# kalj/dealii-cuda

Measured on AMD Instinct MI355X. Metric: DoFs/s on 1305x Laplace vmult (bmop), p=4 3D uniform, higher is better.
Workload: dtype f64; 1 GPU; bmop: DEGREE_FE=4, DIMENSION=3, MATRIX_FREE_UNIFORM_MESH, hyper_cube(-1,1), 54^3 cells, 10218313 DoFs, 1 z-slab(s); cells_per_dir=54, n_dofs=10218313, n_cells=157464, parallelism=slab1, dof_numbering=caller's (lexicographic), finite=True, clock_ramp_steps=2000

## Files before the change

### dealii-cuda_amd/csrc/mfgpu_api.hip

```cpp
#include <hip/hip_runtime.h>

#include <type_traits>

#include <algorithm>
#include <cmath>
#include <cstdlib>
#include <cstring>
#include <memory>
#include <string>
#include <vector>

#include "mfgpu_kernels.h"

using namespace mfgpu;

struct EventTimer {
  std::vector<Event> ev;
  size_t used = 0;
  double ms = 0.0;
  int begin(hipStream_t st) {
    if (used + 2 > ev.size()) {
      Event e0, e1;
      int rc;
      if ((rc = e0.create(hipEventDefault)) || (rc = e1.create(hipEventDefault))) return rc;
      ev.push_back(std::move(e0));
      ev.push_back(std::move(e1));
    }
    HIP_TRY(hipEventRecord(ev[used].get(), st));
    return 0;
  }
  int end(hipStream_t st) {
    HIP_TRY(hipEventRecord(ev[used + 1].get(), st));
    used += 2;
    return 0;
  }
  int drain(double *total) {
    for (size_t i = 0; i + 1 < used; i += 2) {
      float t = 0.f;
      HIP_TRY(hipEventElapsedTime(&t, ev[i].get(), ev[i + 1].get()));
      ms += t;
    }
    used = 0;
    *total = ms;
    return 0;
  }
  void reset() {
    used = 0;
    ms = 0.0;
  }
};

struct mfgpu_handle {
  Plan plan;
  int dim = 0, n = 0, nd = 0, number_type = MFGPU_F64;
  bool hn = false;
  std::vector<double> S, Dt;
  std::vector<double> sv, sg;
  DeviceArray<uint32_t> d_batch_cell_off, d_batch_dof_off, d_bdofs;
  DeviceArray<uint8_t> d_bflags;
  DeviceArray<uint16_t> d_lmap;
  DeviceArray<uint16_t> d_lmapx;
  DeviceArray<uint16_t> d_perm;
  DeviceArray<uint32_t> d_bdofsp, d_idxp;
  DeviceArray<uint32_t> d_shtab;
  bool shared_records = false;
  size_t record_bytes = 0;
  DeviceArray<uint32_t> d_hnrec;
  DeviceArray<uint32_t> d_hn_slot;
  DeviceArray<void> d_coefp;
  DeviceArray<void> d_coef;
  DeviceArray<void> d_mass, d_massp;
  bool updatable = false;
  FoldGeometry geo;
  DeviceArray<uint32_t> d_cell_batch, d_cell_pos;
  size_t n_plane_cells = 0;
  DeviceArray<uint32_t> d_cmask, d_orphans;
  DeviceArray<void> d_hnw;
  DeviceArray<uint32_t> d_constrained;
  uint32_t n_constrained = 0;
  DeviceArray<void> d_tabsd;
  DeviceArray<void> d_tab2;
  bool twopass = true;
  DeviceArray<uint32_t> d_batch_nint, d_halo_off;
  std::vector<uint32_t> seg_end;
  std::vector<DeviceArray<uint32_t>> d_p2arr, d_p2tiles;
  std::vector<uint32_t> n_p2tiles;
  DeviceArray<uint32_t> d_p2rec, d_p2tab;
  bool p2_shared = false, p2_reverse = false, no_shared_records = false;
  Stream side;
  std::vector<Event> ev_seg;
  Event ev_side;
  bool side_pending = false;
  DeviceArray<void> d_halo;
  DeviceArray<unsigned long long> d_stamps;
  size_t lds = 0, device_bytes = 0;
  PlaneKernel planes = PlaneKernel::none;
  BatchKernel batches = BatchKernel::none;
  enum { kPlain, kMasked, kBatch };
  CellKernel<double> kernels_f64[3];
  CellKernel<float> kernels_f32[3];
  template <typename T>
  CellKernel<T> &kernel(int which) {
    if constexpr (std::is_same<T, double>::value) return kernels_f64[which];
    else return kernels_f32[which];
  }
  MultiKernel<double> multi_f64[kMaxFusedWidth - 1];
  MultiKernel<float> multi_f32[kMaxFusedWidth - 1];
  template <typename T>
  MultiKernel<T> &multi(int width) {
    if constexpr (std::is_same<T, double>::value) return multi_f64[width - 2];
    else return multi_f32[width - 2];
  }
  int multi_width = 1;
  DeviceArray<void> d_halo_multi;
  size_t halo_bytes = 0;
  uint32_t n_cus = 0, max_workgroups = 0;
  bool prof = false;
  EventTimer t_cells;
  EventTimer t_pass2;
  uint64_t prof_vmults = 0;
};

namespace {

template <typename T>
hipError_t bind_kernel(const mfgpu_handle *h, PlaneKernel pk, BatchKernel bk, bool hn, bool sh, CellKernel<T> *k) {
  const Plan &P = h->plan;
  const auto bind = pk == PlaneKernel::planes3 ? p_bind<T> : pk == PlaneKernel::planes4 ? q_bind<T>
                    : bk == BatchKernel::batches ? apply_bind<T> : bk == BatchKernel::x ? x_bind<T>
                    : bk == BatchKernel::g ? g_bind<T> : bk == BatchKernel::g2 ? g2_bind<T> : nullptr;
  if (!bind) return hipErrorInvalidValue;
  return bind(P.dim, P.n, hn, h->twopass, sh, h->d_mass.get() != nullptr, P.max_batch_dofs, k);
}

template <typename T, typename Args>
int launch_bound(mfgpu_handle *h, const CellKernel<T, Args> &k, const Args &a, uint32_t nbat, hipStream_t st) {
  if (!k.launch[0]) {
    set_error("cell-loop kernel not bound");
    return MFGPU_EINVAL;
  }
  uint32_t grid = (uint32_t)(k.per_cu < 1 ? 1 : k.per_cu) * h->n_cus;
  if (h->max_workgroups && h->max_workgroups < grid) grid = h->max_workgroups;
  HIP_TRY(k.launch[a.add != 0](a, h->S.data(), h->Dt.data(), k.lds, nbat < grid ? nbat : grid, st));
  return 0;
}

int check_symmetrize(int n, std::vector<double> &S, std::vector<double> &Dt) {
  const int p = n - 1;
  double err = 0, mag = 0;
  for (int r = 0; r < n; ++r)
    for (int c = 0; c < n; ++c) {
      const double s1 = S[r * n + c], s2 = S[(p - r) * n + (p - c)];
      const double d1 = Dt[r * n + c], d2 = -Dt[(p - r) * n + (p - c)];
      err = std::fmax(err, std::fmax(std::fabs(s1 - s2), std::fabs(d1 - d2)));
      mag = std::fmax(mag, std::fmax(std::fabs(s1), std::fabs(d1)));
    }
  if (err > 1e-10 * mag) {
    set_error("shape tables are not symmetric about the cell midpoint (unsupported)");
    return MFGPU_EUNSUPPORTED;
  }
  for (int r = 0; r < n; ++r)
    for (int c = 0; c < n; ++c) {
      const int r2 = p - r, c2 = p - c;
      if (r * n + c < r2 * n + c2) {
        const double s = 0.5 * (S[r * n + c] + S[r2 * n + c2]);
        S[r * n + c] = S[r2 * n + c2] = s;
        const double d = 0.5 * (Dt[r * n + c] - Dt[r2 * n + c2]);
        Dt[r * n + c] = d;
        Dt[r2 * n + c2] = -d;
      } else if (r == r2 && c == c2) {
        Dt[r * n + c] = 0.0;
      }
    }
  return 0;
}

int upload_pass2(mfgpu_handle *h, const uint32_t *priority, uint32_t n_priority) {
  const Plan &P = h->plan;
  const size_t ng = 1 + h->seg_end.size();
  const bool shared = P.sh_p2_use && !h->no_shared_records && n_priority == 0 && ng == 2;
  std::vector<Pass2Group> groups;
  int rc;
  if ((rc = pass2_groups(P, h->seg_end, priority, n_priority, shared, groups))) return rc;
  std::vector<DeviceArray<uint32_t>> d_arr(ng), d_tiles(ng);
  std::vector<uint32_t> n_tiles(ng, 0u);
  const bool reverse = (size_t)P.halo_off.back() * esize(h->number_type) <= ((size_t)256 << 20);
  DeviceArray<uint32_t> d_rec, d_tab;
  if (shared) {
    if ((rc = d_rec.upload(P.sh_p2rec.data(), P.sh_p2rec.size()))) return rc;
    if ((rc = d_tab.upload(P.sh_p2tab.data(), P.sh_p2tab.size()))) return rc;
  }
  for (size_t g = 0; g < ng; ++g) {
    std::vector<uint32_t> arr, tiles;
    build_pass2_classes(groups[g].dofs, groups[g].offsets, groups[g].slots, arr, tiles);
    n_tiles[g] = (uint32_t)(tiles.size() / 4);
    if (reverse) {
      const size_t nt = tiles.size() / 4;
      for (size_t a = 0, b = nt ? nt - 1 : 0; a < b; ++a, --b)
        for (int w = 0; w < 4; ++w) std::swap(tiles[4 * a + w], tiles[4 * b + w]);
    }
    if ((rc = d_arr[g].upload(arr.data(), arr.size()))) return rc;
    if ((rc = d_tiles[g].upload(tiles.data(), tiles.size()))) return rc;
  }
  h->d_p2arr = std::move(d_arr);
  h->d_p2tiles = std::move(d_tiles);
  h->n_p2tiles = std::move(n_tiles);
  h->d_p2rec = std::move(d_rec);
  h->d_p2tab = std::move(d_tab);
  h->p2_shared = shared;
  h->p2_reverse = reverse;
  return 0;
}

template <typename T>
int relayout_planes(mfgpu_handle *h, const uint32_t *cell_batch, const uint32_t *cell_pos, bool coef, bool mass,
                    hipStream_t st) {
  const size_t total = h->n_plane_cells * (size_t)h->nd;
  if (coef)
    HIP_TRY(relayout_coef_launch<T>(h->d_coefp.as<T>(), h->d_coef.as<const T>(), cell_batch, cell_pos, total, h->n, st));
  if (mass)
    HIP_TRY(relayout_coef_launch<T>(h->d_massp.as<T>(), h->d_mass.as<const T>(), cell_batch, cell_pos, total, h->n, st));
  return 0;
}

template <typename T>
int update_typed(mfgpu_handle *h, const void *coef, const void *mass, hipStream_t st) {
  const FoldInputs<T> in = h->geo.inputs<T>();
  if (coef) HIP_TRY(fold_coefficient_launch<T>(h->d_coef.as<T>(), (const T *)coef, in, st));
  if (mass) HIP_TRY(fold_mass_launch<T>(h->d_mass.as<T>(), (const T *)mass, in, st));
  if (h->planes == PlaneKernel::none) return 0;
  return relayout_planes<T>(h, h->d_cell_batch.get(), h->d_cell_pos.get(), coef != nullptr, mass != nullptr, st);
}

template <typename T>
int create_arrays(mfgpu_handle *h, const mfgpu_desc &d) {
  const Plan &P = h->plan;
  const size_t ncell = P.n_cells, nd = (size_t)P.nd;
  size_t &acct = h->device_bytes;
  auto up = [&](auto &arr, const void *src, size_t n) {
    const int rc = arr.upload(src, n);
    acct += arr.bytes();
    return rc;
  };
  int rc;
  if ((rc = up(h->d_batch_cell_off, P.batch_cell_off.data(), P.batch_cell_off.size()))) return rc;
  if ((rc = up(h->d_batch_dof_off, P.batch_dof_off.data(), P.batch_dof_off.size()))) return rc;
  if ((rc = up(h->d_bdofs, P.bdofs.data(), P.bdofs.size()))) return rc;
  if ((rc = up(h->d_bflags, P.bflags.data(), P.bflags.size()))) return rc;
  if ((rc = up(h->d_lmap, P.lmap.data(), P.lmap.size()))) return rc;
  const bool general = h->batches == BatchKernel::g || h->batches == BatchKernel::g2;
  if (h->batches == BatchKernel::x && !h->hn) {
    const std::vector<uint16_t> perm = x_lane_permutation(P.n);
    if ((rc = up(h->d_perm, perm.data(), perm.size()))) return rc;
  }
  if (h->batches == BatchKernel::x || general) {
    const std::vector<uint16_t> lx = x_pencil_runs(P.lmap, P.n);
    if ((rc = up(h->d_lmapx, lx.data(), lx.size()))) return rc;
  }
  if (h->batches == BatchKernel::g2) {
    std::vector<T> sd(2 * (size_t)P.n * P.n);
    for (int i = 0; i < P.n * P.n; ++i) {
      sd[i] = (T)h->S[i];
      sd[P.n * P.n + i] = (T)h->Dt[i];
    }
    if ((rc = up(h->d_tabsd, sd.data(), sd.size() * sizeof(T)))) return rc;
  }
  if (h->planes != PlaneKernel::none) {
    if ((rc = build_plane_records(h->plan, d.constraint_mask))) return rc;
    if (!P.pr_hn.empty()) {
      if ((rc = up(h->d_hnrec, P.pr_hn.data(), P.pr_hn.size()))) return rc;
      if ((rc = up(h->d_hn_slot, P.pr_hn_slot.data(), P.pr_hn_slot.size()))) return rc;
    }
    h->shared_records = P.sh_use && !(d.flags & MFGPU_NO_SHARED_RECORDS) &&
                        kernel_exists(h->planes, P.n, d.number_type, false, true, d.mass_coefficient != nullptr);
    const std::vector<uint32_t> &rd = h->shared_records ? P.sh_dofs : P.pr_dofs;
    const std::vector<uint32_t> &rx = h->shared_records ? P.sh_idx : P.pr_idx;
    if ((rc = up(h->d_bdofsp, rd.data(), rd.size()))) return rc;
    if ((rc = up(h->d_idxp, rx.data(), rx.size()))) return rc;
    if (h->shared_records && (rc = up(h->d_shtab, P.sh_batch.data(), P.sh_batch.size()))) return rc;
    h->record_bytes = h->d_bdofsp.bytes() + h->d_idxp.bytes() + h->d_shtab.bytes();
  }
  if ((rc = up(h->d_orphans, P.orphans.data(), P.orphans.size()))) return rc;
  if (h->twopass) {
    if ((rc = up(h->d_batch_nint, P.batch_nint.data(), P.batch_nint.size()))) return rc;
    if ((rc = up(h->d_halo_off, P.halo_off.data(), P.halo_off.size()))) return rc;
    if (h->planes != PlaneKernel::none && (uint64_t)P.halo_off.back() >= (1ull << 29)) {
      set_error("halo buffer too large for 32-bit byte offsets");
      return MFGPU_EUNSUPPORTED;
    }
    const size_t hb = ((size_t)P.halo_off.back() + 1) * sizeof(T);
    if ((rc = h->d_halo.alloc(hb, true))) return rc;
    acct += hb;
    h->halo_bytes = hb;
  }
  if (h->hn) {
    std::vector<uint32_t> cm(ncell);
    for (size_t i = 0; i < ncell; ++i) cm[i] = d.constraint_mask[P.cell_order[i]];
    if ((rc = up(h->d_cmask, cm.data(), ncell))) return rc;
    std::vector<T> w((size_t)h->n * h->n);
    for (size_t i = 0; i < w.size(); ++i) w[i] = (T)d.constraint_weights[i];
    if ((rc = up(h->d_hnw, w.data(), w.size() * sizeof(T)))) return rc;
  }
  FoldGeometry geo;
  if ((rc = geo.upload(d.JxW, d.inv_jac, P.cell_order.data(), P.dim, (uint32_t)ncell, (uint32_t)nd, general,
                       d.number_type)))
    return rc;
  DeviceArray<T> metric;
  if ((rc = fold_coefficient<T>(metric, d.coefficient, d.quadrature_points, geo.inputs<T>()))) return rc;
  h->d_coef = std::move(metric);
  acct += h->d_coef.bytes();
  if (d.mass_coefficient) {
    DeviceArray<T> mass;
    if ((rc = fold_mass<T>(mass, d.mass_coefficient, geo.inputs<T>()))) return rc;
    h->d_mass = std::move(mass);
    acct += h->d_mass.bytes();
  }
  if (h->updatable) {
    acct += geo.bytes();
    h->geo = std::move(geo);
  }
  if (h->planes != PlaneKernel::none) {
    const int n = P.n, NT = p_cells_per_wave(n) * n;
    const size_t nbat = P.n_plane_batches, total = nbat * (size_t)(n * n) * NT;
    const size_t ncell_p = P.batch_cell_off[nbat];
    std::vector<uint32_t> cb(ncell_p), cp(ncell_p);
    for (size_t b = 0; b < nbat; ++b)
      for (uint32_t c = P.batch_cell_off[b]; c < P.batch_cell_off[b + 1]; ++c) {
        cb[c] = (uint32_t)b;
        cp[c] = c - P.batch_cell_off[b];
      }
    DeviceArray<uint32_t> t_cb, t_cp;
    if ((rc = t_cb.upload(cb.data(), ncell_p))) return rc;
    if ((rc = t_cp.upload(cp.data(), ncell_p))) return rc;
    if ((rc = h->d_coefp.alloc(total * sizeof(T), true))) return rc;
    acct += h->d_coefp.bytes();
    h->n_plane_cells = ncell_p;
    if (d.mass_coefficient) {
      if ((rc = h->d_massp.alloc(total * sizeof(T), true))) return rc;
      acct += h->d_massp.bytes();
    }
    if ((rc = relayout_planes<T>(h, t_cb.get(), t_cp.get(), true, d.mass_coefficient != nullptr, nullptr))) return rc;
    HIP_TRY(hipDeviceSynchronize());
    if (h->updatable) {
      acct += t_cb.bytes() + t_cp.bytes();
      h->d_cell_batch = std::move(t_cb);
      h->d_cell_pos = std::move(t_cp);
    }
  }
  int dev = 0;
  hipDeviceProp_t prop;
  HIP_TRY(hipGetDevice(&dev));
  HIP_TRY(hipGetDeviceProperties(&prop, dev));
  h->n_cus = (uint32_t)prop.multiProcessorCount;
  h->max_workgroups = d.max_workgroups;
  if (h->planes != PlaneKernel::none) {
    CellKernel<T> &plain = h->kernel<T>(mfgpu_handle::kPlain), &masked = h->kernel<T>(mfgpu_handle::kMasked);
    HIP_TRY(bind_kernel<T>(h, h->planes, BatchKernel::none, false, h->shared_records, &plain));
    h->lds = plain.lds;
    if (P.n_plain_plane_batches < P.n_plane_batches) {
      HIP_TRY(bind_kernel<T>(h, h->planes, BatchKernel::none, true, false, &masked));
      h->lds = std::max(h->lds, masked.lds);
    }
  }
  if (h->batches == BatchKernel::none) return 0;
  CellKernel<T> &batch = h->kernel<T>(mfgpu_handle::kBatch);
  const hipError_t bind_batch_family = bind_kernel<T>(h, PlaneKernel::none, h->batches, h->hn, false, &batch);
  h->lds = batch.lds;
  if (h->lds > 160 * 1024) {
    set_error("batch needs more than 160 KiB of LDS; lower max_dofs_per_batch");
    return MFGPU_EINVAL;
  }
  HIP_TRY(bind_batch_family);
  if (h->twopass && h->planes == PlaneKernel::none)
    for (const int w : kFusedWidths) {
      if (!fused_kernel_exists(h->batches, P.n, d.number_type, h->hn, h->d_mass.get() != nullptr, w)) continue;
      MultiKernel<T> &mk = h->multi<T>(w);
      if (g_bind_width<T>(P.n, h->hn, false, h->d_mass.get() != nullptr, w, P.max_batch_dofs, &mk) != hipSuccess) {
        (void)hipGetLastError();
        mk = MultiKernel<T>();
      } else
        h->multi_width = std::max(h->multi_width, w);
    }
  return 0;
}

void choose_segments(mfgpu_handle *h, uint32_t request) {
  const Plan &P = h->plan;
  const uint32_t nb = (uint32_t)(P.batch_cell_off.size() - 1);
  h->seg_end.assign(1, nb);
  if (!h->twopass || nb < 2 || request == 1) return;
  const uint32_t npl = P.n_plane_batches, nplain = P.n_plain_plane_batches;
  std::vector<uint32_t> cuts;
  if (npl > 0 && npl < nb) cuts.push_back(npl);
  if (nplain > 0 && nplain < npl) cuts.push_back(nplain);
  if (request > 1) {
    for (uint32_t i = 1; i < request; ++i) cuts.push_back((uint32_t)((uint64_t)nb * i / request));
  }
  if (request == 0 && !P.pr_hn.empty() && nplain == 0 && P.n == 5) cuts.push_back(nb / 2);
  std::sort(cuts.begin(), cuts.end());
  h->seg_end.clear();
  for (uint32_t c : cuts)
    if (c > 0 && c < nb && (h->seg_end.empty() || h->seg_end.back() != c)) h->seg_end.push_back(c);
  h->seg_end.push_back(nb);
}

template <typename T>
int create_typed(mfgpu_handle *h, const mfgpu_desc &d) {
  int rc = create_arrays<T>(h, d);
  if (rc) return rc;
  choose_segments(h, d.cell_loop_segments);
  if (!h->twopass) return 0;
  if (h->seg_end.size() > 1) {
    int prio_least = 0, prio_greatest = 0;
    HIP_TRY(hipDeviceGetStreamPriorityRange(&prio_least, &prio_greatest));
    if ((rc = h->side.create(hipStreamNonBlocking, prio_least))) return rc;
    if ((rc = h->ev_side.create(hipEventDisableTiming))) return rc;
    h->ev_seg.resize(h->seg_end.size() - 1);
    for (Event &e : h->ev_seg)
      if ((rc = e.create(hipEventDisableTiming))) return rc;
  }
  return upload_pass2(h, nullptr, 0);
}

template <typename T>
int launch_pass2_group(mfgpu_handle *h, size_t group, void *dst, const void *src, hipStream_t st, int add) {
  if (h->p2_shared && group == 1)
    HIP_TRY(reduce_owner_batches_launch<T>((T *)dst, (const T *)src, h->d_halo.as<const T>(), h->d_p2rec.get(),
                                           h->d_p2tab.get(), (uint32_t)(h->plan.batch_cell_off.size() - 1),
                                           (uint32_t)p_hs(h->plan.n) * 64u, h->p2_reverse ? 1 : 0, add, st));
  HIP_TRY(reduce_classes_launch<T>((T *)dst, (const T *)src, h->d_halo.as<const T>(), h->d_p2arr[group].get(),
                                   h->d_p2tiles[group].get(), h->n_p2tiles[group], add, st));
  return 0;
}

template <typename T>
int vmult_pass2(mfgpu_handle *h, int phase, void *dst, const void *src, hipStream_t st, int add) {
  if (!h->twopass) return 0;
  if (phase == 0) return launch_pass2_group<T>(h, 0, dst, src, st, add);
  int rc = launch_pass2_group<T>(h, h->seg_end.size(), dst, src, st, add);
  if (!rc && h->side_pending) {
    HIP_TRY(hipStreamWaitEvent(st, h->ev_side.get(), 0));
    h->side_pending = false;
  }
  return rc;
}

template <typename T>
int launch_cells(mfgpu_handle *h, ApplyArgs<T> a, uint32_t b0, uint32_t b1, hipStream_t st) {
  const Plan &P = h->plan;
  const uint32_t npl = P.n_plane_batches, nplain = P.n_plain_plane_batches;
  if (b0 < nplain) {
    a.batch0 = b0;
    a.batch_end = b1 < nplain ? b1 : nplain;
    if (const int rc = launch_bound(h, h->kernel<T>(mfgpu_handle::kPlain), a, a.batch_end - a.batch0, st)) return rc;
    b0 = a.batch_end;
  }
  if (b0 < npl && b0 < b1) {
    a.batch0 = b0;
    a.batch_end = b1 < npl ? b1 : npl;
    if (const int rc = launch_bound(h, h->kernel<T>(mfgpu_handle::kMasked), a, a.batch_end - a.batch0, st)) return rc;
    b0 = a.batch_end;
  }
  if (b0 >= b1) return 0;
  a.batch0 = b0;
  a.batch_end = b1;
  return launch_bound(h, h->kernel<T>(mfgpu_handle::kBatch), a, b1 - b0, st);
}

template <typename T>
ApplyArgs<T> make_args(mfgpu_handle *h, void *dst, const void *src, int add) {
  const Plan &P = h->plan;
  ApplyArgs<T> a;
  a.batch_cell_off = h->d_batch_cell_off.get();
  a.batch_dof_off = h->d_batch_dof_off.get();
  a.bdofs = h->d_bdofs.get();
  a.bflags = h->d_bflags.get();
  a.lmap = h->d_lmap.get();
  a.lmapx = h->d_lmapx.get();
  a.perm = h->d_perm.get();
  a.bdofsp = h->d_bdofsp.get();
  a.idxp = h->d_idxp.get();
  a.shtab = h->shared_records ? h->d_shtab.get() : nullptr;
  a.hnrec = h->d_hnrec.get();
  a.hn_slot = h->d_hn_slot.get();
  a.coefp = h->d_coefp.as<const T>();
  a.coef = h->d_coef.as<const T>();
  a.mass = h->d_mass.as<const T>();
  a.massp = h->d_massp.as<const T>();
  a.cmask = h->d_cmask.get();
  a.hn_weights = h->d_hnw.as<const T>();
  a.tabS = h->d_tabsd.as<const T>();
  a.tabDt = a.tabS ? a.tabS + (size_t)P.n * P.n : nullptr;
  a.batch_nint = h->d_batch_nint.get();
  a.halo_off = h->d_halo_off.get();
  a.halo = h->d_halo.as<T>();
  a.dst = (T *)dst;
  a.src = (const T *)src;
  a.nb_max = P.max_batch_dofs;
  a.add = add;
  a.stamps = h->d_stamps.get();
  a.dbg = 0;
  return a;
}

template <typename T>
int vmult_main(mfgpu_handle *h, void *dst, const void *src, hipStream_t st, int add) {
  const Plan &P = h->plan;
  ApplyArgs<T> a = make_args<T>(h, dst, src, add);
  int rc;
  if (h->prof && (rc = h->t_cells.begin(st))) return rc;
  if (h->twopass) {
    const size_t nseg = h->seg_end.size();
    if (h->side_pending) {
      HIP_TRY(hipStreamWaitEvent(st, h->ev_side.get(), 0));
      h->side_pending = false;
    }
    for (size_t s = 0; s < nseg; ++s) {
      if ((rc = launch_cells<T>(h, a, s ? h->seg_end[s - 1] : 0u, h->seg_end[s], st))) return rc;
      if (s + 1 < nseg) {
        HIP_TRY(hipEventRecord(h->ev_seg[s].get(), st));
        HIP_TRY(hipStreamWaitEvent(h->side.get(), h->ev_seg[s].get(), 0));
        if ((rc = launch_pass2_group<T>(h, 1 + s, dst, src, h->side.get(), add))) return rc;
      }
    }
    if (nseg > 1) {
      HIP_TRY(hipEventRecord(h->ev_side.get(), h->side.get()));
      h->side_pending = true;
    }
  } else {
    for (size_t c = 0; c + 1 < P.color_batch_off.size(); ++c) {
      if (P.color_batch_off[c + 1] == P.color_batch_off[c]) continue;
      if ((rc = launch_cells<T>(h, a, P.color_batch_off[c], P.color_batch_off[c + 1], st))) return rc;
    }
  }
  if (h->prof && (rc = h->t_cells.end(st))) return rc;
  if (!h->twopass)
    HIP_TRY(orphan_launch<T>((T *)dst, (const T *)src, h->d_orphans.get(), (uint32_t)P.orphans.size(), add, st));
  if (h->prof) h->prof_vmults++;
  return 0;
}

template <typename T>
int vmult_typed(mfgpu_handle *h, void *dst, const void *src, hipStream_t st, int add) {
  int rc = vmult_main<T>(h, dst, src, st, add);
  if (rc) return rc;
  const bool timed = h->prof && h->twopass;
  if (timed && (rc = h->t_pass2.begin(st))) return rc;
  rc = vmult_pass2<T>(h, 0, dst, src, st, add);
  if (!rc) rc = vmult_pass2<T>(h, 1, dst, src, st, add);
  if (!rc && timed) rc = h->t_pass2.end(st);
  return rc;
}

bool fused_by_default(int , int ) { return false; }

template <typename T>
int multi_fused_group(mfgpu_handle *h, T *dst, const T *src, int nv, size_t stride, hipStream_t st, int add) {
  const MultiKernel<T> &k = h->multi<T>(nv);
  if (!k.launch[0]) {
    set_error("fused kernel not bound");
    return MFGPU_EINVAL;
  }
  if (!h->d_halo_multi.get()) {
    const size_t bytes = (size_t)(h->multi_width - 1) * h->halo_bytes;
    if (const int rc = h->d_halo_multi.alloc(bytes, true)) return rc;
// ... 41 lines not shown
  for (const uint32_t g : multi_groups(n_vectors, widths)) {
    const int rc = g > 1 ? multi_fused_group<T>(h, d, s, (int)g, stride, st, add) : vmult_typed<T>(h, d, s, st, add);
    if (rc) return rc;
    d += (size_t)g * stride;
    s += (size_t)g * stride;
  }
  return 0;
}

}

namespace {
template <typename T>
int inverse_diagonal_typed(mfgpu_handle *h, void *diag, hipStream_t st) {
  const Plan &P = h->plan;
  const bool general = h->batches == BatchKernel::g || h->batches == BatchKernel::g2;
  if (!h->d_tab2.get()) {
    const int nn = h->n * h->n;
    std::vector<T> t2(2 * (size_t)nn);
    for (int i = 0; i < nn; ++i) {
      t2[i] = (T)(general ? h->sv[i] : h->sv[i] * h->sv[i]);
      t2[nn + i] = (T)(general ? h->sg[i] : h->sg[i] * h->sg[i]);
    }
    if (const int rc = h->d_tab2.upload(t2.data(), t2.size() * sizeof(T))) return rc;
    h->device_bytes += h->d_tab2.bytes();
  }
  HIP_TRY(fill_launch<T>((T *)diag, P.n_dofs, T(0), st));
  const uint32_t nb = (uint32_t)(P.batch_cell_off.size() - 1), *cell_off = h->d_batch_cell_off.get();
  const uint32_t *dof_off = h->d_batch_dof_off.get(), *bdofs = h->d_bdofs.get(), *cmask = h->d_cmask.get();
  const uint16_t *lmap = h->d_lmap.get();
  const T *coef = h->d_coef.as<const T>(), *hnw = h->d_hnw.as<const T>(), *tab2 = h->d_tab2.as<const T>();
  if (h->batches == BatchKernel::g2)
    HIP_TRY(diag_general2_launch<T>(P.n, (T *)diag, nb, cell_off, dof_off, bdofs, lmap, coef, cmask, hnw, tab2, st));
  else if (h->batches == BatchKernel::g)
    HIP_TRY(diag_general_launch<T>(P.n, (T *)diag, nb, cell_off, dof_off, bdofs, lmap, coef, cmask, hnw, tab2, st));
  else
    HIP_TRY(diag_launch<T>(P.dim, P.n, (T *)diag, nb, cell_off, dof_off, bdofs, lmap, coef, cmask, hnw, tab2, st));
  if (h->d_mass.get())
    HIP_TRY(diag_mass_launch<T>(P.dim, P.n, (T *)diag, nb, cell_off, dof_off, bdofs, lmap, h->d_mass.as<const T>(), cmask,
                                hnw, tab2, !general, st));
  HIP_TRY(set_values_launch<T>((T *)diag, h->d_constrained.get(), h->n_constrained, T(1), st));
  HIP_TRY(vec_map_launch<T>(4, (T *)diag, nullptr, T(0), T(0), P.n_dofs, st));
  return 0;
}
}


namespace {
int vec_map(int op, void *v, const void *w, double s, double a, size_t n, int nt, void *stream) {
  if ((!v && n) || (!w && n && op <= 3)) {
    set_error("null vector");
    return MFGPU_EINVAL;
  }
  if (nt == MFGPU_F32)
    HIP_TRY(vec_map_launch<float>(op, (float *)v, (const float *)w, (float)s, (float)a, n, (hipStream_t)stream));
  else if (nt == MFGPU_F64)
    HIP_TRY(vec_map_launch<double>(op, (double *)v, (const double *)w, s, a, n, (hipStream_t)stream));
  else
    return MFGPU_EINVAL;
  return 0;
}
int vec_reduce(int op, void *v, const void *x, const void *w, double a, size_t n, int nt, void *stream, double *out) {
  if (!out || (n && (!v || (op != 2 && !w) || (op == 1 && !x)))) {
    set_error("null argument");
    return MFGPU_EINVAL;
  }
  if (nt == MFGPU_F32)
    HIP_TRY(vec_reduce_launch<float>(op, (float *)v, (const float *)x, (const float *)w, (float)a, n, (hipStream_t)stream, out));
  else if (nt == MFGPU_F64)
    HIP_TRY(vec_reduce_launch<double>(op, (double *)v, (const double *)x, (const double *)w, a, n, (hipStream_t)stream, out));
  else
    return MFGPU_EINVAL;
  return 0;
}
}


namespace mfgpu {
int handle_number_type(const mfgpu_handle *h) { return h->number_type; }
int handle_set_priority_dofs(mfgpu_handle *h, const uint32_t *ids, uint32_t n) {
  return h->twopass ? upload_pass2(h, ids, n) : 0;
}
int handle_n_batches(const mfgpu_handle *h) { return (int)h->plan.batch_cell_off.size() - 1; }
bool handle_ranged_ok(const mfgpu_handle *h) { return h->twopass && h->seg_end.size() == 1; }
int handle_batches_touching(const mfgpu_handle *h, const uint32_t *ids, uint32_t n, std::vector<uint8_t> &flags) {
  const Plan &P = h->plan;
  std::vector<uint8_t> mark(P.n_dofs, 0);
  for (uint32_t i = 0; i < n; ++i) {
    if (ids[i] >= P.n_dofs) {
      set_error("interface dof out of range");
      return MFGPU_EINVAL;
    }
    mark[ids[i]] = 1;
  }
  const size_t nb = P.batch_cell_off.size() - 1;
  flags.assign(nb, 0);
  for (size_t b = 0; b < nb; ++b)
    for (uint32_t t = P.batch_dof_off[b]; t < P.batch_dof_off[b + 1]; ++t)
      if (mark[P.bdofs[t] & 0x7fffffffu]) {
        flags[b] = 1;
        break;
      }
  return 0;
}
int handle_cells_range(mfgpu_handle *h, uint32_t b0, uint32_t b1, void *dst, const void *src, void *stream, int add) {
  if (b0 >= b1) return 0;
  hipStream_t st = (hipStream_t)stream;
  if (h->number_type == MFGPU_F64) return launch_cells<double>(h, make_args<double>(h, dst, src, add), b0, b1, st);
  return launch_cells<float>(h, make_args<float>(h, dst, src, add), b0, b1, st);
}
int handle_cells_two_ranges(mfgpu_handle *h, uint32_t b0, uint32_t b1, uint32_t c0, uint32_t c1, void *dst,
                            const void *src, void *stream, int add) {
  const uint32_t nplain = h->plan.n_plain_plane_batches, npl = h->plan.n_plane_batches;
  const bool plain = c1 <= nplain, masked = b0 >= nplain && c1 <= npl;
  if (b0 >= b1 || c0 >= c1 || b1 > c0 || !(plain || masked)) {
    const int rc = handle_cells_range(h, b0, b1, dst, src, stream, add);
    return rc ? rc : handle_cells_range(h, c0, c1, dst, src, stream, add);
  }
  hipStream_t st = (hipStream_t)stream;
  auto run = [&](auto a) -> int {
    a.batch0 = b0;
    a.batch_end = c1;
    a.hole0 = b1;
    a.hole_len = c0 - b1;
    using T = typename std::remove_const<typename std::remove_pointer<decltype(a.src)>::type>::type;
    return launch_bound(h, h->kernel<T>(plain ? mfgpu_handle::kPlain : mfgpu_handle::kMasked), a, (b1 - b0) + (c1 - c0),
                        st);
  };
  return h->number_type == MFGPU_F64 ? run(make_args<double>(h, dst, src, add)) : run(make_args<float>(h, dst, src, add));
}
int handle_pass2_group(mfgpu_handle *h, int group, void *dst, const void *src, void *stream, int add) {
  if (!h->twopass) return 0;
  hipStream_t st = (hipStream_t)stream;
  return h->number_type == MFGPU_F64 ? launch_pass2_group<double>(h, (size_t)group, dst, src, st, add)
                                     : launch_pass2_group<float>(h, (size_t)group, dst, src, st, add);
}
int handle_vmult_phase(mfgpu_handle *h, int phase, void *dst, const void *src, void *stream, int add) {
  hipStream_t st = (hipStream_t)stream;
  if (h->number_type == MFGPU_F64)
    return phase == 0 ? vmult_main<double>(h, dst, src, st, add) : vmult_pass2<double>(h, phase - 1, dst, src, st, add);
  return phase == 0 ? vmult_main<float>(h, dst, src, st, add) : vmult_pass2<float>(h, phase - 1, dst, src, st, add);
}
}

extern "C" {

int mfgpu_create(const mfgpu_desc *desc, mfgpu_handle **out) {
  if (!desc || !out) {
    set_error("null argument");
    return MFGPU_EINVAL;
  }
  const mfgpu_desc &d = *desc;
  if (!valid_number_type(d.number_type)) {
    set_error("number_type must be MFGPU_F64 or MFGPU_F32");
    return MFGPU_EINVAL;
  }
  const bool general = !(d.flags & MFGPU_UNIFORM_J0);
  if (general && (d.flags & MFGPU_COLORED_SCATTER)) {
    set_error("the general-Jacobian path (no MFGPU_UNIFORM_J0) is implemented in two-pass scatter mode only");
    return MFGPU_EUNSUPPORTED;
  }
  if (!d.JxW || !d.inv_jac || !d.shape_values || !d.shape_gradients ||
      (!d.coefficient && !d.quadrature_points)) {
    set_error("JxW, inv_jac, shape tables and coefficient (or quadrature_points) are required");
    return MFGPU_EINVAL;
  }
  const bool hn = (d.flags & MFGPU_HANGING_NODES) != 0;
// ... 66 lines not shown
}

int mfgpu_vmult_multi(mfgpu_handle *h, void *dst, const void *src, uint32_t n_vectors, size_t stride, uint32_t flags,
                      void *stream) {
  if (!h || !dst || !src) {
    set_error("null argument");
    return MFGPU_EINVAL;
  }
  const size_t nd = h->plan.n_dofs;
  if (n_vectors == 0 || (n_vectors > 1 && stride < nd)) {
    set_error("mfgpu_vmult_multi: n_vectors must be >= 1 and stride >= n_dofs");
    return MFGPU_EINVAL;
  }
  if ((flags & ~(MFGPU_MULTI_ADD | MFGPU_MULTI_LOOP | MFGPU_MULTI_FUSED)) ||
      ((flags & MFGPU_MULTI_LOOP) && (flags & MFGPU_MULTI_FUSED))) {
    set_error("mfgpu_vmult_multi: bad flags (MFGPU_MULTI_LOOP and MFGPU_MULTI_FUSED exclude each other)");
    return MFGPU_EINVAL;
  }
  const size_t bytes = ((size_t)(n_vectors - 1) * stride + nd) * esize(h->number_type);
  const char *d0 = (const char *)dst, *s0 = (const char *)src;
  if (d0 < s0 + bytes && s0 < d0 + bytes) {
    set_error("mfgpu_vmult_multi: the dst range overlaps the src range");
    return MFGPU_EINVAL;
  }
  return h->number_type == MFGPU_F64 ? vmult_multi_typed<double>(h, dst, src, n_vectors, stride, flags, (hipStream_t)stream)
                                     : vmult_multi_typed<float>(h, dst, src, n_vectors, stride, flags, (hipStream_t)stream);
}

int mfgpu_multi_width(const mfgpu_handle *h) { return h ? h->multi_width : 0; }

int mfgpu_update_coefficients(mfgpu_handle *h, const void *coefficient_dev, const void *mass_coefficient_dev,
                              void *stream) {
  if (!h) {
    set_error("null argument");
    return MFGPU_EINVAL;
  }
  if (!h->updatable) {
    set_error("mfgpu_update_coefficients: the handle was created without MFGPU_UPDATABLE_COEFFICIENTS");
    return MFGPU_EINVAL;
  }
  if (!coefficient_dev && !mass_coefficient_dev) {
    set_error("mfgpu_update_coefficients: coefficient_dev and mass_coefficient_dev are both NULL");
    return MFGPU_EINVAL;
  }
  if (mass_coefficient_dev && !h->d_mass.get()) {
    set_error("mfgpu_update_coefficients: the handle was created without a mass term (its kernels have no mass "
              "instantiation bound); create it with mass_coefficient");
    return MFGPU_EINVAL;
  }
  return h->number_type == MFGPU_F64 ? update_typed<double>(h, coefficient_dev, mass_coefficient_dev, (hipStream_t)stream)
                                     : update_typed<float>(h, coefficient_dev, mass_coefficient_dev, (hipStream_t)stream);
}

uint32_t mfgpu_n_dofs(const mfgpu_handle *h) { return h ? h->plan.n_dofs : 0; }

size_t mfgpu_memory_consumption(const mfgpu_handle *h) { return h ? h->device_bytes : 0; }

int mfgpu_plan_stats(const mfgpu_handle *h, uint64_t s[8]) {
  if (!h || !s) return MFGPU_EINVAL;
  const Plan &P = h->plan;
  s[0] = P.batch_cell_off.size() - 1;
  s[1] = P.color_batch_off.size() - 1;
  s[2] = P.bdofs.size();
  s[3] = P.max_batch_dofs;
  s[4] = P.max_batch_cells;
  s[5] = P.orphans.size();
  s[6] = P.n_first;
  s[7] = P.n_add;
  if (h->twopass) {
    const uint32_t nb = (uint32_t)s[0], npl = P.n_plane_batches, nplain = P.n_plain_plane_batches;
    const uint32_t edge[4] = {0u, nplain, npl, nb};
    s[1] = 0;
    for (size_t g = 0; g < h->seg_end.size(); ++g) {
      const uint32_t s0 = g ? h->seg_end[g - 1] : 0u, s1 = h->seg_end[g];
      for (int f = 0; f < 3; ++f)
        if (std::max(s0, edge[f]) < std::min(s1, edge[f + 1])) ++s[1];
    }
    s[6] = P.sdofs.size();
    s[7] = P.halo_off.back();
  }
  return 0;
}

int mfgpu_record_stats(const mfgpu_handle *h, uint64_t s[4]) {
  if (!h || !s) return MFGPU_EINVAL;
  const Plan &P = h->plan;
  const size_t n = (size_t)P.n, nb = (size_t)p_kgu((int)n) * 64, nx = ((n * n + 1) / 2) * (p_cells_per_wave((int)n) * n);
  const bool planes = h->planes != PlaneKernel::none;
  s[0] = (h->shared_records ? 1 : 0) | (h->p2_shared ? 2 : 0);
  s[1] = planes ? P.sh_dofs.size() / nb : 0;
  s[2] = planes ? P.sh_idx.size() / nx : 0;
  s[3] = h->record_bytes;
  return 0;
}

const char *mfgpu_kernel_name(const mfgpu_handle *h) {
  if (!h) return "";
  const bool x = h->batches == BatchKernel::x;
  switch (h->planes) {
    case PlaneKernel::planes3: return x ? "apply_planes3+apply_batches_x" : "apply_planes3";
    case PlaneKernel::planes4: return x ? "apply_planes4+apply_batches_x" : "apply_planes4";
    default: break;
  }
  switch (h->batches) {
    case BatchKernel::x: return "apply_batches_x";
    case BatchKernel::g: return "apply_batches_g";
    case BatchKernel::g2: return "apply_batches_g2";
    default: return "apply_batches";
  }
}

int mfgpu_profile_enable(mfgpu_handle *h, int on) {
  if (!h) return MFGPU_EINVAL;
  h->prof = on != 0;
  h->t_cells.reset();
  h->t_pass2.reset();
  h->prof_vmults = 0;
  return 0;
}

int mfgpu_profile_read_pass2(mfgpu_handle *h, double *ms) {
  if (!h || !ms) return MFGPU_EINVAL;
  HIP_TRY(hipDeviceSynchronize());
  return h->t_pass2.drain(ms);
}

int mfgpu_profile_read(mfgpu_handle *h, double *ms, uint64_t *nv) {
  if (!h || !ms || !nv) return MFGPU_EINVAL;
  HIP_TRY(hipDeviceSynchronize());
  if (const int rc = h->t_cells.drain(ms)) return rc;
  *nv = h->prof_vmults;
  return 0;
}

#ifdef MFGPU_STAMPS
int mfgpu_debug_stamps(mfgpu_handle *h, unsigned long long *out, size_t n_batches) {
  if (!h) return MFGPU_EINVAL;
  const size_t nbt = h->plan.batch_cell_off.size() - 1;
  if (!h->d_stamps.get()) return h->d_stamps.alloc(2 * nbt * 16, true);
  if (out && n_batches == nbt) {
    HIP_TRY(hipDeviceSynchronize());
    HIP_TRY(hipMemcpy(out, h->d_stamps.get(), 2 * nbt * 16 * sizeof(unsigned long long), hipMemcpyDeviceToHost));
  }
  return 0;
}
#endif


int mfgpu_compute_inverse_diagonal(mfgpu_handle *h, void *inv_diag, void *stream) {
  if (!h || !inv_diag) {
    set_error("null argument");
    return MFGPU_EINVAL;
  }
  return h->number_type == MFGPU_F64 ? inverse_diagonal_typed<double>(h, inv_diag, (hipStream_t)stream)
                                     : inverse_diagonal_typed<float>(h, inv_diag, (hipStream_t)stream);
}

int mfgpu_set_constrained_values(mfgpu_handle *h, void *vec, double value, void *stream) {
  if (!h || !vec) {
    set_error("null argument");
    return MFGPU_EINVAL;
  }
  if (h->number_type == MFGPU_F64)
    HIP_TRY(set_values_launch<double>((double *)vec, h->d_constrained.get(), h->n_constrained, value, (hipStream_t)stream));
  else
    HIP_TRY(set_values_launch<float>((float *)vec, h->d_constrained.get(), h->n_constrained, (float)value,
// ... 81 lines not shown
```

### dealii-cuda_amd/csrc/mfgpu_internal.h

```cpp
#ifndef MFGPU_INTERNAL_H
#define MFGPU_INTERNAL_H

#include <cstdint>
#include <string>
#include <vector>

#include "../../include/mfgpu.h"

namespace mfgpu {

void set_error(const std::string &msg);

inline int ipow(int a, int e) {
  int r = 1;
  for (int i = 0; i < e; ++i) r *= a;
  return r;
}

constexpr int p_cells_per_wave(int n) { return 64 / n; }
constexpr int p_ji(int n) { return n == 3 ? 2 : n == 4 ? 5 : n == 5 ? 9 : n == 6 ? 14 : 23; }
constexpr int p_hs(int n) { return n == 3 ? 3 : n == 4 ? 6 : n == 5 ? 9 : n == 6 ? 14 : 18; }
constexpr int p_kgu(int n) { return p_ji(n) + p_hs(n); }
constexpr int p_cell_stride(int n) {
  int s = n * n * n;
  while ((s & 31) != (n & 31)) ++s;
  return s;
}

constexpr int q_plane_stride(int n) { return n >= 6 ? 65 : n == 5 ? 33 : n == 4 ? 17 : 33; }
constexpr int q_cell_stride(int n) { return n * q_plane_stride(n); }
constexpr int p_priv_max(int n) { return n >= 5 ? 384 : n == 4 ? 256 : 192; }
constexpr int kHnOpRounds = 2;
constexpr int p_hn_rows(int n) { return p_priv_max(n) / 64 + 3 * kHnOpRounds * 3 + 2; }

template <typename T>
constexpr size_t q_region_doubles(int n) {
  const size_t t = ((size_t)(p_cells_per_wave(n) + 1) * q_cell_stride(n) * sizeof(T) + 7) / 8;
  const size_t u = (size_t)p_kgu(n) * 64 + p_priv_max(n);
  return t > u ? t : u;
}
template <typename T>
constexpr size_t q_lds_bytes(int n, bool hn) {
  return (q_region_doubles<T>(n) + (hn ? (size_t)n * n : 0)) * 8;
}

constexpr uint8_t kFlagConstrained = 1;
constexpr uint8_t kFlagAdd = 2;

struct Plan {
  int dim = 0, degree = 0, n = 0, nd = 0;
  uint32_t n_dofs = 0, n_cells = 0;
  std::vector<uint32_t> cell_order;
  std::vector<uint32_t> batch_cell_off;
  std::vector<uint32_t> batch_dof_off;
  std::vector<uint32_t> color_batch_off;
  std::vector<uint32_t> bdofs;
  std::vector<uint8_t> bflags;
  std::vector<uint16_t> lmap;
  std::vector<uint32_t> orphans;
  std::vector<uint32_t> batch_nint;
  std::vector<uint32_t> halo_off;
  std::vector<uint32_t> sdofs;
  std::vector<uint32_t> s_off;
  std::vector<uint32_t> s_idx;
  std::vector<uint32_t> chunks;
  std::vector<uint32_t> gstarts;
  uint32_t max_batch_dofs = 0, max_batch_cells = 0;
  uint32_t n_plane_batches = 0;
  uint32_t n_plain_plane_batches = 0;
  std::vector<uint32_t> pr_dofs, pr_idx, pr_hn, pr_hn_slot;
  std::vector<uint32_t> sh_dofs, sh_idx, sh_batch;
  bool sh_use = false;
  std::vector<uint32_t> sh_p2rec, sh_p2tab;
  bool sh_p2_use = false;
  uint64_t n_first = 0, n_add = 0;
};

struct PlanLimits {
  uint32_t max_cells = 0, max_dofs = 0;
  uint32_t interior_max = 0, shared_max = 0, halo_stride = 0;
  bool segregate_masked = false;
  bool masked_planes = false;
  uint32_t private_max = 0;
};

int build_plan(const mfgpu_desc &d, Plan &plan, uint32_t max_chunks = 3, const PlanLimits *limits = nullptr);

struct HnLine {
  uint16_t node[8];
};
void hn_cell_lines(unsigned mask, int n, std::vector<HnLine> (&lines)[3], std::vector<uint16_t> &nodes);

enum class PlaneKernel : uint8_t { none, planes3, planes4 };
enum class BatchKernel : uint8_t { none, batches, x, g, g2 };
int choose_kernel_and_plan(const mfgpu_desc &d, PlaneKernel &pk, BatchKernel &bk, Plan &plan);

constexpr bool planes4_wide(int n) { return n >= 6; }
constexpr bool kernel_exists(PlaneKernel k, int n, int number_type, bool hn, bool sh, bool mass) {
  switch (k) {
    case PlaneKernel::planes3: return n >= 3 && n <= 5 && !(sh && hn);
    case PlaneKernel::planes4:
      return planes4_wide(n) ? n <= 7 && !hn && !sh && !mass
                             : n >= 3 && !sh && !(mass && n == 5 && number_type == MFGPU_F64);
    default: return false;
  }
}
constexpr bool kernel_exists(BatchKernel k, int n, int , bool , bool sh, bool ) {
  return k != BatchKernel::none && n >= 2 && n <= 7 && !sh;
}
constexpr int kFusedWidths[] = {3, 2};
constexpr bool fused_kernel_exists(BatchKernel k, int n, int number_type, bool hn, bool , int nv) {
  return k == BatchKernel::g && n >= 2 && n <= 7 && (nv == 2 || nv == 3) &&
         !(hn && number_type == MFGPU_F64 && n >= (nv == 3 ? 6 : 7));
}
std::vector<uint32_t> multi_groups(uint32_t n_vectors, const std::vector<uint32_t> &widths);
int build_plane_records(Plan &plan, const uint32_t *constraint_mask);
constexpr int kShBatchWords = 4;
constexpr double kShareMaxFraction = 0.5;
void share_plane_records(Plan &plan);
constexpr int kP2Header = 16, kP2MaxK = 12, kP2SlotBits = 12;
void share_pass2_records(Plan &plan);

std::vector<uint16_t> x_lane_permutation(int n);
std::vector<uint16_t> x_pencil_runs(const std::vector<uint16_t> &lmap, int n);
struct Pass2Group {
  std::vector<uint32_t> dofs, offsets = std::vector<uint32_t>(1, 0u), slots;
};
int pass2_groups(const Plan &plan, const std::vector<uint32_t> &seg_end, const uint32_t *priority, uint32_t n_priority,
                 bool shared, std::vector<Pass2Group> &groups);

int derive_tables(int n, const double *shape_values, const double *shape_gradients,
                  std::vector<double> &S, std::vector<double> &Dt);

int handle_number_type(const mfgpu_handle *h);
int handle_set_priority_dofs(mfgpu_handle *h, const uint32_t *ids, uint32_t n);
int handle_vmult_phase(mfgpu_handle *h, int phase, void *dst, const void *src, void *stream, int add);
int handle_n_batches(const mfgpu_handle *h);
bool handle_ranged_ok(const mfgpu_handle *h);
int handle_batches_touching(const mfgpu_handle *h, const uint32_t *ids, uint32_t n, std::vector<uint8_t> &flags);
int handle_cells_range(mfgpu_handle *h, uint32_t b0, uint32_t b1, void *dst, const void *src, void *stream, int add);
int handle_cells_two_ranges(mfgpu_handle *h, uint32_t b0, uint32_t b1, uint32_t c0, uint32_t c1, void *dst,
                            const void *src, void *stream, int add);
int handle_pass2_group(mfgpu_handle *h, int group, void *dst, const void *src, void *stream, int add);

void transfer_sizes(const mfgpu_transfer *t, uint32_t *n_coarse_dofs, uint32_t *n_fine_dofs, int *number_type);
void vcycle_active(const mfgpu_vcycle *v, int *active_type, uint32_t *n_active);

}

struct mfgpu_plan {
  mfgpu::Plan plan;
};

#endif
```

### dealii-cuda_amd/csrc/mfgpu_kernels.h

```cpp
#ifndef MFGPU_KERNELS_H
#define MFGPU_KERNELS_H

#include <hip/hip_runtime.h>

#include <type_traits>

#include "mfgpu_device.h"
#include "mfgpu_internal.h"

namespace mfgpu {

template <typename T>
struct ApplyArgs {
  const uint32_t *batch_cell_off;
  const uint32_t *batch_dof_off;
  const uint32_t *bdofs;
  const uint8_t *bflags;
  const uint16_t *lmap;
  const uint16_t *lmapx;
  const uint16_t *perm;
  const uint32_t *bdofsp;
  const uint32_t *idxp;
  const T *coefp;
  const uint32_t *hnrec;
  const uint32_t *hn_slot;
  const T *coef;
  const uint32_t *cmask;
  const T *hn_weights;
  const T *tabS, *tabDt;
  const uint32_t *batch_nint;
  const uint32_t *halo_off;
  T *halo;
  T *dst;
  const T *src;
  uint32_t batch0;
  uint32_t batch_end;
  uint32_t hole0 = 0xffffffffu, hole_len = 0;
  uint32_t nb_max;
  int add;
  unsigned long long *stamps;
  int dbg;
  const uint32_t *shtab = nullptr;
  const T *mass = nullptr;
  const T *massp = nullptr;
};

constexpr int kMaxFusedWidth = 3;
template <typename T>
struct MultiArgs : ApplyArgs<T> {
  size_t stride = 0;
  T *halos[kMaxFusedWidth];
};
constexpr size_t kMaxLdsBytes = 160 * 1024;

template <typename T, int n>
struct Tables {
  T S[((n + 1) / 2) * n];
  T Dt[((n + 1) / 2) * n];
};

template <typename T, int n>
inline Tables<T, n> make_tables(const double *S, const double *Dt) {
  Tables<T, n> tab;
  for (int i = 0; i < ((n + 1) / 2) * n; ++i) {
    tab.S[i] = (T)S[i];
    tab.Dt[i] = (T)Dt[i];
  }
  return tab;
}

template <typename T, typename Args = ApplyArgs<T>>
struct CellKernel {
  size_t lds = 0;
  int per_cu = 0;
  hipError_t (*launch[2])(const Args &a, const double *S, const double *Dt, size_t lds, uint32_t grid,
                          hipStream_t st) = {nullptr, nullptr};
};

template <typename T, int Block, auto K, auto MakeTab, typename Args = ApplyArgs<T>>
hipError_t launch_cell_kernel(const Args &a, const double *S, const double *Dt, size_t lds, uint32_t grid,
                              hipStream_t st) {
  if constexpr (std::is_null_pointer_v<decltype(MakeTab)>)
    hipLaunchKernelGGL(K, dim3(grid), dim3(Block), lds, st, a);
  else
    hipLaunchKernelGGL(K, dim3(grid), dim3(Block), lds, st, a, MakeTab(S, Dt));
  return hipGetLastError();
}

template <typename T, int Block, auto K0, auto K1, auto MakeTab, typename Args = ApplyArgs<T>>
hipError_t bind_cell_kernel(size_t lds, CellKernel<T, Args> *k) {
  k->lds = lds;
  for (const void *f : {(const void *)K1, (const void *)K0})
    if (const hipError_t e = hipFuncSetAttribute(f, hipFuncAttributeMaxDynamicSharedMemorySize, (int)lds)) return e;
  k->launch[0] = launch_cell_kernel<T, Block, K0, MakeTab, Args>;
  k->launch[1] = launch_cell_kernel<T, Block, K1, MakeTab, Args>;
  return hipOccupancyMaxActiveBlocksPerMultiprocessor(&k->per_cu, (const void *)K0, Block, lds);
}

template <typename F>
hipError_t dispatch_flags(F &&f) { return f(); }
template <typename F, typename... B>
hipError_t dispatch_flags(F &&f, bool flag, B... rest) {
  return dispatch_flags(
      [&](auto... c) { return flag ? f(std::true_type{}, c...) : f(std::false_type{}, c...); }, rest...);
}
template <typename F, typename... B>
hipError_t dispatch_instantiation(int n, F &&f, B... flags) {
  auto at = [&](auto N) { return dispatch_flags([&](auto... c) { return f(N, c...); }, flags...); };
  switch (n) {
    case 2: return at(std::integral_constant<int, 2>{});
    case 3: return at(std::integral_constant<int, 3>{});
    case 4: return at(std::integral_constant<int, 4>{});
    case 5: return at(std::integral_constant<int, 5>{});
    case 6: return at(std::integral_constant<int, 6>{});
    case 7: return at(std::integral_constant<int, 7>{});
    default: return hipErrorInvalidValue;
  }
}
template <typename T>
constexpr int number_type_of = sizeof(T) == 8 ? MFGPU_F64 : MFGPU_F32;

#define MFGPU_CELL_LOOP_FAMILY(F)                                                                              \
  template <typename T>                                                                                        \
  hipError_t F##_bind(int dim, int n, bool hn, bool twopass, bool sh, bool mass, uint32_t nb_max, CellKernel<T> *k);
MFGPU_CELL_LOOP_FAMILY(apply)
MFGPU_CELL_LOOP_FAMILY(x)
MFGPU_CELL_LOOP_FAMILY(g)
MFGPU_CELL_LOOP_FAMILY(g2)
MFGPU_CELL_LOOP_FAMILY(p)
MFGPU_CELL_LOOP_FAMILY(q)
#undef MFGPU_CELL_LOOP_FAMILY
template <typename T>
using MultiKernel = CellKernel<T, MultiArgs<T>>;
template <typename T, typename Args>
hipError_t g_bind_width(int n, bool hn, bool sh, bool mass, int nv, uint32_t nb_max, CellKernel<T, Args> *k);

void build_pass2_classes(const std::vector<uint32_t> &sdofs, const std::vector<uint32_t> &s_off,
                         const std::vector<uint32_t> &s_idx, std::vector<uint32_t> &arr, std::vector<uint32_t> &tiles);
template <typename T>
hipError_t reduce_classes_launch(T *dst, const T *src, const T *halo, const uint32_t *arr, const uint32_t *tiles,
                                 uint32_t n_tiles, int add, hipStream_t st);
template <typename T>
hipError_t reduce_classes_multi_launch(int nv, T *dst, const T *src, size_t stride, T *const *halos, const uint32_t *arr,
                                       const uint32_t *tiles, uint32_t n_tiles, int add, hipStream_t st);
template <typename T>
hipError_t reduce_owner_batches_launch(T *dst, const T *src, const T *halo, const uint32_t *rec, const uint32_t *tab,
                                       uint32_t n_batches, uint32_t hstride, int reverse, int add, hipStream_t st);
template <typename T>
hipError_t relayout_coef_launch(T *out, const T *in, const uint32_t *cell_batch, const uint32_t *cell_pos,
                                size_t total, int n, hipStream_t st);
template <typename T>
hipError_t fold_general_launch(T *M, const T *coef, const T *jxw, const T *jinv, const uint32_t *order,
                               uint32_t n_cells, uint32_t nd, hipStream_t st);
template <typename T>
hipError_t fold_general2_launch(T *M, const T *coef, const T *jxw, const T *jinv, const uint32_t *order,
                                uint32_t n_cells, uint32_t nd, hipStream_t st);
template <typename T>
hipError_t orphan_launch(T *dst, const T *src, const uint32_t *orph, uint32_t n, int add, hipStream_t st);
template <typename T>
hipError_t coefficient_launch(T *coef, const T *qpts, size_t nq, int dim, hipStream_t st);
template <typename T>
hipError_t fold_launch(T *c, const T *coef, const T *jxw, const T *j0, const uint32_t *order,
                       uint32_t n_cells, uint32_t nd, hipStream_t st);
template <typename T>
hipError_t fill_launch(T *v, size_t n, T a, hipStream_t st);
template <typename T>
struct FoldInputs {
  const T *jxw = nullptr, *jinv = nullptr;
  const uint32_t *order = nullptr;
  int dim = 0;
  uint32_t n_cells = 0, nd = 0;
  bool general = false;
  size_t metric_entries() const { return (size_t)n_cells * nd * (general ? (dim == 3 ? 6 : 3) : 1); }
};
template <typename T>
hipError_t fold_coefficient_launch(T *out, const T *coef, const FoldInputs<T> &in, hipStream_t st);
template <typename T>
hipError_t fold_mass_launch(T *out, const T *c, const FoldInputs<T> &in, hipStream_t st);
struct FoldGeometry {
  DeviceArray<void> jxw, jinv;
  DeviceArray<uint32_t> order;
  int dim = 0;
  uint32_t n_cells = 0, nd = 0;
  bool general = false;
  int upload(const void *JxW, const void *inv_jac, const uint32_t *cell_order, int dim_, uint32_t n_cells_, uint32_t nd_,
             bool general_, int number_type);
  size_t bytes() const { return jxw.bytes() + jinv.bytes() + order.bytes(); }
  template <typename T>
  FoldInputs<T> inputs(const T *jxw_resident = nullptr) const {
    FoldInputs<T> in;
    in.jxw = jxw_resident ? jxw_resident : jxw.as<const T>();
    in.jinv = jinv.as<const T>();
    in.order = order.get();
    in.dim = dim, in.n_cells = n_cells, in.nd = nd, in.general = general;
    return in;
  }
};
template <typename T>
int fold_mass(DeviceArray<T> &out, const void *mass_coefficient, const FoldInputs<T> &in);
template <typename T>
int fold_coefficient(DeviceArray<T> &out, const void *coefficient, const void *quadrature_points,
                     const FoldInputs<T> &in);

template <typename T>
hipError_t diag_launch(int dim, int n, T *diag, uint32_t n_batches, const uint32_t *batch_cell_off,
                       const uint32_t *batch_dof_off, const uint32_t *bdofs, const uint16_t *lmap, const T *coef,
                       const uint32_t *cmask, const T *hn_weights, const T *tab2, hipStream_t st);
template <typename T>
hipError_t diag_general_launch(int n, T *diag, uint32_t n_batches, const uint32_t *batch_cell_off,
                               const uint32_t *batch_dof_off, const uint32_t *bdofs, const uint16_t *lmap,
                               const T *metric, const uint32_t *cmask, const T *hn_weights, const T *tab,
                               hipStream_t st);
template <typename T>
hipError_t diag_general2_launch(int n, T *diag, uint32_t n_batches, const uint32_t *batch_cell_off,
                                const uint32_t *batch_dof_off, const uint32_t *bdofs, const uint16_t *lmap,
                                const T *metric, const uint32_t *cmask, const T *hn_weights, const T *tab,
                                hipStream_t st);
template <typename T>
hipError_t diag_mass_launch(int dim, int n, T *diag, uint32_t n_batches, const uint32_t *batch_cell_off,
                            const uint32_t *batch_dof_off, const uint32_t *bdofs, const uint16_t *lmap, const T *mass,
                            const uint32_t *cmask, const T *hn_weights, const T *tab, bool squared, hipStream_t st);
template <typename T>
hipError_t set_values_launch(T *v, const uint32_t *idx, uint32_t n, T value, hipStream_t st);
template <typename T>
hipError_t vec_map_launch(int op, T *v, const T *w, T s, T a, size_t n, hipStream_t st);
template <typename T>
hipError_t vec_reduce_launch(int op, T *v, const T *x, const T *w, T a, size_t n, hipStream_t st, double *out);

}
#endif
// ... 1 lines not shown
```

### dealii-cuda_amd/csrc/mfgpu_kernels_p.hip

```cpp
#include <hip/hip_runtime.h>

#include "mfgpu_cell.h"
#include "mfgpu_kernels.h"
#include "mfgpu_planes.h"

namespace mfgpu {

#define MFGPU_PIN_VMEM() __builtin_amdgcn_sched_barrier(0x380)

template <int n, typename T, bool ADD, bool HN, bool SH = false, bool MASS = false>
__global__ void __launch_bounds__(64) __attribute__((amdgpu_waves_per_eu(1, 1)))
apply_planes3(const ApplyArgs<T> A, const TablesEO<T, n> tab) {
  constexpr int n2 = n * n;
  constexpr int CW = p_cells_per_wave(n);
  constexpr int NT = CW * n;
  constexpr int KGU = p_kgu(n);
  constexpr int JI = p_ji(n);
  constexpr int HS = KGU - JI;
  constexpr int SA = p_cell_stride(n);
  constexpr int NIW = (n2 + 1) / 2;
  extern __shared__ __attribute__((aligned(16))) unsigned char smem_raw[];
  constexpr int PRIV = HN ? p_priv_max(n) : 0;
  double *ua = reinterpret_cast<double *>(smem_raw);
  T *Aw = reinterpret_cast<T *>(ua + KGU * 64 + PRIV + (HN ? n2 : 0));
  T *Bw = Aw + (CW + 1) * SA;
  double *Wl = ua + KGU * 64 + PRIV;

  const int lane = threadIdx.x;
  if (HN) {
    if (lane < n2) Wl[lane] = (double)A.hn_weights[lane];
  }
  const int lc = lane / n, k = lane - lc * n;
  const bool lane_on = lane < NT;
  const int tk = lane_on ? lane : NT - 1;

  uint32_t b, bstride, bend;
  {
    const uint32_t nbt = A.batch_end - A.batch0 - A.hole_len, G = gridDim.x;
    if (G >= 8 && nbt >= G) {
      const uint32_t xcd = blockIdx.x & 7u, slot = blockIdx.x >> 3;
      const uint32_t q = G >> 3, rem = G & 7u;
      const uint32_t wlo = xcd * q + (xcd < rem ? xcd : rem);
      const uint32_t w = q + (xcd < rem ? 1u : 0u);
      b = A.batch0 + (uint32_t)((uint64_t)nbt * wlo / G) + slot;
      bend = A.batch0 + (uint32_t)((uint64_t)nbt * (wlo + w) / G);
      bstride = w;
    } else {
      b = A.batch0 + blockIdx.x;
      bend = A.batch_end - A.hole_len;
      bstride = G;
    }
  }
  if (b >= bend) return;
  const uint32_t hole0 = A.hole0, hole_len = A.hole_len;
  auto next_of = [&](uint32_t x) {
    const uint32_t l = (x >= hole0 ? x - hole_len : x) + bstride;
    return l < bend ? (l >= hole0 ? l + hole_len : l) : x;
  };
  if (b >= hole0) b += hole_len;
  static_assert(kernel_exists(PlaneKernel::planes3, n, number_type_of<T>, HN, SH, MASS), "no such instantiation");
  struct Meta {
    uint32_t base, drec, irec;
  };
  auto meta_request = [&](uint32_t bb) -> uint32_t {
    return A.shtab[(size_t)bb * kShBatchWords + (lane & (kShBatchWords - 1))];
  };
  auto meta_of = [&](uint32_t v) -> Meta {
    return Meta{(uint32_t)__builtin_amdgcn_readlane((int)v, 0), (uint32_t)__builtin_amdgcn_readlane((int)v, 1),
                (uint32_t)__builtin_amdgcn_readlane((int)v, 2)};
  };

  auto load_dofs = [&](uint32_t rec, uint32_t (&g)[KGU]) {
    const uint32_t *p = A.bdofsp + (size_t)rec * (KGU * 64) + lane;
#pragma unroll
    for (int j = 0; j < KGU; ++j) g[j] = SH ? p[j * 64] : nt_load(p + j * 64);
  };
  auto src_at = [&](uint32_t base, uint32_t g) -> T {
    const T *const sp = SH ? A.src + base : A.src;
    return *reinterpret_cast<const T *>(reinterpret_cast<const char *>(sp) + (uint32_t)(g * (uint32_t)sizeof(T)));
  };
  auto dst_at = [&](uint32_t base, uint32_t g) -> T * {
    T *const dp = SH ? A.dst + base : A.dst;
    return reinterpret_cast<T *>(reinterpret_cast<char *>(dp) + (uint32_t)(g * (uint32_t)sizeof(T)));
  };
  auto load_ix = [&](uint32_t rec, uint32_t (&ix)[NIW]) {
    const uint32_t *p = A.idxp + (size_t)rec * (NIW * NT) + tk;
#pragma unroll
    for (int w = 0; w < NIW; ++w) ix[w] = SH ? p[w * NT] : nt_load(p + w * NT);
  };
  auto stage_src = [&](const uint32_t (&g)[KGU], const T (&sv)[KGU]) {
#pragma unroll
    for (int j = 0; j < KGU; ++j) {
      double v = (double)sv[j];
      if (j >= JI) {
        const unsigned long long keep = (unsigned long long)(long long)~((int)g[j] >> 31);
        v = __longlong_as_double((long long)((unsigned long long)__double_as_longlong(v) & keep));
      }
      ua[lane + j * 64] = v;
    }
  };
  auto ixb = [&](const uint32_t (&ix)[NIW], int i) -> uint32_t {
    return (i & 1) ? (ix[i >> 1] >> 16) : (ix[i >> 1] & 0xffffu);
  };
  auto scatter_slot = [&](int j, uint32_t bb, uint32_t base, uint32_t g, T r, T oldv) {
    if (j < JI) {
      *dst_at(base, g) = ADD ? oldv + r : r;
    } else {
      T *const hp = A.halo + (size_t)bb * (HS * 64) + lane;
      hp[(j - JI) * 64] = r;
    }
  };

  uint32_t b1 = next_of(b), b2 = next_of(b1);
  uint32_t Gp[KGU], Gc[KGU], Gn[KGU], Gnn[KGU];
  uint32_t IXc[NIW], IXn[NIW];
  constexpr int CR = PRIV / 64, HROWS = HN ? p_hn_rows(n) : 1;
  uint32_t Hc[HROWS], Hn[HROWS];
  auto load_hn = [&](uint32_t bb, uint32_t (&H)[HROWS]) {
    const uint32_t slot = A.hn_slot[bb];
    if (slot != 0xffffffffu) {
      const uint32_t *p = A.hnrec + (size_t)slot * (HROWS * 64) + lane;
#pragma unroll
      for (int w = 0; w < HROWS; ++w) H[w] = nt_load(p + w * 64);
    } else {
#pragma unroll
      for (int w = 0; w < HROWS; ++w) H[w] = 0u;
    }
  };
  T Cc[n2];
  T Mm[MASS ? n2 : 1];
  T SVn[KGU], R[KGU], old[KGU];
  Meta Mp{0u, 0u, 0u}, Mc = Mp, M1 = Mp, M2 = Mp;
  uint32_t Mv = 0u;
  if (SH) {
    Mc = meta_of(meta_request(b));
    M1 = meta_of(meta_request(b1));
    M2 = meta_of(meta_request(b2));
    Mp = Mc;
  }
  load_dofs(SH ? Mc.drec : b, Gc);
  load_dofs(SH ? M1.drec : b1, Gn);
  load_ix(SH ? Mc.irec : b, IXc);
  if (HN) load_hn(b, Hc);
  constexpr uint32_t kDummyIx = 8u * (uint32_t)(KGU * 64 - 1) * 0x10001u;
#pragma unroll
  for (int w = 0; w < NIW; ++w) IXc[w] = lane_on ? IXc[w] : kDummyIx;
  {
    const T *p = A.coefp + (size_t)b * (n2 * NT) + tk;
#pragma unroll
    for (int r = 0; r < n2; ++r) Cc[r] = nt_load(p + r * NT);
  }
  if (MASS) {
    const T *p = A.massp + (size_t)b * (n2 * NT) + tk;
#pragma unroll
    for (int r = 0; r < n2; ++r) Mm[r] = nt_load(p + r * NT);
  }
#pragma unroll
  for (int j = 0; j < KGU; ++j) {
    SVn[j] = src_at(Mc.base, Gc[j]);
    Gp[j] = Gc[j];
    R[j] = T(0);
    old[j] = T(0);
  }
  stage_src(Gc, SVn);
  WaveSync::sync();

  const int pxy = lc * SA + n2 * k;
  const int pyz = lc * SA + k;
  uint32_t bp = b;

  while (true) {
    const bool has_next = b1 != b;
    constexpr int kH2 = HN ? HROWS - 2 : 0, kH1 = HN ? HROWS - 1 : 0;
    const uint32_t hn_ncopy = HN ? (uint32_t)__builtin_amdgcn_readfirstlane(Hc[kH2] & 0xffffu) : 0u;
    auto hn_count = [&](int dir) -> uint32_t {
      const uint32_t w = dir == 0 ? Hc[kH2] >> 16 : dir == 1 ? Hc[kH1] & 0xffffu : Hc[kH1] >> 16;
      return (uint32_t)__builtin_amdgcn_readfirstlane(w);
    };
    auto hn_pass = [&](int dir, bool transposed, const double (&Wr)[n2]) {
      const uint32_t count = hn_count(dir);
#pragma unroll
      for (int r = 0; r < kHnOpRounds; ++r) {
        if ((uint32_t)(r * 64) >= count) break;
        const bool on = (uint32_t)(r * 64 + lane) < count;
        const uint32_t *ww = &Hc[CR + (dir * kHnOpRounds + r) * 3];
        double v[n], o[n];
        uint32_t pos[n];
#pragma unroll
        for (int t = 0; t < n; ++t) {
          pos[t] = on ? (ww[t >> 1] >> (16 * (t & 1))) & 0xffffu : (uint32_t)(KGU * 64 + PRIV - 1);
          v[t] = ua[pos[t]];
        }
#pragma unroll
        for (int i = 0; i < n; ++i) {
          double acc = 0.0;
#pragma unroll
          for (int k2 = 0; k2 < n; ++k2) acc = fma(transposed ? Wr[k2 * n + i] : Wr[i * n + k2], v[k2], acc);
          o[i] = acc;
        }
        if (on) {
#pragma unroll
          for (int i = 0; i < n; ++i) ua[pos[i]] = o[i];
        }
      }
    };
    if (HN && hn_ncopy) {
      double Wr[n2];
#pragma unroll
      for (int i = 0; i < n2; ++i) Wr[i] = Wl[i];
      double cv[CR > 0 ? CR : 1];
#pragma unroll
      for (int r = 0; r < CR; ++r) cv[r] = (uint32_t)(r * 64 + lane) < hn_ncopy ? ua[Hc[r] & 0xffffu] : 0.0;
#pragma unroll
      for (int r = 0; r < CR; ++r)
        if ((uint32_t)(r * 64 + lane) < hn_ncopy) ua[Hc[r] >> 16] = cv[r];
      WaveSync::sync();
      hn_pass(0, false, Wr);
      WaveSync::sync();
      hn_pass(1, false, Wr);
      WaveSync::sync();
      hn_pass(2, false, Wr);
      WaveSync::sync();
    }
    STAMP(0);
    RSTAMP(8);
    WGSTAMP(10);
    load_dofs(SH ? M2.drec : b2, Gnn);
    load_ix(SH ? M1.irec : b1, IXn);
    if (SH) Mv = meta_request(next_of(b2));
    if (HN) load_hn(b1, Hn);
    if (ADD) {
#pragma unroll
      for (int j = 0; j < JI; ++j) old[j] = *dst_at(Mp.base, Gp[j]);
    }
    STAMP(1);
    auto hookA = [&](int) {};
    auto hookB = [&](int s) {
      MFGPU_PIN_VMEM();
#pragma unroll
      for (int j = (KGU * s) / (5 * n); j < (KGU * (s + 1)) / (5 * n); ++j)
        scatter_slot(j, bp, Mp.base, Gp[j], R[j], old[j]);
#pragma unroll
      for (int j = (KGU * s) / (5 * n); j < (KGU * (s + 1)) / (5 * n); ++j)
        SVn[j] = src_at(M1.base, Gn[j]);
      MFGPU_PIN_VMEM();
    };
    const T *const cnext = A.coefp + (size_t)b1 * (n2 * NT) + tk;
    const T *const mnext = MASS ? A.massp + (size_t)b1 * (n2 * NT) + tk : nullptr;
    auto hookC = [&](int s) {
      MFGPU_PIN_VMEM();
#pragma unroll
      for (int r = (n2 * s) / (2 * n); r < (n2 * (s + 1)) / (2 * n); ++r)
        Cc[r] = nt_load(cnext + r * NT);
      if (MASS) {
#pragma unroll
        for (int r = (n2 * s) / (2 * n); r < (n2 * (s + 1)) / (2 * n); ++r)
          Mm[r] = nt_load(mnext + r * NT);
      }
      MFGPU_PIN_VMEM();
    };

    {
      T u[n2];
#pragma unroll
      for (int x = 0; x < n; ++x)
#pragma unroll
        for (int y = 0; y < n; ++y)
          u[x + n * y] = (T) * reinterpret_cast<const double *>(reinterpret_cast<const char *>(ua) + ixb(IXc, x + n * y));
#pragma unroll
      for (int x = 0; x < n; ++x) {
        T in[n], out[n];
        get_line<n, 1>(u, x, in);
        eo_apply<n, 0>(tab, in, out);
        set_line<n, 1>(u, x, out);
        hookA(x);
      }
#pragma unroll
      for (int y = 0; y < n; ++y) {
        T in[n], a[n], bb[n];
        get_line<n, 0>(u, y, in);
        eo_apply<n, 0>(tab, in, a);
        eo_apply<n, 2>(tab, a, bb);
#pragma unroll
        for (int x = 0; x < n; ++x) {
          Aw[pxy + x + n * y] = a[x];
          Bw[pxy + x + n * y] = bb[x];
        }
        hookA(n + y);
      }
    }
    WaveSync::sync();
    STAMP(2);
#pragma unroll
    for (int j = 0; j < KGU + PRIV / 64; ++j) ua[lane + j * 64] = 0.0;

    {
      T nx[n];
#pragma unroll
      for (int z = 0; z < n; ++z) nx[z] = Bw[pyz + n2 * z];
#pragma unroll
      for (int y = 0; y < n; ++y) {
        T in[n], g[n], o[n];
#pragma unroll
        for (int z = 0; z < n; ++z) in[z] = nx[z];
#pragma unroll
        for (int z = 0; z < n; ++z) nx[z] = y + 1 < n ? Bw[pyz + n * (y + 1) + n2 * z] : Aw[pyz + n2 * z];
        eo_apply<n, 0>(tab, in, g);
#pragma unroll
        for (int z = 0; z < n; ++z) g[z] *= Cc[y + n * z];
        eo_apply<n, 1>(tab, g, o);
#pragma unroll
        for (int z = 0; z < n; ++z) Bw[pyz + n * y + n2 * z] = o[z];
        hookB(y);
      }
      T v[n2], r[n2];
#pragma unroll
      for (int y = 0; y < n; ++y) {
        T in[n], o[n];
#pragma unroll
        for (int z = 0; z < n; ++z) in[z] = nx[z];
        if (y + 1 < n) {
#pragma unroll
          for (int z = 0; z < n; ++z) nx[z] = Aw[pyz + n * (y + 1) + n2 * z];
        }
// ... 21 lines not shown
        for (int y = 0; y < n; ++y) g[y] *= Cc[y + n * z];
        eo_apply<n, 3>(tab, g, o);
#pragma unroll
        for (int y = 0; y < n; ++y) r[y + n * z] += MASS ? fma(Mm[y + n * z], in[y], o[y]) : o[y];
        hookB(3 * n + z);
      }
#pragma unroll
      for (int y = 0; y < n; ++y) {
        T in[n], o[n];
        get_line<n, 1>(r, y, in);
        eo_apply<n, 1>(tab, in, o);
#pragma unroll
        for (int z = 0; z < n; ++z) Aw[pyz + n * y + n2 * z] = o[z];
        hookB(4 * n + y);
      }
    }
    WaveSync::sync();
    STAMP(3);

    {
      T o[n2];
      T nr[n], nt[n];
#pragma unroll
      for (int x = 0; x < n; ++x) {
        nr[x] = Aw[pxy + x];
        nt[x] = Bw[pxy + x];
      }
#pragma unroll
      for (int y = 0; y < n; ++y) {
        T rp[n], tp[n], w[n], ol[n];
#pragma unroll
        for (int x = 0; x < n; ++x) {
          rp[x] = nr[x];
          tp[x] = nt[x];
        }
        if (y + 1 < n) {
#pragma unroll
          for (int x = 0; x < n; ++x) {
            nr[x] = Aw[pxy + x + n * (y + 1)];
            nt[x] = Bw[pxy + x + n * (y + 1)];
          }
        }
        eo_apply<n, 3>(tab, tp, w);
#pragma unroll
        for (int x = 0; x < n; ++x) w[x] += rp[x];
        eo_apply<n, 1>(tab, w, ol);
        set_line<n, 0>(o, y, ol);
        hookC(y);
      }
#pragma unroll
      for (int x = 0; x < n; ++x) {
        T in[n], out[n];
        get_line<n, 1>(o, x, in);
        eo_apply<n, 1>(tab, in, out);
#pragma unroll
        for (int y = 0; y < n; ++y)
          lds_add(reinterpret_cast<double *>(reinterpret_cast<char *>(ua) + ixb(IXc, x + n * y)), (double)out[y]);
        hookC(n + x);
      }
    }
    WaveSync::sync();
    STAMP(4);

    if (HN && hn_ncopy) {
      double Wr[n2];
#pragma unroll
      for (int i = 0; i < n2; ++i) Wr[i] = Wl[i];
      hn_pass(2, true, Wr);
      WaveSync::sync();
      hn_pass(1, true, Wr);
      WaveSync::sync();
      hn_pass(0, true, Wr);
      WaveSync::sync();
      double cv[CR > 0 ? CR : 1];
#pragma unroll
      for (int r = 0; r < CR; ++r) cv[r] = (uint32_t)(r * 64 + lane) < hn_ncopy ? ua[Hc[r] >> 16] : 0.0;
#pragma unroll
      for (int r = 0; r < CR; ++r)
        if ((uint32_t)(r * 64 + lane) < hn_ncopy) lds_add(ua + (Hc[r] & 0xffffu), cv[r]);
      WaveSync::sync();
    }
#pragma unroll
    for (int j = 0; j < KGU; ++j) R[j] = (T)ua[lane + j * 64];
    WaveSync::sync();
    STAMP(5);
    stage_src(Gn, SVn);
    STAMP(6);
    bp = b;
    if (SH) Mp = Mc;
#pragma unroll
    for (int j = 0; j < KGU; ++j) Gp[j] = Gc[j];
    STAMP(7);
    RSTAMP(9);
    if (!has_next) break;
    WaveSync::sync();
    b = b1;
    b1 = b2;
    b2 = next_of(b2);
    if (SH) {
      Mc = M1;
      M1 = M2;
      M2 = meta_of(Mv);
    }
#pragma unroll
    for (int j = 0; j < KGU; ++j) {
      Gc[j] = Gn[j];
      Gn[j] = Gnn[j];
    }
#pragma unroll
    for (int w = 0; w < NIW; ++w) IXc[w] = lane_on ? IXn[w] : kDummyIx;
    if (HN) {
#pragma unroll
      for (int w = 0; w < HROWS; ++w) Hc[w] = Hn[w];
    }
  }
  if (ADD) {
#pragma unroll
    for (int j = 0; j < JI; ++j) old[j] = *dst_at(Mp.base, Gp[j]);
  }
#pragma unroll
  for (int j = 0; j < KGU; ++j) scatter_slot(j, bp, Mp.base, Gp[j], R[j], old[j]);
}

template <int n, typename T>
static size_t p_lds_bytes(bool hn) {
  return ((size_t)p_kgu(n) * 64 + (hn ? (size_t)p_priv_max(n) + n * n : 0)) * sizeof(double) +
         (size_t)2 * (p_cells_per_wave(n) + 1) * p_cell_stride(n) * sizeof(T);
}

template <typename T>
hipError_t p_bind(int, int n, bool hn, bool, bool sh, bool mass, uint32_t, CellKernel<T> *k) {
  return dispatch_instantiation(n, [&](auto N, auto HN, auto SH, auto MASS) {
    constexpr int n_ = N;
    if constexpr (kernel_exists(PlaneKernel::planes3, n_, number_type_of<T>, HN, SH, MASS))
      return bind_cell_kernel<T, 64, apply_planes3<n_, T, false, HN, SH, MASS>, apply_planes3<n_, T, true, HN, SH, MASS>,
                              make_tables_eo<T, n_>>(p_lds_bytes<n_, T>(HN), k);
    else
      return hipErrorInvalidValue;
  }, hn, sh, mass);
}
template hipError_t p_bind<double>(int, int, bool, bool, bool, bool, uint32_t, CellKernel<double> *);
template hipError_t p_bind<float>(int, int, bool, bool, bool, bool, uint32_t, CellKernel<float> *);

template <typename T>
__global__ void relayout_coef_kernel(T *out, const T *in, const uint32_t *cell_batch, const uint32_t *cell_pos,
                                     size_t total, int n) {
  const size_t i = (size_t)blockIdx.x * blockDim.x + threadIdx.x;
  if (i >= total) return;
  const int n2 = n * n, nd = n2 * n, NT = (64 / n) * n;
  const size_t cell = i / nd;
  const int q = (int)(i - cell * nd);
  const int x = q % n, r = q / n;
  out[((size_t)cell_batch[cell] * n2 + r) * NT + cell_pos[cell] * n + x] = in[i];
}

template <typename T>
hipError_t relayout_coef_launch(T *out, const T *in, const uint32_t *cell_batch, const uint32_t *cell_pos,
                                size_t total, int n, hipStream_t st) {
  if (total == 0) return hipSuccess;
  hipLaunchKernelGGL(relayout_coef_kernel<T>, dim3((unsigned)((total + 255) / 256)), dim3(256), 0, st, out, in,
                     cell_batch, cell_pos, total, n);
  return hipGetLastError();
}
template hipError_t relayout_coef_launch<double>(double *, const double *, const uint32_t *, const uint32_t *, size_t,
                                                 int, hipStream_t);
template hipError_t relayout_coef_launch<float>(float *, const float *, const uint32_t *, const uint32_t *, size_t, int,
                                                hipStream_t);

}
```

### dealii-cuda_amd/csrc/mfgpu_pass2.hip

```cpp
#include <hip/hip_runtime.h>

#include <algorithm>

#include "mfgpu_kernels.h"

namespace mfgpu {

namespace {

template <typename T>
struct GroupHalos {
  size_t stride;
  const T *h[kMaxFusedWidth];
};
template <typename T, typename P>
__device__ __forceinline__ P *vec_at(const T *, P *p, int) { return p; }
template <typename T, typename P>
__device__ __forceinline__ P *vec_at(const GroupHalos<T> &g, P *p, int v) { return p + (size_t)v * g.stride; }
template <typename T>
__device__ __forceinline__ const T *vec_halo(const T *halo, int) { return halo; }
template <typename T>
__device__ __forceinline__ const T *vec_halo(const GroupHalos<T> &g, int v) { return g.h[v]; }

template <typename T, int NV>
using HalosArg = std::conditional_t<NV == 1, const T *__restrict__, GroupHalos<T>>;

template <typename T, int K, int NV>
__device__ __forceinline__ void reduce_two(T *__restrict__ dst0, const T *__restrict__ src0, const HalosArg<T, NV> halos,
                                           const uint32_t *__restrict__ p, uint32_t cnt, uint32_t i0, uint32_t k,
                                           int add) {
  const uint32_t i1 = i0 + 256u;
  const uint32_t d0 = p[i0], d1 = p[i1];
  constexpr int KU = K > 0 ? K : 1;
  uint32_t s0[KU], s1[KU];
#pragma unroll
  for (int t = 0; t < KU; ++t) {
    s0[t] = p[(size_t)(1 + t) * cnt + i0];
    s1[t] = p[(size_t)(1 + t) * cnt + i1];
  }
  const bool on0 = d0 != 0xffffffffu, on1 = d1 != 0xffffffffu;
  const uint32_t g0 = d0 & 0x7fffffffu, g1 = d1 & 0x7fffffffu;
#pragma unroll
  for (int iv = 0; iv < NV; ++iv) {
    const int v = NV == 1 ? 0 : iv;
    const T *__restrict__ halo = vec_halo(halos, v);
    const T *__restrict__ src = vec_at(halos, src0, v);
    T *__restrict__ dst = vec_at(halos, dst0, v);
    T v0 = T(0), v1 = T(0), o0 = T(0), o1 = T(0);
    if (on0) {
      if (d0 >> 31) {
        v0 = src[g0];
      } else {
        T q[KU];
#pragma unroll
        for (int t = 0; t < KU; ++t) q[t] = halo[s0[t]];
        v0 = q[0];
#pragma unroll
        for (int t = 1; t < KU; ++t) v0 += q[t];
        if (K == 0)
          for (uint32_t t = 1; t < k; ++t) v0 += halo[p[(size_t)(1 + t) * cnt + i0]];
      }
      if (add) o0 = dst[g0];
    }
    if (on1) {
      if (d1 >> 31) {
        v1 = src[g1];
      } else {
        T q[KU];
#pragma unroll
        for (int t = 0; t < KU; ++t) q[t] = halo[s1[t]];
        v1 = q[0];
#pragma unroll
        for (int t = 1; t < KU; ++t) v1 += q[t];
        if (K == 0)
          for (uint32_t t = 1; t < k; ++t) v1 += halo[p[(size_t)(1 + t) * cnt + i1]];
      }
      if (add) o1 = dst[g1];
    }
    if (on0) dst[g0] = add ? o0 + v0 : v0;
    if (on1) dst[g1] = add ? o1 + v1 : v1;
    if (NV == 1) break;
  }
}

template <typename T, int NV>
__global__ void __launch_bounds__(256)
reduce_classes(T *__restrict__ dst, const T *__restrict__ src, const HalosArg<T, NV> halos,
               const uint32_t *__restrict__ arr, const uint4 *__restrict__ tiles, int add) {
  const uint4 td = tiles[blockIdx.x];
  const uint32_t *p = arr + td.x;
  const uint32_t i0 = td.w + threadIdx.x;
  switch (td.y) {
    case 1: reduce_two<T, 1, NV>(dst, src, halos, p, td.z, i0, 1, add); break;
    case 2: reduce_two<T, 2, NV>(dst, src, halos, p, td.z, i0, 2, add); break;
    case 3: reduce_two<T, 3, NV>(dst, src, halos, p, td.z, i0, 3, add); break;
    case 4: reduce_two<T, 4, NV>(dst, src, halos, p, td.z, i0, 4, add); break;
    case 8: reduce_two<T, 8, NV>(dst, src, halos, p, td.z, i0, 8, add); break;
    default: reduce_two<T, 0, NV>(dst, src, halos, p, td.z, i0, td.y, add); break;
  }
}

template <typename T, int K>
__device__ __forceinline__ void reduce_owned(T *__restrict__ dst, const T *__restrict__ src,
                                             const T *__restrict__ halo, const uint32_t *__restrict__ r, uint32_t e,
                                             uint32_t d, uint32_t kk, uint32_t kw, uint32_t hslot0, uint32_t hstride,
                                             int add) {
  const T *const hb = halo + hslot0;
  auto partial = [&](uint32_t w) -> T {
    return hb[(w >> kP2SlotBits) * hstride + (w & ((1u << kP2SlotBits) - 1u))];
  };
  constexpr int KU = K > 0 ? K : 1;
  uint32_t w[KU];
#pragma unroll
  for (int t = 0; t < KU; ++t) w[t] = (uint32_t)t < kk ? r[r[3 + t] + e] : 0u;
  if (d == 0xffffffffu) return;
  T v;
  if (d >> 31) {
    v = src[d & 0x7fffffffu];
  } else {
    T q[KU];
#pragma unroll
    for (int t = 0; t < KU; ++t) q[t] = (uint32_t)t < kk ? partial(w[t]) : T(0);
    v = q[0];
#pragma unroll
    for (int t = 1; t < KU; ++t)
      if ((uint32_t)t < kk) v += q[t];
    if (K == 0)
      for (uint32_t t = 1; t < kw; ++t)
        if (t < kk) v += partial(r[r[3 + t] + e]);
  }
  T *const out = dst + (d & 0x7fffffffu);
  *out = add ? *out + v : v;
}

template <typename T>
__global__ void __launch_bounds__(256)
reduce_owner_batches(T *__restrict__ dst, const T *__restrict__ src, const T *__restrict__ halo,
                     const uint32_t *__restrict__ rec, const uint2 *__restrict__ tab, uint32_t n_batches,
                     uint32_t hstride, int reverse, int add) {
  const uint32_t ob = reverse ? n_batches - 1u - blockIdx.x : blockIdx.x;
  const uint2 t = tab[ob];
  const uint32_t *const r = rec + t.y;
  const uint32_t e0 = r[1];
  dst += t.x;
  src += t.x;
  for (uint32_t e = threadIdx.x; e < e0; e += 256u) {
    const uint32_t d = r[kP2Header + e], kk = r[kP2Header + e0 + e];
    const uint32_t kw = (uint32_t)__builtin_amdgcn_readfirstlane((int)kk);
    const uint32_t h0 = ob * hstride;
    switch (kw) {
      case 0: break;
      case 1: reduce_owned<T, 1>(dst, src, halo, r, e, d, kk, kw, h0, hstride, add); break;
      case 2: reduce_owned<T, 2>(dst, src, halo, r, e, d, kk, kw, h0, hstride, add); break;
      case 3: reduce_owned<T, 3>(dst, src, halo, r, e, d, kk, kw, h0, hstride, add); break;
      case 4: reduce_owned<T, 4>(dst, src, halo, r, e, d, kk, kw, h0, hstride, add); break;
      case 5: case 6: case 7:
      case 8: reduce_owned<T, 8>(dst, src, halo, r, e, d, kk, kw, h0, hstride, add); break;
      default: reduce_owned<T, 0>(dst, src, halo, r, e, d, kk, kw, h0, hstride, add); break;
    }
  }
}

}

void build_pass2_classes(const std::vector<uint32_t> &sdofs, const std::vector<uint32_t> &s_off,
                         const std::vector<uint32_t> &s_idx, std::vector<uint32_t> &arr, std::vector<uint32_t> &tiles) {
  arr.clear();
  tiles.clear();
  const size_t ns = sdofs.size();
  uint32_t kmax = 0;
  for (size_t i = 0; i < ns; ++i) kmax = std::max(kmax, s_off[i + 1] - s_off[i]);
  std::vector<std::vector<uint32_t>> members(kmax + 1);
  for (size_t i = 0; i < ns; ++i) {
    uint32_t k = s_off[i + 1] - s_off[i];
    if (k == 0) k = 1;
    members[k].push_back((uint32_t)i);
  }
  for (uint32_t k = 1; k <= kmax; ++k) {
    const std::vector<uint32_t> &m = members[k];
    if (m.empty()) continue;
    const uint32_t entries = (uint32_t)((m.size() + 511) / 512 * 512);
    const uint32_t base = (uint32_t)arr.size();
    arr.resize(arr.size() + (size_t)(1 + k) * entries, 0u);
    for (uint32_t e = 0; e < entries; ++e) arr[base + e] = e < m.size() ? sdofs[m[e]] : 0xffffffffu;
    for (size_t e = 0; e < m.size(); ++e) {
      const uint32_t i = m[e], cnt = s_off[i + 1] - s_off[i];
      for (uint32_t t = 0; t < k; ++t) arr[base + (size_t)(1 + t) * entries + e] = t < cnt ? s_idx[s_off[i] + t] : 0u;
    }
    for (uint32_t first = 0; first < entries; first += 512) {
      tiles.push_back(base);
      tiles.push_back(k);
      tiles.push_back(entries);
      tiles.push_back(first);
    }
  }
}

template <typename T>
hipError_t reduce_classes_launch(T *dst, const T *src, const T *halo, const uint32_t *arr, const uint32_t *tiles,
                                 uint32_t n_tiles, int add, hipStream_t st) {
  if (n_tiles == 0) return hipSuccess;
  hipLaunchKernelGGL((reduce_classes<T, 1>), dim3(n_tiles), dim3(256), 0, st, dst, src, halo, arr,
                     reinterpret_cast<const uint4 *>(tiles), add);
  return hipGetLastError();
}
template <typename T>
hipError_t reduce_classes_multi_launch(int nv, T *dst, const T *src, size_t stride, T *const *halos, const uint32_t *arr,
                                       const uint32_t *tiles, uint32_t n_tiles, int add, hipStream_t st) {
  if (n_tiles == 0) return hipSuccess;
  if (nv != 2 && nv != 3) return hipErrorInvalidValue;
  GroupHalos<T> gh;
  gh.stride = stride;
  for (int v = 0; v < kMaxFusedWidth; ++v) gh.h[v] = v < nv ? halos[v] : nullptr;
  const uint4 *t4 = reinterpret_cast<const uint4 *>(tiles);
  if (nv == 2)
    hipLaunchKernelGGL((reduce_classes<T, 2>), dim3(n_tiles), dim3(256), 0, st, dst, src, gh, arr, t4, add);
  else
    hipLaunchKernelGGL((reduce_classes<T, 3>), dim3(n_tiles), dim3(256), 0, st, dst, src, gh, arr, t4, add);
  return hipGetLastError();
}
template hipError_t reduce_classes_multi_launch<double>(int, double *, const double *, size_t, double *const *,
                                                        const uint32_t *, const uint32_t *, uint32_t, int, hipStream_t);
template hipError_t reduce_classes_multi_launch<float>(int, float *, const float *, size_t, float *const *,
                                                       const uint32_t *, const uint32_t *, uint32_t, int, hipStream_t);
template <typename T>
hipError_t reduce_owner_batches_launch(T *dst, const T *src, const T *halo, const uint32_t *rec, const uint32_t *tab,
                                       uint32_t n_batches, uint32_t hstride, int reverse, int add, hipStream_t st) {
  if (n_batches == 0) return hipSuccess;
  hipLaunchKernelGGL(reduce_owner_batches<T>, dim3(n_batches), dim3(256), 0, st, dst, src, halo, rec,
                     reinterpret_cast<const uint2 *>(tab), n_batches, hstride, reverse, add);
  return hipGetLastError();
}
template hipError_t reduce_owner_batches_launch<double>(double *, const double *, const double *, const uint32_t *,
                                                        const uint32_t *, uint32_t, uint32_t, int, int, hipStream_t);
template hipError_t reduce_owner_batches_launch<float>(float *, const float *, const float *, const uint32_t *,
                                                       const uint32_t *, uint32_t, uint32_t, int, int, hipStream_t);
template hipError_t reduce_classes_launch<double>(double *, const double *, const double *, const uint32_t *,
                                                  const uint32_t *, uint32_t, int, hipStream_t);
template hipError_t reduce_classes_launch<float>(float *, const float *, const float *, const uint32_t *,
                                                 const uint32_t *, uint32_t, int, hipStream_t);

}
```

### dealii-cuda_amd/csrc/mfgpu_plan.cpp

```cpp
#include <algorithm>
#include <cassert>
#include <cmath>
#include <cstring>
#include <numeric>
#include <unordered_map>

#include "mfgpu_internal.h"

namespace mfgpu {

static thread_local std::string g_err;
void set_error(const std::string &msg) { g_err = msg; }
const char *last_error() { return g_err.c_str(); }

int derive_tables(int n, const double *sv, const double *sg, std::vector<double> &S,
                  std::vector<double> &Dt) {
  std::vector<long double> A(n * n), B(n * n);
  for (int i = 0; i < n * n; ++i) {
    A[i] = sv[i];
    B[i] = sg[i];
  }
  for (int c = 0; c < n; ++c) {
    int piv = c;
    for (int r = c + 1; r < n; ++r)
// ... 610 lines not shown
  P.halo_off.assign(1, 0);
  for (uint32_t k = 0; k < nb; ++k) {
    const uint32_t b = order[k];
    const std::vector<uint32_t> &v = C.bd[b];
    P.batch_nint.push_back(C.nint[b]);
    P.halo_off.push_back(P.halo_off.back() +
                         (R.in_planes(B.masked[b]) ? R.halo_stride : (uint32_t)(v.size() - C.nint[b])));
    for (uint32_t g : v) {
      uint8_t f = 0;
      if (m.constrained[g]) f |= kFlagConstrained;
      if (touched[g]) {
        f |= kFlagAdd;
        ++P.n_add;
      } else {
        touched[g] = 1;
        ++P.n_first;
      }
      P.bdofs.push_back(m.flagged(g));
      P.bflags.push_back(f);
    }
    for (size_t t = 0; t < v.size(); ++t) pos_in_batch[v[t]] = (uint16_t)t;
    for (uint32_t c : B.cells[b]) {
      const size_t pos = P.cell_order.size();
      P.cell_order.push_back(c);
      for (uint32_t i = 0; i < m.nd; ++i) P.lmap[pos * m.nd + i] = pos_in_batch[m.dofs_of(c)[i]];
    }
    P.batch_cell_off.push_back((uint32_t)P.cell_order.size());
    P.batch_dof_off.push_back((uint32_t)P.bdofs.size());
    P.max_batch_dofs = std::max<uint32_t>(P.max_batch_dofs, (uint32_t)v.size());
    P.max_batch_cells = std::max<uint32_t>(P.max_batch_cells, (uint32_t)B.cells[b].size());
  }
  P.orphans.clear();
  for (uint32_t g = 0; g < m.N; ++g)
    if (!touched[g]) P.orphans.push_back(m.flagged(g));
}

void count_plane_batches(Plan &P, const BatchRules &R, const std::vector<uint8_t> &batch_masked) {
  P.n_plane_batches = P.n_plain_plane_batches = 0;
  for (const uint8_t cls : batch_masked)
    if (R.in_planes(cls)) {
      ++P.n_plane_batches;
      P.n_plain_plane_batches += cls ? 0u : 1u;
    }
  if (P.n_plain_plane_batches < P.n_plane_batches) P.n_plain_plane_batches = 0;
}

void emit_pass2_csr(Plan &P, const Description &m, const std::vector<uint32_t> &ntouch, const SharedGroups &G) {
  const size_t ns = G.ids.size(), nb = P.batch_nint.size();
  P.sdofs.resize(ns);
  for (size_t i = 0; i < ns; ++i) P.sdofs[i] = m.flagged(G.ids[G.sorder[i]]);
  P.s_off.assign(ns + 1, 0);
  for (size_t i = 0; i < ns; ++i) P.s_off[i + 1] = P.s_off[i] + ntouch[P.sdofs[i] & 0x7fffffffu];
  P.s_idx.assign(P.s_off[ns], 0);
  std::vector<uint32_t> fill(P.s_off.begin(), P.s_off.end() - 1);
  for (size_t k = 0; k < nb; ++k) {
    const uint32_t ni = P.batch_nint[k];
    const uint32_t d0 = P.batch_dof_off[k], d1 = P.batch_dof_off[k + 1];
    for (uint32_t t = d0 + ni; t < d1; ++t) {
      const uint32_t g = P.bdofs[t] & 0x7fffffffu;
      P.s_idx[fill[G.spos[g]]++] = P.halo_off[k] + (t - d0 - ni);
    }
  }
}

void emit_pass2_groups(Plan &P, const SharedGroups &G) {
  const size_t ns = G.ids.size();
  P.chunks.clear();
  P.gstarts.clear();
  for (size_t i = 0; i < ns;) {
    size_t j = i + 1;
    while (j < ns && G.same_group(G.sorder[i], G.sorder[j])) ++j;
    const uint32_t k = P.s_off[i + 1] - P.s_off[i], tstart = (uint32_t)P.gstarts.size();
    for (uint32_t t = 0; t < k; ++t) P.gstarts.push_back(P.s_idx[P.s_off[i] + t]);
    for (size_t o = i; o < j; o += 64) {
      const uint32_t cnt = (uint32_t)std::min<size_t>(64, j - o);
      P.chunks.push_back((uint32_t)o);
      P.chunks.push_back(cnt | (k << 16));
      P.chunks.push_back(tstart);
      P.chunks.push_back((uint32_t)(o - i));
    }
    i = j;
  }
}
}

int build_plan(const mfgpu_desc &d, Plan &P, uint32_t max_chunks, const PlanLimits *limits) {
  int rc;
  Description m;
  if ((rc = check_description(d, m))) return rc;
  P.dim = d.dim;
  P.degree = d.degree;
  P.n = m.n;
  P.nd = (int)m.nd;
  P.n_dofs = d.n_dofs;
  P.n_cells = d.n_cells;
  BatchRules R;
  if ((rc = resolve_batch_rules(d, max_chunks, limits, R))) return rc;
  const Incidence inc = dof_cell_incidence(m);
  Batches B = make_batches(m, inc, R);
  if (R.segregate && !R.in_planes(true)) plane_batches_first(B);
  if ((d.flags & MFGPU_HANGING_NODES) && d.constraint_mask) masked_cells_first(B, d.constraint_mask);
  Classified C;
  if ((rc = classify_dofs(m, R, B, C))) return rc;
  std::vector<uint32_t> order;
  if ((rc = colour_and_order(C.bd, m.N, (d.flags & MFGPU_COLORED_SCATTER) != 0, order, P.color_batch_off))) return rc;
  const SharedGroups G = group_shared_dofs(C, order, m.N);
  emit_batches(P, m, R, B, C, order);
  count_plane_batches(P, R, B.masked);
  emit_pass2_csr(P, m, C.ntouch, G);
  emit_pass2_groups(P, G);
  return 0;
}

int build_plane_records(Plan &P, const uint32_t *constraint_mask) {
  const int n = P.n, n2 = n * n, NT = p_cells_per_wave(n) * n, NIW = (n2 + 1) / 2;
  const int JI = p_ji(n) * 64, NB = p_kgu(n) * 64;
  const size_t nbat = P.n_plane_batches;
  const uint32_t dummy = 8u * (uint32_t)(NB - 1);
  std::vector<uint32_t> &bd = P.pr_dofs, &ix = P.pr_idx;
  bd.assign((size_t)NB * nbat, 0u);
  ix.assign((size_t)NIW * NT * nbat, dummy | (dummy << 16));
  std::vector<uint32_t> slot_of;
  const int HROWS = p_hn_rows(n), CR = p_priv_max(n) / 64;
  std::vector<uint32_t> &hnrec = P.pr_hn;
  hnrec.clear();
  P.pr_hn_slot.assign(nbat, 0xffffffffu);
  std::vector<HnLine> lines[3];
  std::vector<uint16_t> pnodes;
  std::vector<uint32_t> priv_pos((size_t)P.nd);
  for (size_t b = 0; b < nbat; ++b) {
    const uint32_t c0 = P.batch_cell_off[b], nc = P.batch_cell_off[b + 1] - c0;
    const uint32_t d0 = P.batch_dof_off[b], nbd = P.batch_dof_off[b + 1] - d0, ni = P.batch_nint[b];
    if ((int)nc * n > NT || (int)ni > JI || (int)(nbd - ni) >= NB - JI || nbd == ni) {
      set_error("internal: batch does not fit the plane kernel's dof-list slots");
      return MFGPU_EINVAL;
    }
    slot_of.assign(nbd, 0u);
    for (uint32_t t = 0; t < nbd; ++t) slot_of[t] = t < ni ? t : (uint32_t)JI + (t - ni);
    for (int t = 0; t < NB; ++t) {
      uint32_t src_t;
      if (t < JI) src_t = (uint32_t)t < ni ? (uint32_t)t : ni;
      else src_t = std::min<uint32_t>(ni + (uint32_t)(t - JI), nbd - 1);
      bd[b * NB + t] = P.bdofs[d0 + src_t];
    }
    bool hnb = false;
    if (constraint_mask && b >= P.n_plain_plane_batches)
      for (uint32_t c = 0; c < nc; ++c) hnb = hnb || constraint_mask[P.cell_order[c0 + c]] != 0;
    uint32_t next_priv = (uint32_t)NB;
    std::vector<uint32_t> copies, ops_d[3];
    for (uint32_t c = 0; c < nc; ++c) {
      const unsigned mask = hnb ? constraint_mask[P.cell_order[c0 + c]] : 0u;
      std::fill(priv_pos.begin(), priv_pos.end(), 0xffffffffu);
      if (mask) {
        hn_cell_lines(mask, n, lines, pnodes);
        for (uint16_t node : pnodes) {
          if (next_priv >= (uint32_t)NB + (uint32_t)p_priv_max(n)) {
            set_error("internal: batch exceeds the plane kernel's private hanging-node entries");
            return MFGPU_EINVAL;
          }
          priv_pos[node] = next_priv;
          copies.push_back((next_priv << 16) | slot_of[P.lmap[(size_t)(c0 + c) * P.nd + node]]);
          ++next_priv;
        }
        for (int dir = 0; dir < 3; ++dir)
          for (const HnLine &L : lines[dir]) {
            uint32_t w[3] = {0u, 0u, 0u};
            for (int t = 0; t < n; ++t) w[t >> 1] |= priv_pos[L.node[t]] << (16 * (t & 1));
            ops_d[dir].insert(ops_d[dir].end(), w, w + 3);
          }
      }
      for (int k = 0; k < n; ++k)
        for (int i = 0; i < n2; ++i) {
          const int node = i + n2 * k;
          const uint32_t pos = priv_pos[node] != 0xffffffffu ? priv_pos[node] : slot_of[P.lmap[(size_t)(c0 + c) * P.nd + node]];
          const uint32_t off = 8u * pos;
          uint32_t &w = ix[(b * NIW + i / 2) * NT + c * n + k];
          w = (i & 1) ? ((w & 0xffffu) | (off << 16)) : ((w & 0xffff0000u) | off);
        }
    }
    if (hnb) {
      P.pr_hn_slot[b] = (uint32_t)(hnrec.size() / ((size_t)HROWS * 64));
      hnrec.resize(hnrec.size() + (size_t)HROWS * 64, 0u);
      uint32_t *rec = hnrec.data() + (size_t)P.pr_hn_slot[b] * HROWS * 64;
      for (size_t e = 0; e < copies.size(); ++e) rec[e] = copies[e];
      for (int dir = 0; dir < 3; ++dir) {
        const size_t nops = ops_d[dir].size() / 3;
        if (nops > (size_t)kHnOpRounds * 64) {
          set_error("internal: more hanging-node lines in a batch than the plane kernel's record holds");
          return MFGPU_EINVAL;
        }
        for (size_t e = 0; e < nops; ++e)
          for (int w = 0; w < 3; ++w)
            rec[(size_t)(CR + (dir * kHnOpRounds + (int)(e / 64)) * 3 + w) * 64 + e % 64] = ops_d[dir][e * 3 + w];
      }
      const uint32_t h0 = (uint32_t)copies.size() | ((uint32_t)(ops_d[0].size() / 3) << 16);
      const uint32_t h1 = (uint32_t)(ops_d[1].size() / 3) | ((uint32_t)(ops_d[2].size() / 3) << 16);
      for (int l = 0; l < 64; ++l) {
        rec[(size_t)(HROWS - 2) * 64 + l] = h0;
        rec[(size_t)(HROWS - 1) * 64 + l] = h1;
      }
    }
  }
  share_plane_records(P);
  share_pass2_records(P);
  return 0;
}

namespace {
uint64_t hash_words(const uint32_t *w, size_t n) {
  uint64_t h = 1469598103934665603ull;
  for (size_t i = 0; i < n; ++i) h = (h ^ w[i]) * 1099511628211ull;
  return h;
}

using SeenRecords = std::unordered_multimap<uint64_t, std::pair<size_t, size_t>>;
size_t intern_record(std::vector<uint32_t> &table, SeenRecords &seen, const uint32_t *rec, size_t len) {
  const uint64_t h = hash_words(rec, len);
  const auto range = seen.equal_range(h);
  for (auto it = range.first; it != range.second; ++it)
    if (it->second.second == len && !std::memcmp(table.data() + it->second.first, rec, len * sizeof(uint32_t)))
      return it->second.first;
  const size_t off = table.size();
  table.insert(table.end(), rec, rec + len);
  seen.emplace(h, std::make_pair(off, len));
  return off;
}
}

void share_plane_records(Plan &P) {
  const int n = P.n, NT = p_cells_per_wave(n) * n, NIW = (n * n + 1) / 2;
  const size_t NB = (size_t)p_kgu(n) * 64, NX = (size_t)NIW * NT, nbat = P.n_plane_batches;
  P.sh_dofs.clear();
  P.sh_idx.clear();
  P.sh_batch.assign(nbat * kShBatchWords, 0u);
  SeenRecords seen_d, seen_x;
  std::vector<uint32_t> rel(NB);
  for (size_t b = 0; b < nbat; ++b) {
    const uint32_t *g = P.pr_dofs.data() + b * NB;
    uint32_t base = 0x7fffffffu;
    for (size_t t = 0; t < NB; ++t) base = std::min(base, g[t] & 0x7fffffffu);
    for (size_t t = 0; t < NB; ++t) rel[t] = g[t] - base;
    uint32_t *e = P.sh_batch.data() + b * kShBatchWords;
    e[0] = base;
    e[1] = (uint32_t)(intern_record(P.sh_dofs, seen_d, rel.data(), NB) / NB);
    e[2] = (uint32_t)(intern_record(P.sh_idx, seen_x, P.pr_idx.data() + b * NX, NX) / NX);
  }
  const size_t shared = P.sh_dofs.size() + P.sh_idx.size() + P.sh_batch.size();
  const size_t expanded = P.pr_dofs.size() + P.pr_idx.size();
  P.sh_use = nbat > 0 && P.pr_hn.empty() && (double)shared <= kShareMaxFraction * (double)expanded;
}

void share_pass2_records(Plan &P) {
  P.sh_p2rec.clear();
  P.sh_p2tab.clear();
  P.sh_p2_use = false;
  const size_t nb = P.batch_cell_off.size() - 1;
  const uint32_t hs = (uint32_t)p_hs(P.n) * 64u;
  if (nb == 0 || P.n_plane_batches != nb || P.halo_off.size() != nb + 1 || hs > (1u << kP2SlotBits)) return;
  for (size_t b = 0; b <= nb; ++b)
    if (P.halo_off[b] != (uint64_t)b * hs) return;
  std::vector<std::vector<uint32_t>> owned(nb);
  size_t expanded = 0;
  for (size_t i = 0; i < P.sdofs.size(); ++i) {
    const uint32_t k = P.s_off[i + 1] - P.s_off[i];
    expanded += 1 + (k ? k : 1);
    if (k == 0) continue;
    if (k > (uint32_t)kP2MaxK) return;
    const uint32_t owner = P.s_idx[P.s_off[i]] / hs;
    for (uint32_t t = 0; t < k; ++t) {
      const uint32_t tb = P.s_idx[P.s_off[i] + t] / hs;
      if (tb >= nb || tb < owner || tb - owner >= (1u << (32 - kP2SlotBits))) return;
    }
    owned[owner].push_back((uint32_t)i);
  }
  P.sh_p2tab.assign(2 * nb, 0u);
  SeenRecords seen;
  std::vector<uint32_t> rec;
  for (size_t b = 0; b < nb; ++b) {
    std::vector<uint32_t> &m = owned[b];
    auto k_of = [&](uint32_t i) { return P.s_off[i + 1] - P.s_off[i]; };
    std::stable_sort(m.begin(), m.end(), [&](uint32_t x, uint32_t y) { return k_of(x) > k_of(y); });
    const uint32_t base = P.sh_batch[b * kShBatchWords], ne = (uint32_t)m.size(), kmax = ne ? k_of(m[0]) : 0u;
    auto pad = [](uint32_t x) { return (x + 63u) & ~63u; };
    const uint32_t e0 = pad(ne);
    rec.assign(kP2Header, 0u);
    rec[0] = ne;
    rec[1] = e0;
    rec[2] = kmax;
    rec.resize(kP2Header + 2 * (size_t)e0, 0u);
    for (uint32_t e = 0; e < e0; ++e) rec[kP2Header + e] = e < ne ? P.sdofs[m[e]] - base : 0xffffffffu;
    for (uint32_t e = 0; e < ne; ++e) rec[kP2Header + e0 + e] = k_of(m[e]);
    for (uint32_t t = 0; t < kmax; ++t) {
      uint32_t cnt = 0;
      while (cnt < ne && k_of(m[cnt]) > t) ++cnt;
      rec[3 + t] = (uint32_t)rec.size();
      rec.resize(rec.size() + pad(cnt), 0u);
      for (uint32_t e = 0; e < cnt; ++e) {
        const uint32_t slot = P.s_idx[P.s_off[m[e]] + t], tb = slot / hs;
        rec[rec[3 + t] + e] = ((tb - (uint32_t)b) << kP2SlotBits) | (slot - tb * hs);
      }
    }
    P.sh_p2tab[2 * b] = base;
    P.sh_p2tab[2 * b + 1] = (uint32_t)intern_record(P.sh_p2rec, seen, rec.data(), rec.size());
  }
  const size_t shared = P.sh_p2rec.size() + P.sh_p2tab.size();
  P.sh_p2_use = (double)shared <= kShareMaxFraction * (double)expanded;
}

int choose_kernel_and_plan(const mfgpu_desc &d, PlaneKernel &pk, BatchKernel &bk, Plan &plan) {
  const bool general = !(d.flags & MFGPU_UNIFORM_J0), hn = (d.flags & MFGPU_HANGING_NODES) != 0;
  const bool colored = (d.flags & MFGPU_COLORED_SCATTER) != 0;
  if (d.kernel > MFGPU_KERNEL_PLANES_2W) {
    set_error("unknown mfgpu_desc.kernel");
    return MFGPU_EINVAL;
  }
  const bool pk_ok = d.dim == 3 && !general && !colored && d.degree >= 2 && d.degree <= 6 &&
                     d.n_dofs < (1u << 29);
  const bool xk_ok = d.dim == 3 && !general && !colored;
  const bool want_planes = d.kernel == MFGPU_KERNEL_PLANES || d.kernel == MFGPU_KERNEL_PLANES_2W;
  if ((want_planes && !pk_ok) || (d.kernel == MFGPU_KERNEL_PENCILS_X && !xk_ok) ||
      (d.kernel == MFGPU_KERNEL_PENCILS && general)) {
    set_error("mfgpu_desc.kernel: this kernel family does not cover the description (see include/mfgpu.h)");
    return MFGPU_EUNSUPPORTED;
  }
  const bool planes4 = d.kernel == MFGPU_KERNEL_PLANES_2W || d.degree >= 5 ||
                       (d.kernel == MFGPU_KERNEL_AUTO && d.degree == 3 && d.number_type == MFGPU_F64);
  const PlaneKernel plane_kind = planes4 ? PlaneKernel::planes4 : PlaneKernel::planes3;
  const bool mass = d.mass_coefficient != nullptr;
  auto plane_kernel_exists = [&](bool with_hn) {
    return kernel_exists(plane_kind, d.degree + 1, d.number_type, with_hn, false, mass);
  };
  const bool mass_without_planes = mass && pk_ok && !plane_kernel_exists(false);
  if (mass_without_planes && want_planes) {
    set_error("mfgpu_desc.kernel: this plane kernel has no mass-term instantiation at this degree (apply_planes4w at "
              "p = 5, 6; apply_planes4 at p = 4 in double); use MFGPU_KERNEL_AUTO or MFGPU_KERNEL_PENCILS_X");
    return MFGPU_EUNSUPPORTED;
  }
  bool planes = pk_ok && !mass_without_planes && (want_planes || (d.kernel == MFGPU_KERNEL_AUTO &&
                                     (d.degree >= 4 || (d.degree == 3 && (hn || d.number_type == MFGPU_F64)))));
  bool pencils_x = xk_ok && !planes && d.kernel != MFGPU_KERNEL_PENCILS;
  PlanLimits lim;
  if (planes) {
    lim.max_cells = (uint32_t)p_cells_per_wave(d.degree + 1);
    lim.max_dofs = (uint32_t)p_kgu(d.degree + 1) * 64u - 1u;
    lim.interior_max = (uint32_t)p_ji(d.degree + 1) * 64u;
    lim.halo_stride = (uint32_t)p_hs(d.degree + 1) * 64u;
    lim.shared_max = lim.halo_stride - 1u;
    lim.segregate_masked = hn;
    lim.masked_planes = hn && plane_kernel_exists(true);
    lim.private_max = (uint32_t)p_priv_max(d.degree + 1);
  }
  int rc = build_plan(d, plan, (pencils_x && d.degree == 3) ? 4u : 3u, planes ? &lim : nullptr);
  if (rc == MFGPU_EUNSUPPORTED && planes && d.kernel == MFGPU_KERNEL_AUTO && xk_ok) {
    planes = false;
    pencils_x = true;
    plan = Plan();
    rc = build_plan(d, plan, d.degree == 3 ? 4u : 3u, nullptr);
  }
  if (!rc && planes) {
    const uint32_t nbat = (uint32_t)plan.batch_cell_off.size() - 1;
    pencils_x = plan.n_plane_batches < nbat;
    if (plan.n_plane_batches == 0) planes = false;
  }
  pk = planes ? plane_kind : PlaneKernel::none;
  bk = pencils_x ? BatchKernel::x : general ? (d.dim == 2 ? BatchKernel::g2 : BatchKernel::g)
                                   : planes ? BatchKernel::none : BatchKernel::batches;
  assert(rc || (pk != PlaneKernel::none) == (plan.n_plane_batches > 0));
  return rc;
}

}

namespace mfgpu {
std::vector<uint32_t> multi_groups(uint32_t n_vectors, const std::vector<uint32_t> &widths) {
  std::vector<uint32_t> groups;
  uint32_t left = n_vectors;
  for (uint32_t w : widths)
    for (; w > 1 && left >= w; left -= w) groups.push_back(w);
  groups.insert(groups.end(), left, 1u);
  return groups;
}

std::vector<uint16_t> x_lane_permutation(int n) {
  const int n2 = n * n, PP = n2, CH = 256 / PP, ndl = n2 * n;
  std::vector<uint16_t> perm(512, 0xffff);
  for (int layout = 0; layout < 2; ++layout) {
    uint16_t *lanes = perm.data() + 256 * layout;
    std::vector<int> fill(32, 0), overflow;
    for (int q = 0; q < CH * PP; ++q) {
      const int cell = q / PP, pen = q % PP, a = pen % n, b = pen / n;
      const int base = cell * ndl + (layout == 0 ? a + n2 * b : a + n * b);
      const int r = base & 31;
      if (fill[r] < 8) lanes[32 * fill[r]++ + r] = (uint16_t)q;
      else overflow.push_back(q);
    }
    for (int l = 255; l >= 0 && !overflow.empty(); --l)
      if (lanes[l] == 0xffff) {
        lanes[l] = (uint16_t)overflow.back();
        overflow.pop_back();
      }
  }
  return perm;
}

std::vector<uint16_t> x_pencil_runs(const std::vector<uint16_t> &lmap, int n_) {
  const size_t n = (size_t)n_, np = (n + 1) & ~(size_t)1, runs = lmap.size() / n;
  std::vector<uint16_t> lx(runs * np, 0);
  for (size_t r = 0; r < runs; ++r)
    for (size_t i = 0; i < n; ++i) lx[r * np + i] = lmap[r * n + i];
  return lx;
}

int pass2_groups(const Plan &P, const std::vector<uint32_t> &seg_end, const uint32_t *priority, uint32_t n_priority,
                 bool shared, std::vector<Pass2Group> &groups) {
  std::vector<uint8_t> prio(P.n_dofs, 0);
  for (uint32_t i = 0; i < n_priority; ++i) {
    if (priority[i] >= P.n_dofs) {
      set_error("priority dof out of range");
      return MFGPU_EINVAL;
    }
    prio[priority[i]] = 1;
  }
  groups.assign(1 + seg_end.size(), Pass2Group());
  auto add = [&](uint32_t dof, const uint32_t *slots, uint32_t k, size_t seg) {
    Pass2Group &g = groups[prio[dof & 0x7fffffffu] ? 0 : 1 + seg];
    g.dofs.push_back(dof);
    g.slots.insert(g.slots.end(), slots, slots + k);
    g.offsets.push_back((uint32_t)g.slots.size());
  };
  for (size_t i = 0; i < P.sdofs.size(); ++i) {
    size_t seg = 0;
    if (shared && P.s_off[i + 1] > P.s_off[i]) continue;
    if (P.s_off[i + 1] > P.s_off[i]) {
      const uint32_t slot = P.s_idx[P.s_off[i + 1] - 1];
      const uint32_t batch = (uint32_t)(std::upper_bound(P.halo_off.begin(), P.halo_off.end(), slot) - P.halo_off.begin()) - 1;
      seg = (size_t)(std::upper_bound(seg_end.begin(), seg_end.end(), batch) - seg_end.begin());
      if (seg >= seg_end.size()) seg = seg_end.size() - 1;
    }
    add(P.sdofs[i], P.s_idx.data() + P.s_off[i], P.s_off[i + 1] - P.s_off[i], seg);
  }
  const uint32_t zero_slot = P.halo_off.empty() ? 0u : P.halo_off.back();
  for (uint32_t orph : P.orphans) add(orph, &zero_slot, 1, 0);
  return 0;
}
}

extern "C" {

const char *mfgpu_last_error(void) { return mfgpu::last_error(); }

int mfgpu_plan_create(const mfgpu_desc *desc, mfgpu_plan **out) {
  if (!desc || !out) {
    mfgpu::set_error("null argument");
    return MFGPU_EINVAL;
  }
  mfgpu_plan *p = new mfgpu_plan();
  mfgpu::PlaneKernel pk;
  mfgpu::BatchKernel bk;
  mfgpu_desc d = *desc;
  d.mass_coefficient = nullptr;
  int rc = mfgpu::choose_kernel_and_plan(d, pk, bk, p->plan);
  if (!rc && pk != mfgpu::PlaneKernel::none) rc = mfgpu::build_plane_records(p->plan, desc->constraint_mask);
  if (rc) {
    delete p;
    return rc;
  }
  *out = p;
  return 0;
}

void mfgpu_plan_destroy(mfgpu_plan *p) { delete p; }

size_t mfgpu_desc_size(void) { return sizeof(mfgpu_desc); }

int mfgpu_suggest_renumbering(const mfgpu_desc *desc, uint32_t *new_index) {
  if (!desc || !new_index) {
    mfgpu::set_error("null argument");
    return MFGPU_EINVAL;
  }
  mfgpu::Plan P;
  mfgpu::PlaneKernel pk;
  mfgpu::BatchKernel bk;
  mfgpu_desc d = *desc;
  d.mass_coefficient = nullptr;
  int rc = mfgpu::choose_kernel_and_plan(d, pk, bk, P);
  if (rc) return rc;
  const uint32_t NONE = 0xffffffffu;
  std::fill(new_index, new_index + desc->n_dofs, NONE);
  uint32_t next = 0;
  const size_t nb = P.batch_cell_off.size() - 1;
  for (size_t b = 0; b < nb; ++b) {
    const uint32_t d0 = P.batch_dof_off[b];
    const uint32_t ni = P.batch_nint.empty() ? P.batch_dof_off[b + 1] - d0 : P.batch_nint[b];
    for (uint32_t t = 0; t < ni; ++t) {
      const uint32_t g = P.bdofs[d0 + t] & 0x7fffffffu;
      if (new_index[g] == NONE) new_index[g] = next++;
    }
  }
  for (uint32_t e : P.sdofs) {
    const uint32_t g = e & 0x7fffffffu;
    if (new_index[g] == NONE) new_index[g] = next++;
  }
  for (uint32_t g = 0; g < desc->n_dofs; ++g)
    if (new_index[g] == NONE) new_index[g] = next++;
  if (next != desc->n_dofs) {
    mfgpu::set_error("internal: renumbering is not a permutation");
    return MFGPU_EINVAL;
  }
  return 0;
}

int64_t mfgpu_plan_array_u32(const mfgpu_plan *p, int what, const uint32_t **ptr) {
  if (!p || !ptr) return MFGPU_EINVAL;
  const std::vector<uint32_t> *v = nullptr;
  switch (what) {
    case 0: v = &p->plan.batch_cell_off; break;
    case 1: v = &p->plan.batch_dof_off; break;
    case 2: v = &p->plan.color_batch_off; break;
    case 3: v = &p->plan.cell_order; break;
    case 4: v = &p->plan.bdofs; break;
    case 5: v = &p->plan.orphans; break;
    case 6: v = &p->plan.batch_nint; break;
    case 7: v = &p->plan.halo_off; break;
    case 8: v = &p->plan.sdofs; break;
    case 9: v = &p->plan.s_off; break;
    case 10: v = &p->plan.s_idx; break;
    case 11: v = &p->plan.chunks; break;
    case 12: v = &p->plan.gstarts; break;
    case 13: v = &p->plan.pr_dofs; break;
    case 14: v = &p->plan.pr_idx; break;
    case 15: v = &p->plan.pr_hn; break;
    case 16: v = &p->plan.pr_hn_slot; break;
    case 17: v = &p->plan.sh_dofs; break;
    case 18: v = &p->plan.sh_idx; break;
    case 19: v = &p->plan.sh_batch; break;
    case 20: v = &p->plan.sh_p2rec; break;
    case 21: v = &p->plan.sh_p2tab; break;
    default: mfgpu::set_error("bad array id"); return MFGPU_EINVAL;
  }
  *ptr = v->data();
  return (int64_t)v->size();
}

int mfgpu_plan_multi_groups(uint32_t n_vectors, const uint32_t *widths, uint32_t n_widths, uint32_t *groups,
                            uint32_t capacity) {
  if ((!widths && n_widths) || (!groups && capacity)) return MFGPU_EINVAL;
  const std::vector<uint32_t> g = mfgpu::multi_groups(n_vectors, std::vector<uint32_t>(widths, widths + n_widths));
  for (size_t i = 0; i < g.size() && i < capacity; ++i) groups[i] = g[i];
  return (int)g.size();
}

int mfgpu_plan_shares_records(const mfgpu_plan *p) {
  return p ? (p->plan.sh_use ? 1 : 0) | (p->plan.sh_p2_use ? 2 : 0) : 0;
}

int64_t mfgpu_plan_lmap(const mfgpu_plan *p, const uint16_t **ptr) {
  if (!p || !ptr) return MFGPU_EINVAL;
  *ptr = p->plan.lmap.data();
  return (int64_t)p->plan.lmap.size();
}

int64_t mfgpu_plan_bflags(const mfgpu_plan *p, const uint8_t **ptr) {
  if (!p || !ptr) return MFGPU_EINVAL;
  *ptr = p->plan.bflags.data();
  return (int64_t)p->plan.bflags.size();
}

}
```

### dealii-cuda_amd/pymfgpu/__init__.py

```python
from __future__ import annotations

import ctypes as C
import os

import numpy as np

_HERE = os.path.dirname(os.path.abspath(__file__))
LIB_PATH = os.environ.get("MFGPU_LIB") or os.path.join(os.path.dirname(_HERE), "lib", "libmfgpu.so")

F64, F32 = 0, 1
OK, EINVAL = 0, -1
EUNSUPPORTED = -4
MULTI_ADD, MULTI_LOOP, MULTI_FUSED = 1, 2, 4
UNIFORM_J0, HANGING_NODES, COLORED_SCATTER, NO_SHARED_RECORDS = 1, 2, 1 << 8, 1 << 9
UPDATABLE_COEFFICIENTS = 1 << 10
KERNEL_AUTO, KERNEL_PENCILS, KERNEL_PENCILS_X, KERNEL_PLANES, KERNEL_PLANES_2W = 0, 1, 2, 3, 4


class MfgpuError(RuntimeError):
    pass


class Desc(C.Structure):
    _fields_ = [
        ("dim", C.c_int32), ("degree", C.c_int32), ("number_type", C.c_int32), ("flags", C.c_uint32),
        ("n_dofs", C.c_uint32), ("n_cells", C.c_uint32),
        ("loc2glob", C.c_void_p), ("constraint_mask", C.c_void_p),
        ("JxW", C.c_void_p), ("inv_jac", C.c_void_p), ("coefficient", C.c_void_p),
        ("quadrature_points", C.c_void_p), ("shape_values", C.c_void_p), ("shape_gradients", C.c_void_p),
        ("constraint_weights", C.c_void_p), ("constrained_dofs", C.c_void_p),
        ("n_constrained", C.c_uint32), ("max_cells_per_batch", C.c_uint32), ("max_dofs_per_batch", C.c_uint32),
        ("kernel", C.c_uint32), ("cell_loop_segments", C.c_uint32), ("max_workgroups", C.c_uint32),
        ("mass_coefficient", C.c_void_p),
    ]


CG_NONE, CG_JACOBI, CG_CHEBYSHEV, CG_CALLBACK = 0, 1, 2, 3
CG_STATE_BYTES, CG_PARTIAL_BYTES = 128, 3 * 2048 * 8


class CGInfo(C.Structure):
    _fields_ = [("iterations", C.c_uint32), ("status", C.c_uint32), ("residual", C.c_double),
                ("initial_residual", C.c_double)]

    def as_tuple(self):
        return int(self.iterations), int(self.status), float(self.residual), float(self.initial_residual)


VCYCLE_COARSE_AUTO, VCYCLE_COARSE_DENSE, VCYCLE_COARSE_CG = 0, 1, 2
VCYCLE_DENSE_MAX = 2048
SPD_INVERSE_DEVICE_MAX = 512
EIG_STATE_BYTES, EIG_PARTIAL_BYTES = 64, 2 * 2048 * 8


class EigResult(C.Structure):
    _fields_ = [("lambda_max", C.c_double), ("estimate", C.c_double), ("steps", C.c_uint32), ("status", C.c_uint32)]


class VCycleRefreshInfo(C.Structure):
    _fields_ = [("coarse_status", C.c_uint32), ("eig_status_max", C.c_uint32), ("eig_steps_max", C.c_uint32),
                ("reserved", C.c_uint32)]


class VCycleLevelDesc(C.Structure):
    _fields_ = [("op", C.c_void_p), ("edges", C.c_void_p), ("from_coarser", C.c_void_p), ("to_mg", C.c_void_p),
                ("from_mg", C.c_void_p)]


class VCycleDesc(C.Structure):
    _fields_ = [("n_levels", C.c_uint32), ("levels", C.POINTER(VCycleLevelDesc)), ("active_type", C.c_int32),
                ("n_active", C.c_uint32), ("smoother_degree", C.c_uint32), ("smoothing_range", C.c_double),
                ("eig_iterations", C.c_uint32), ("lambda_max", C.POINTER(C.c_double)), ("coarse", C.c_uint32),
                ("coarse_tolerance", C.c_double), ("coarse_max_iterations", C.c_uint32)]


CG_CALLBACK_TYPE = C.CFUNCTYPE(C.c_int, C.c_void_p, C.c_void_p, C.c_void_p, C.c_void_p)


SYMBOLS = [
    "mfgpu_vmult_multi", "mfgpu_multi_width", "mfgpu_plan_multi_groups",
    "mfgpu_create", "mfgpu_vmult", "mfgpu_vmult_add", "mfgpu_n_dofs", "mfgpu_memory_consumption",
    "mfgpu_destroy", "mfgpu_last_error", "mfgpu_plan_stats", "mfgpu_kernel_name", "mfgpu_compute_inverse_diagonal", "mfgpu_set_constrained_values",
    "mfgpu_vec_sadd", "mfgpu_vec_equ", "mfgpu_vec_scale", "mfgpu_vec_divide", "mfgpu_vec_invert", "mfgpu_vec_mul",
    "mfgpu_vec_dot", "mfgpu_vec_l2_norm", "mfgpu_vec_add_and_dot", "mfgpu_vec_all_zero", "mfgpu_profile_enable", "mfgpu_profile_read", "mfgpu_profile_read_pass2",
    "mfgpu_plan_create", "mfgpu_plan_destroy", "mfgpu_plan_array_u32", "mfgpu_plan_lmap", "mfgpu_plan_bflags",
    "mfgpu_plan_shares_records", "mfgpu_record_stats",
    "mfgpu_vec_alloc", "mfgpu_vec_free", "mfgpu_vec_fill", "mfgpu_vec_from_host", "mfgpu_vec_to_host",
    "mfgpu_device_synchronize", "mfgpu_device_memory_info", "mfgpu_mesh_create_uniform", "mfgpu_mesh_create_adaptive", "mfgpu_mesh_create_ball", "mfgpu_mesh_create_from_leaves",
    "mfgpu_mesh_cell_levels", "mfgpu_mesh_destroy",
    "mfgpu_mesh_desc", "mfgpu_mesh_dof_coords", "mfgpu_mesh_interface_dofs",
    "mfgpu_dist_unique_id", "mfgpu_dist_create", "mfgpu_dist_connect_local", "mfgpu_dist_attach", "mfgpu_dist_schedule",
    "mfgpu_vmult_dist_begin", "mfgpu_vmult_dist_end", "mfgpu_vmult_dist", "mfgpu_dist_destroy",
    "mfgpu_transfer_create", "mfgpu_transfer_create_from_meshes", "mfgpu_transfer_prolongate",
    "mfgpu_transfer_restrict_and_add", "mfgpu_transfer_memory_consumption", "mfgpu_transfer_destroy",
    "mfgpu_mesh_transfer_patches", "mfgpu_suggest_renumbering", "mfgpu_mesh_renumber",
    "mfgpu_level_create", "mfgpu_level_operator", "mfgpu_level_vmult_interface_down", "mfgpu_level_vmult_interface_up",
    "mfgpu_level_destroy", "mfgpu_index_pairs_create", "mfgpu_vec_copy_pairs", "mfgpu_index_pairs_destroy",
    "mfgpu_mesh_create_adaptive_mg", "mfgpu_mg_hierarchy_create", "mfgpu_mg_n_levels", "mfgpu_mg_level_mesh",
    "mfgpu_mg_edge_dofs", "mfgpu_mg_copy_pairs", "mfgpu_mg_transfer_arrays", "mfgpu_mg_hierarchy_destroy",
    "mfgpu_integrator_create", "mfgpu_integrator_rhs", "mfgpu_integrator_l2_error", "mfgpu_integrator_error_points",
    "mfgpu_integrator_destroy",
    "mfgpu_vec_convert", "mfgpu_vec_copy_pairs_convert", "mfgpu_vec_chebyshev_start", "mfgpu_vec_chebyshev_update",
    "mfgpu_desc_size",
    "mfgpu_update_coefficients", "mfgpu_level_update_coefficients", "mfgpu_integrator_update_coefficients",
    "mfgpu_integrator_evaluate",
    "mfgpu_cg_create", "mfgpu_cg_set_callback", "mfgpu_cg_begin", "mfgpu_cg_iterate", "mfgpu_cg_status", "mfgpu_cg_solve",
    "mfgpu_cg_memory_consumption", "mfgpu_cg_destroy", "mfgpu_cg_chebyshev_scalars",
    "mfgpu_cg_begin_relative", "mfgpu_cg_set_vcycle", "mfgpu_transfer_prolongate_add", "mfgpu_vec_residual",
    "mfgpu_vcycle_create", "mfgpu_vcycle_apply", "mfgpu_vcycle_lambda_max", "mfgpu_vcycle_memory_consumption",
    "mfgpu_vcycle_destroy", "mfgpu_estimate_lambda_max", "mfgpu_spd_inverse",
    "mfgpu_vec_chebyshev_start_dev", "mfgpu_vec_chebyshev_update_dev", "mfgpu_cg_chebyshev_scalars_dev",
    "mfgpu_eig_workspace_bytes", "mfgpu_estimate_lambda_max_enqueue", "mfgpu_spd_inverse_workspace_bytes",
    "mfgpu_spd_inverse_enqueue", "mfgpu_vcycle_refresh", "mfgpu_vcycle_refresh_status", "mfgpu_estimate_lambda_max_steps",
    "mfgpu_transfer_create_p", "mfgpu_transfer_create_p_from_meshes", "mfgpu_transfer_p_prolongation_1d",
    "mfgpu_transfer_create_p_hn", "mfgpu_transfer_create_p_hn_from_meshes", "mfgpu_transfer_p_owner_list",
]

_lib = None


def lib():
    global _lib
    if _lib is None:
        if not os.path.exists(LIB_PATH):
            raise MfgpuError(f"{LIB_PATH} not found: build it with __graft_entry__.build() "
                             "(make -C dealii-cuda_amd); there is no fallback path")
        L = C.CDLL(LIB_PATH)
        L.mfgpu_last_error.restype = C.c_char_p
        L.mfgpu_create.argtypes = [C.POINTER(Desc), C.POINTER(C.c_void_p)]
        L.mfgpu_desc_size.argtypes = []
        L.mfgpu_desc_size.restype = C.c_size_t
        L.mfgpu_vmult.argtypes = [C.c_void_p, C.c_void_p, C.c_void_p, C.c_void_p]
        L.mfgpu_vmult_add.argtypes = [C.c_void_p, C.c_void_p, C.c_void_p, C.c_void_p]
        L.mfgpu_n_dofs.argtypes = [C.c_void_p]
        L.mfgpu_n_dofs.restype = C.c_uint32
        L.mfgpu_memory_consumption.argtypes = [C.c_void_p]
        L.mfgpu_memory_consumption.restype = C.c_size_t
        L.mfgpu_destroy.argtypes = [C.c_void_p]
        L.mfgpu_destroy.restype = None
        L.mfgpu_plan_stats.argtypes = [C.c_void_p, C.POINTER(C.c_uint64)]
        L.mfgpu_device_memory_info.argtypes = [C.POINTER(C.c_size_t), C.POINTER(C.c_size_t)]
        L.mfgpu_kernel_name.argtypes = [C.c_void_p]
        L.mfgpu_kernel_name.restype = C.c_char_p
        L.mfgpu_compute_inverse_diagonal.argtypes = [C.c_void_p, C.c_void_p, C.c_void_p]
        L.mfgpu_set_constrained_values.argtypes = [C.c_void_p, C.c_void_p, C.c_double, C.c_void_p]
        vp, d, z, i = C.c_void_p, C.c_double, C.c_size_t, C.c_int
        L.mfgpu_vec_sadd.argtypes = [vp, d, d, vp, z, i, vp]
        L.mfgpu_vec_equ.argtypes = [vp, d, vp, z, i, vp]
        L.mfgpu_vec_scale.argtypes = [vp, vp, z, i, vp]
        L.mfgpu_vec_divide.argtypes = [vp, vp, z, i, vp]
        L.mfgpu_vec_invert.argtypes = [vp, z, i, vp]
        L.mfgpu_vec_mul.argtypes = [vp, d, z, i, vp]
        L.mfgpu_vec_dot.argtypes = [vp, vp, z, i, vp, C.POINTER(d)]
        L.mfgpu_vec_l2_norm.argtypes = [vp, z, i, vp, C.POINTER(d)]
        L.mfgpu_vec_add_and_dot.argtypes = [vp, d, vp, vp, z, i, vp, C.POINTER(d)]
        L.mfgpu_vec_all_zero.argtypes = [vp, z, i, vp, C.POINTER(i)]
        L.mfgpu_profile_enable.argtypes = [C.c_void_p, C.c_int]
        L.mfgpu_profile_read.argtypes = [C.c_void_p, C.POINTER(C.c_double), C.POINTER(C.c_uint64)]
        L.mfgpu_profile_read_pass2.argtypes = [C.c_void_p, C.POINTER(C.c_double)]
        L.mfgpu_plan_create.argtypes = [C.POINTER(Desc), C.POINTER(C.c_void_p)]
        L.mfgpu_plan_destroy.argtypes = [C.c_void_p]
        L.mfgpu_plan_destroy.restype = None
        L.mfgpu_plan_array_u32.argtypes = [C.c_void_p, C.c_int, C.POINTER(C.c_void_p)]
        L.mfgpu_plan_array_u32.restype = C.c_int64
        L.mfgpu_plan_lmap.argtypes = [C.c_void_p, C.POINTER(C.c_void_p)]
        L.mfgpu_plan_lmap.restype = C.c_int64
        L.mfgpu_plan_bflags.argtypes = [C.c_void_p, C.POINTER(C.c_void_p)]
        L.mfgpu_plan_bflags.restype = C.c_int64
        L.mfgpu_plan_shares_records.argtypes = [C.c_void_p]
        L.mfgpu_record_stats.argtypes = [C.c_void_p, C.POINTER(C.c_uint64)]
        L.mfgpu_vec_alloc.argtypes = [C.POINTER(C.c_void_p), C.c_size_t, C.c_int]
        L.mfgpu_vec_free.argtypes = [C.c_void_p]
        L.mfgpu_vec_fill.argtypes = [C.c_void_p, C.c_size_t, C.c_int, C.c_double, C.c_void_p]
        L.mfgpu_vec_from_host.argtypes = [C.c_void_p, C.c_void_p, C.c_size_t, C.c_int]
        L.mfgpu_vec_to_host.argtypes = [C.c_void_p, C.c_void_p, C.c_size_t, C.c_int]
        L.mfgpu_mesh_create_uniform.argtypes = [C.c_int, C.c_int, C.POINTER(C.c_uint32), C.c_double, C.c_double,
                                                C.c_uint32, C.c_uint32, C.c_int, C.POINTER(C.c_void_p)]
        L.mfgpu_mesh_create_adaptive.argtypes = [C.c_int, C.c_int, C.c_int, C.c_int, C.POINTER(C.c_void_p)]
        L.mfgpu_mesh_create_ball.argtypes = [C.c_int, C.c_int, C.c_int, C.c_int, C.POINTER(C.c_void_p)]
        L.mfgpu_mesh_create_from_leaves.argtypes = [C.c_int, C.c_int, C.c_void_p, C.c_uint32, C.c_int, C.POINTER(C.c_void_p)]
        L.mfgpu_mesh_cell_levels.argtypes = [C.c_void_p, C.POINTER(C.c_void_p)]
        L.mfgpu_mesh_cell_levels.restype = C.c_int64
        L.mfgpu_mesh_destroy.argtypes = [C.c_void_p]
        L.mfgpu_mesh_destroy.restype = None
        L.mfgpu_mesh_desc.argtypes = [C.c_void_p, C.POINTER(Desc)]
        L.mfgpu_mesh_dof_coords.argtypes = [C.c_void_p, C.POINTER(C.c_void_p)]
        L.mfgpu_mesh_dof_coords.restype = C.c_int64
        L.mfgpu_mesh_interface_dofs.argtypes = [C.c_void_p, C.c_int, C.POINTER(C.c_void_p)]
        L.mfgpu_mesh_interface_dofs.restype = C.c_int64
        L.mfgpu_transfer_create.argtypes = [C.c_int, C.c_int, C.c_int, C.c_uint32, C.c_void_p, C.c_void_p, C.c_uint32,
                                            C.c_uint32, C.c_void_p, C.c_uint32, C.c_void_p, C.POINTER(C.c_void_p)]
        L.mfgpu_transfer_create_from_meshes.argtypes = [C.c_void_p, C.c_void_p, C.POINTER(C.c_void_p)]
        L.mfgpu_transfer_prolongate.argtypes = [C.c_void_p, C.c_void_p, C.c_void_p, C.c_void_p]
        L.mfgpu_transfer_restrict_and_add.argtypes = [C.c_void_p, C.c_void_p, C.c_void_p, C.c_void_p]
        L.mfgpu_transfer_memory_consumption.argtypes = [C.c_void_p]
        L.mfgpu_transfer_memory_consumption.restype = C.c_size_t
        L.mfgpu_mesh_transfer_patches.argtypes = [C.c_void_p, C.c_void_p, C.c_void_p, C.c_void_p]
        L.mfgpu_mesh_transfer_patches.restype = C.c_int64
        L.mfgpu_suggest_renumbering.argtypes = [C.POINTER(Desc), C.c_void_p]
        L.mfgpu_mesh_renumber.argtypes = [C.c_void_p, C.c_void_p]
        L.mfgpu_level_create.argtypes = [C.POINTER(Desc), C.c_void_p, C.c_uint32, C.POINTER(C.c_void_p)]
        L.mfgpu_level_operator.argtypes = [C.c_void_p]
        L.mfgpu_level_operator.restype = C.c_void_p
        L.mfgpu_level_vmult_interface_down.argtypes = [C.c_void_p, C.c_void_p, C.c_void_p, C.c_void_p]
        L.mfgpu_level_vmult_interface_up.argtypes = [C.c_void_p, C.c_void_p, C.c_void_p, C.c_void_p]
        L.mfgpu_mesh_create_adaptive_mg.argtypes = [C.c_int, C.c_int, C.c_int, C.c_int, C.POINTER(C.c_void_p)]
        L.mfgpu_mg_hierarchy_create.argtypes = [C.c_void_p, C.POINTER(C.c_void_p)]
        L.mfgpu_mg_n_levels.argtypes = [C.c_void_p]
        L.mfgpu_mg_level_mesh.argtypes = [C.c_void_p, C.c_int]
        L.mfgpu_mg_level_mesh.restype = C.c_void_p
        L.mfgpu_mg_edge_dofs.argtypes = [C.c_void_p, C.c_int, C.POINTER(C.c_void_p)]
        L.mfgpu_mg_edge_dofs.restype = C.c_int64
        L.mfgpu_mg_copy_pairs.argtypes = [C.c_void_p, C.c_int, C.POINTER(C.c_void_p), C.POINTER(C.c_void_p)]
        L.mfgpu_mg_copy_pairs.restype = C.c_int64
        L.mfgpu_mg_transfer_arrays.argtypes = [C.c_void_p, C.c_int, C.POINTER(C.c_void_p), C.POINTER(C.c_void_p)]
        L.mfgpu_mg_transfer_arrays.restype = C.c_int64
        L.mfgpu_mg_hierarchy_destroy.argtypes = [C.c_void_p]
        L.mfgpu_mg_hierarchy_destroy.restype = None
        L.mfgpu_index_pairs_create.argtypes = [C.c_void_p, C.c_void_p, C.c_uint32, C.POINTER(C.c_void_p)]
        L.mfgpu_vec_copy_pairs.argtypes = [C.c_void_p, C.c_void_p, C.c_void_p, C.c_int, C.c_void_p]
        L.mfgpu_index_pairs_destroy.argtypes = [C.c_void_p]
        L.mfgpu_index_pairs_destroy.restype = None
        L.mfgpu_level_destroy.argtypes = [C.c_void_p]
        L.mfgpu_level_destroy.restype = None
        L.mfgpu_transfer_destroy.argtypes = [C.c_void_p]
        L.mfgpu_transfer_destroy.restype = None
        L.mfgpu_integrator_create.argtypes = [C.POINTER(Desc), C.POINTER(C.c_void_p)]
        L.mfgpu_integrator_rhs.argtypes = [C.c_void_p, C.c_void_p, C.c_void_p, C.c_void_p, C.c_void_p]
        L.mfgpu_integrator_l2_error.argtypes = [C.c_void_p, C.c_void_p, C.c_void_p, C.c_void_p, C.c_void_p,
                                                C.POINTER(C.c_double)]
        L.mfgpu_integrator_error_points.argtypes = [C.c_void_p, C.c_void_p, C.c_void_p]
        L.mfgpu_integrator_destroy.argtypes = [C.c_void_p]
        L.mfgpu_integrator_destroy.restype = None
        L.mfgpu_vec_convert.argtypes = [vp, i, vp, i, z, vp]
        L.mfgpu_update_coefficients.argtypes = [vp, vp, vp, vp]
        L.mfgpu_level_update_coefficients.argtypes = [vp, vp, vp, vp]
        L.mfgpu_integrator_update_coefficients.argtypes = [vp, vp, vp, vp]
        L.mfgpu_integrator_evaluate.argtypes = [vp, vp, vp, vp, vp]
        L.mfgpu_vec_copy_pairs_convert.argtypes = [vp, vp, i, vp, i, vp]
        L.mfgpu_vec_chebyshev_start.argtypes = [vp, vp, vp, vp, vp, vp, d, i, z, i, vp]
        L.mfgpu_vec_chebyshev_update.argtypes = [vp, vp, vp, vp, vp, d, d, z, i, vp]
        L.mfgpu_vmult_multi.argtypes = [vp, vp, vp, C.c_uint32, z, C.c_uint32, vp]
        L.mfgpu_multi_width.argtypes = [vp]
        L.mfgpu_plan_multi_groups.argtypes = [C.c_uint32, C.POINTER(C.c_uint32), C.c_uint32, C.POINTER(C.c_uint32),
                                              C.c_uint32]
        u32 = C.c_uint32
        L.mfgpu_cg_create.argtypes = [vp, i, vp, u32, d, d, C.POINTER(vp)]
        L.mfgpu_cg_set_callback.argtypes = [vp, CG_CALLBACK_TYPE, vp]
        L.mfgpu_cg_begin.argtypes = [vp, vp, vp, d, u32, vp]
        L.mfgpu_cg_iterate.argtypes = [vp, u32, vp]
        L.mfgpu_cg_status.argtypes = [vp, vp, C.POINTER(CGInfo)]
        L.mfgpu_cg_solve.argtypes = [vp, vp, vp, d, u32, u32, vp, C.POINTER(CGInfo)]
        L.mfgpu_cg_memory_consumption.argtypes = [vp]
# ... 185 lines not shown
    def ptr(a, dtype):
        if a is None:
            return None
        a = np.ascontiguousarray(a, dtype=dtype)
        keep.append(a)
        return a.ctypes.data

    d = Desc()
    d.dim, d.degree, d.number_type = dim, degree, number_type
    l2g = np.ascontiguousarray(loc2glob, dtype=np.uint32)
    d.n_dofs = int(n_dofs)
    d.n_cells = l2g.size // ((degree + 1) ** dim)
    uniform = np.asarray(inv_jac).size == d.n_cells
    assert uniform or np.asarray(inv_jac).size == l2g.size * dim * dim
    d.flags = ((UNIFORM_J0 if uniform else 0) | (HANGING_NODES if constraint_mask is not None else 0)
               | (COLORED_SCATTER if colored else 0))
    d.loc2glob = ptr(l2g, np.uint32)
    d.constraint_mask = ptr(constraint_mask, np.uint32)
    d.JxW = ptr(JxW, dt)
    d.inv_jac = ptr(inv_jac, dt)
    d.coefficient = ptr(coefficient, dt)
    d.quadrature_points = ptr(quadrature_points, dt)
    d.shape_values = ptr(shape_values, dt)
    d.shape_gradients = ptr(shape_gradients, dt)
    d.constraint_weights = ptr(constraint_weights, np.float64)
    c = np.ascontiguousarray(constrained, dtype=np.uint32)
    d.constrained_dofs = ptr(c, np.uint32)
    d.n_constrained = c.size
    d.max_cells_per_batch = max_cells_per_batch
    d.max_dofs_per_batch = max_dofs_per_batch
    d.kernel = kernel
    d.cell_loop_segments = cell_loop_segments
    d.max_workgroups = max_workgroups
    d.mass_coefficient = ptr(mass_coefficient, dt)
    return d, keep


class Plan:

    def __init__(self, desc: Desc, keep=None):
        self._keep = keep
        self.nd = (desc.degree + 1) ** desc.dim
        h = C.c_void_p()
        _check(lib().mfgpu_plan_create(C.byref(desc), C.byref(h)))
        self._h = h

    def __del__(self):
        if getattr(self, "_h", None) and _lib is not None:
            _lib.mfgpu_plan_destroy(self._h)
            self._h = None

    def _u32(self, what):
        p = C.c_void_p()
        cnt = lib().mfgpu_plan_array_u32(self._h, what, C.byref(p))
        if cnt < 0:
            _check(int(cnt))
        return _view(p.value, cnt, np.uint32).copy()

    batch_cell_off = property(lambda s: s._u32(0))
    batch_dof_off = property(lambda s: s._u32(1))
    color_batch_off = property(lambda s: s._u32(2))
    cell_order = property(lambda s: s._u32(3))
    bdofs = property(lambda s: s._u32(4) & np.uint32(0x7fffffff))
    bdofs_constrained = property(lambda s: (s._u32(4) >> np.uint32(31)).astype(bool))
    orphans = property(lambda s: s._u32(5))
    batch_nint = property(lambda s: s._u32(6))
    halo_off = property(lambda s: s._u32(7))
    sdofs = property(lambda s: s._u32(8))
    s_off = property(lambda s: s._u32(9))
    s_idx = property(lambda s: s._u32(10))
    chunks = property(lambda s: s._u32(11).reshape(-1, 4))
    gstarts = property(lambda s: s._u32(12))
    pr_dofs = property(lambda s: s._u32(13))
    pr_idx = property(lambda s: s._u32(14))
    pr_hn = property(lambda s: s._u32(15))
    pr_hn_slot = property(lambda s: s._u32(16))
    sh_dofs = property(lambda s: s._u32(17))
    sh_idx = property(lambda s: s._u32(18))
    sh_batch = property(lambda s: s._u32(19).reshape(-1, 4))
    shares_records = property(lambda s: bool(lib().mfgpu_plan_shares_records(s._h) & 1))
    sh_p2rec = property(lambda s: s._u32(20))
    sh_p2tab = property(lambda s: s._u32(21).reshape(-1, 2))
    shares_pass2_records = property(lambda s: bool(lib().mfgpu_plan_shares_records(s._h) & 2))

    @property
    def lmap(self):
        p = C.c_void_p()
        cnt = lib().mfgpu_plan_lmap(self._h, C.byref(p))
        return _view(p.value, cnt, np.uint16).reshape(-1, self.nd).copy()

    @property
    def bflags(self):
        p = C.c_void_p()
        cnt = lib().mfgpu_plan_bflags(self._h, C.byref(p))
        return _view(p.value, cnt, np.uint8).copy()


class DeviceVector:

    def __init__(self, n, number_type=F64):
        self.n, self.number_type = int(n), number_type
        p = C.c_void_p()
        _check(lib().mfgpu_vec_alloc(C.byref(p), self.n, number_type))
        self.ptr = p.value

    @classmethod
    def view(cls, ptr, n, number_type=F64):
        v = cls.__new__(cls)
        v.n, v.number_type, v.ptr, v._borrowed = int(n), number_type, int(ptr), True
        return v

    def __del__(self):
        if getattr(self, "ptr", None) and _lib is not None and not getattr(self, "_borrowed", False):
            _lib.mfgpu_vec_free(self.ptr)
            self.ptr = None

    def fill(self, value, stream=None):
        _check(lib().mfgpu_vec_fill(self.ptr, self.n, self.number_type, float(value), stream))

    def from_host(self, a):
        a = np.ascontiguousarray(a, dtype=np_dtype(self.number_type))
        assert a.size == self.n
        _check(lib().mfgpu_vec_from_host(self.ptr, a.ctypes.data, self.n, self.number_type))

    def to_host(self):
        a = np.empty(self.n, dtype=np_dtype(self.number_type))
        _check(lib().mfgpu_vec_to_host(a.ctypes.data, self.ptr, self.n, self.number_type))
        return a

    def swap(self, other):
        self.ptr, other.ptr = other.ptr, self.ptr
        self.n, other.n = other.n, self.n

    def _a(self, other=None):
        if other is not None:
            assert other.n == self.n and other.number_type == self.number_type
        return self.n, self.number_type

    def sadd(self, s, a, w, stream=None):
        _check(lib().mfgpu_vec_sadd(self.ptr, float(s), float(a), w.ptr, *self._a(w), stream))

    def add(self, a, w, stream=None):
        self.sadd(1.0, a, w, stream)

    def equ(self, a, w, stream=None):
        _check(lib().mfgpu_vec_equ(self.ptr, float(a), w.ptr, *self._a(w), stream))

    def scale(self, w, stream=None):
        _check(lib().mfgpu_vec_scale(self.ptr, w.ptr, *self._a(w), stream))

    def divide(self, w, stream=None):
        _check(lib().mfgpu_vec_divide(self.ptr, w.ptr, *self._a(w), stream))

    def invert(self, stream=None):
        _check(lib().mfgpu_vec_invert(self.ptr, *self._a(), stream))

    def mul(self, a, stream=None):
        _check(lib().mfgpu_vec_mul(self.ptr, float(a), *self._a(), stream))

    def dot(self, w, stream=None):
        r = C.c_double()
        _check(lib().mfgpu_vec_dot(self.ptr, w.ptr, *self._a(w), stream, C.byref(r)))
        return r.value

    def l2_norm(self, stream=None):
        r = C.c_double()
        _check(lib().mfgpu_vec_l2_norm(self.ptr, *self._a(), stream, C.byref(r)))
        return r.value

    def add_and_dot(self, a, x, w, stream=None):
        r = C.c_double()
        self._a(x)
        _check(lib().mfgpu_vec_add_and_dot(self.ptr, float(a), x.ptr, w.ptr, *self._a(w), stream, C.byref(r)))
        return r.value

    def all_zero(self, stream=None):
        r = C.c_int()
        _check(lib().mfgpu_vec_all_zero(self.ptr, *self._a(), stream, C.byref(r)))
        return bool(r.value)


class Operator:

    def __init__(self, desc: Desc, keep=None):
        self._keep = keep
        self.number_type = desc.number_type
        h = C.c_void_p()
        _check(lib().mfgpu_create(C.byref(desc), C.byref(h)))
        self._h = h

    def __del__(self):
        self.clear()

    def clear(self):
        if getattr(self, "_h", None) and _lib is not None:
            _lib.mfgpu_destroy(self._h)
            self._h = None

    def n(self):
        return int(lib().mfgpu_n_dofs(self._h))

    m = n

    def vmult(self, dst, src, stream=None):
        _check(lib().mfgpu_vmult(self._h, _ptr(dst), _ptr(src), stream))

    def vmult_add(self, dst, src, stream=None):
        _check(lib().mfgpu_vmult_add(self._h, _ptr(dst), _ptr(src), stream))

    def vmult_multi(self, dst, src, n_vectors, stride=None, add=False, mode=None, stream=None):
        flags = (MULTI_ADD if add else 0) | (mode or 0)
        _check(lib().mfgpu_vmult_multi(self._h, _ptr(dst), _ptr(src), int(n_vectors),
                                       self.n() if stride is None else int(stride), flags, stream))

    def multi_width(self):
        return int(lib().mfgpu_multi_width(self._h))

    def memory_consumption(self):
        return int(lib().mfgpu_memory_consumption(self._h))

    def plan_stats(self):
        s = (C.c_uint64 * 8)()
        _check(lib().mfgpu_plan_stats(self._h, s))
        keys = ["n_batches", "n_launches", "batch_dofs", "max_batch_dofs", "max_batch_cells", "n_orphans",
                "first_touch_or_shared_dofs", "rmw_adds_or_halo_slots"]
        out = dict(zip(keys, [int(v) for v in s]))
        r = (C.c_uint64 * 4)()
        _check(lib().mfgpu_record_stats(self._h, r))
        out.update(index_records="shared" if r[0] & 1 else "expanded",
                   pass2_records="shared" if r[0] & 2 else "expanded", distinct_dof_records=int(r[1]),
                   distinct_index_records=int(r[2]), index_record_bytes=int(r[3]))
        return out

    def kernel_name(self):
        return lib().mfgpu_kernel_name(self._h).decode()

    def compute_inverse_diagonal(self, inv_diag, stream=None):
        _check(lib().mfgpu_compute_inverse_diagonal(self._h, _ptr(inv_diag), stream))

    def set_constrained_values(self, vec, value, stream=None):
        _check(lib().mfgpu_set_constrained_values(self._h, _ptr(vec), float(value), stream))

    def update_coefficients(self, coef=None, mass=None, stream=None):
        _check(lib().mfgpu_update_coefficients(self._h, _optr(coef), _optr(mass), stream))

    def profile_enable(self, on=True):
        _check(lib().mfgpu_profile_enable(self._h, int(on)))

    def profile_read(self):
        ms, nv = C.c_double(), C.c_uint64()
        _check(lib().mfgpu_profile_read(self._h, C.byref(ms), C.byref(nv)))
        return ms.value, int(nv.value)

    def profile_read_pass2(self):
        ms = C.c_double()
        _check(lib().mfgpu_profile_read_pass2(self._h, C.byref(ms)))
        return ms.value


def cg_chebyshev_scalars(degree, lambda_max, smoothing_range):
    out = (C.c_double * max(2 * int(degree) - 1, 1))()
    _check(lib().mfgpu_cg_chebyshev_scalars(int(degree), float(lambda_max), float(smoothing_range), out))
    return np.array(out[:2 * int(degree) - 1], dtype=np.float64)


class CG:

    def __init__(self, op: "Operator", preconditioner=CG_NONE, inv_diag=None, degree=0, lambda_max=0.0,
                 smoothing_range=0.0, callback=None):
        self._op, self._inv_diag = op, inv_diag
        self._cb = self._cb_error = None
        self.n, self.number_type = op.n(), op.number_type
        h = C.c_void_p()
        _check(lib().mfgpu_cg_create(op._h, int(preconditioner), _optr(inv_diag), int(degree), float(lambda_max),
                                     float(smoothing_range), C.byref(h)))
        self._h = h
        if callback is not None:
            self.set_callback(callback)

    def set_callback(self, callback):
        def trampoline(_ctx, z, r, stream):
            try:
                rc = callback(DeviceVector.view(z, self.n, self.number_type),
                              DeviceVector.view(r, self.n, self.number_type), stream)
                return 0 if rc is None else int(rc)
            except Exception as e:
                self._cb_error = e
                return EINVAL

        cb = CG_CALLBACK_TYPE(trampoline)
        _check(lib().mfgpu_cg_set_callback(self._h, cb, None))
        self._cb = cb

    def _done(self, rc, check):
        e, self._cb_error = self._cb_error, None
        if e is not None:
            raise e
        return _check(rc) if check else rc

    def destroy(self):
        if getattr(self, "_h", None) and _lib is not None:
            _lib.mfgpu_cg_destroy(self._h)
            self._h = None

    __del__ = destroy

    def begin(self, x, b, tolerance, max_iterations, stream=None, check=True):
        return self._done(lib().mfgpu_cg_begin(self._h, _optr(x), _optr(b), float(tolerance), int(max_iterations), stream),
                          check)

    def begin_relative(self, x, b, relative_tolerance, max_iterations, stream=None, check=True):
        return self._done(lib().mfgpu_cg_begin_relative(self._h, _optr(x), _optr(b), float(relative_tolerance),
                                                        int(max_iterations), stream), check)

# ... 577 lines not shown
```

### include/mfgpu.h

```cpp
#ifndef MFGPU_H
#define MFGPU_H

#include <stddef.h>
#include <stdint.h>

#ifdef __cplusplus
extern "C" {
#endif

#define MFGPU_OK 0
#define MFGPU_EINVAL (-1)
#define MFGPU_EHIP (-2)
#define MFGPU_ENOMEM (-3)
#define MFGPU_EUNSUPPORTED (-4)

#define MFGPU_F64 0
#define MFGPU_F32 1

#define MFGPU_UNIFORM_J0 (1u << 0)
#define MFGPU_HANGING_NODES (1u << 1)

#define MFGPU_COLORED_SCATTER (1u << 8)

#define MFGPU_NO_SHARED_RECORDS (1u << 9)

#define MFGPU_UPDATABLE_COEFFICIENTS (1u << 10)

typedef struct mfgpu_handle mfgpu_handle;

typedef struct mfgpu_desc {
  int32_t dim;
  int32_t degree;
  int32_t number_type;
  uint32_t flags;
  uint32_t n_dofs;
  uint32_t n_cells;
  const uint32_t *loc2glob;
  const uint32_t *constraint_mask;
  const void *JxW;
  const void *inv_jac;
  const void *coefficient;
  const void *quadrature_points;
  const void *shape_values;
  const void *shape_gradients;
  const double *constraint_weights;
  const uint32_t *constrained_dofs;
  uint32_t n_constrained;
  uint32_t max_cells_per_batch;
  uint32_t max_dofs_per_batch;
  uint32_t kernel;
  uint32_t cell_loop_segments;
  uint32_t max_workgroups;
  const void *mass_coefficient;
} mfgpu_desc;

size_t mfgpu_desc_size(void);

#define MFGPU_KERNEL_AUTO 0
#define MFGPU_KERNEL_PENCILS 1
#define MFGPU_KERNEL_PENCILS_X 2
#define MFGPU_KERNEL_PLANES 3
#define MFGPU_KERNEL_PLANES_2W 4


int mfgpu_create(const mfgpu_desc *desc, mfgpu_handle **out);

int mfgpu_vmult(mfgpu_handle *h, void *dst_dev, const void *src_dev, void *stream);

int mfgpu_vmult_add(mfgpu_handle *h, void *dst_dev, const void *src_dev, void *stream);

#define MFGPU_MULTI_ADD   (1u << 0)
#define MFGPU_MULTI_LOOP  (1u << 1)
#define MFGPU_MULTI_FUSED (1u << 2)

int mfgpu_vmult_multi(mfgpu_handle *h, void *dst_dev, const void *src_dev, uint32_t n_vectors, size_t stride,
                      uint32_t flags, void *stream);
int mfgpu_multi_width(const mfgpu_handle *h);

int mfgpu_update_coefficients(mfgpu_handle *h, const void *coefficient_dev, const void *mass_coefficient_dev,
                              void *stream);

uint32_t mfgpu_n_dofs(const mfgpu_handle *h);

size_t mfgpu_memory_consumption(const mfgpu_handle *h);

void mfgpu_destroy(mfgpu_handle *h);

const char *mfgpu_last_error(void);

int mfgpu_plan_stats(const mfgpu_handle *h, uint64_t stats[8]);

int mfgpu_record_stats(const mfgpu_handle *h, uint64_t stats[4]);

const char *mfgpu_kernel_name(const mfgpu_handle *h);

int mfgpu_profile_enable(mfgpu_handle *h, int on);
int mfgpu_profile_read(mfgpu_handle *h, double *kernel_ms_total, uint64_t *n_vmults);
int mfgpu_profile_read_pass2(mfgpu_handle *h, double *pass2_ms_total);

typedef struct mfgpu_plan mfgpu_plan;
int mfgpu_plan_create(const mfgpu_desc *desc, mfgpu_plan **out);
void mfgpu_plan_destroy(mfgpu_plan *p);
int64_t mfgpu_plan_array_u32(const mfgpu_plan *p, int what, const uint32_t **ptr);
int mfgpu_plan_shares_records(const mfgpu_plan *p);
int mfgpu_plan_multi_groups(uint32_t n_vectors, const uint32_t *widths, uint32_t n_widths, uint32_t *groups,
                            uint32_t capacity);
int64_t mfgpu_plan_lmap(const mfgpu_plan *p, const uint16_t **ptr);
int64_t mfgpu_plan_bflags(const mfgpu_plan *p, const uint8_t **ptr);

int mfgpu_suggest_renumbering(const mfgpu_desc *desc, uint32_t *new_index );

int mfgpu_compute_inverse_diagonal(mfgpu_handle *h, void *inv_diag, void *stream);
int mfgpu_set_constrained_values(mfgpu_handle *h, void *vec, double value, void *stream);

int mfgpu_vec_sadd(void *v, double s, double a, const void *w, size_t n, int number_type, void *stream);
int mfgpu_vec_equ(void *v, double a, const void *w, size_t n, int number_type, void *stream);
int mfgpu_vec_scale(void *v, const void *w, size_t n, int number_type, void *stream);
int mfgpu_vec_divide(void *v, const void *w, size_t n, int number_type, void *stream);
int mfgpu_vec_invert(void *v, size_t n, int number_type, void *stream);
int mfgpu_vec_mul(void *v, double a, size_t n, int number_type, void *stream);
int mfgpu_vec_dot(const void *v, const void *w, size_t n, int number_type, void *stream, double *result);
int mfgpu_vec_l2_norm(const void *v, size_t n, int number_type, void *stream, double *result);
int mfgpu_vec_add_and_dot(void *v, double a, const void *x, const void *w, size_t n, int number_type,
                          void *stream, double *result);
int mfgpu_vec_all_zero(const void *v, size_t n, int number_type, void *stream, int *result);

int mfgpu_vec_alloc(void **dev, size_t n, int number_type);
int mfgpu_vec_free(void *dev);
int mfgpu_vec_fill(void *dev, size_t n, int number_type, double value, void *stream);
int mfgpu_vec_from_host(void *dev, const void *host, size_t n, int number_type);
int mfgpu_vec_to_host(void *host, const void *dev, size_t n, int number_type);
int mfgpu_device_synchronize(void);
int mfgpu_device_memory_info(size_t *free_bytes, size_t *total_bytes);

typedef struct mfgpu_dist mfgpu_dist;
int mfgpu_dist_unique_id(void *id128);
int mfgpu_dist_create(const void *id128, int rank, int world, const uint32_t *lower_ids, uint32_t n_lower,
                      const uint32_t *upper_ids, uint32_t n_upper, const uint32_t *constrained_dofs,
                      uint32_t n_constrained, uint32_t n_dofs, int number_type, mfgpu_dist **out);
int mfgpu_dist_connect_local(mfgpu_dist *lower_rank, mfgpu_dist *upper_rank);
int mfgpu_dist_attach(mfgpu_dist *d, mfgpu_handle *h);
int mfgpu_dist_schedule(const mfgpu_dist *d, uint32_t info[4]);
int mfgpu_vmult_dist_begin(mfgpu_handle *h, mfgpu_dist *d, void *dst_dev, const void *src_dev, void *stream);
int mfgpu_vmult_dist_end(mfgpu_handle *h, mfgpu_dist *d, void *dst_dev, void *stream);
int mfgpu_vmult_dist(mfgpu_handle *h, mfgpu_dist *d, void *dst_dev, const void *src_dev, void *stream);
void mfgpu_dist_destroy(mfgpu_dist *d);

typedef struct mfgpu_transfer mfgpu_transfer;
int mfgpu_transfer_create(int dim, int degree, int number_type, uint32_t n_coarse_cells,
                          const uint32_t *coarse_cell_dofs ,
                          const uint32_t *fine_patch_dofs  , uint32_t n_coarse_dofs,
                          uint32_t n_fine_dofs, const uint32_t *coarse_dirichlet, uint32_t n_coarse_dirichlet,
                          const double *prolongation_1d ,
                          mfgpu_transfer **out);
int mfgpu_transfer_prolongate(mfgpu_transfer *t, void *dst_fine_dev, const void *src_coarse_dev, void *stream);
int mfgpu_transfer_restrict_and_add(mfgpu_transfer *t, void *dst_coarse_dev, const void *src_fine_dev, void *stream);
int mfgpu_transfer_prolongate_add(mfgpu_transfer *t, void *dst_fine_dev, const void *src_coarse_dev, void *stream);
size_t mfgpu_transfer_memory_consumption(const mfgpu_transfer *t);
void mfgpu_transfer_destroy(mfgpu_transfer *t);

int mfgpu_transfer_create_p(int dim, int degree_coarse, int degree_fine, int number_type, uint32_t n_cells,
                            const uint32_t *coarse_cell_dofs ,
                            const uint32_t *fine_cell_dofs , uint32_t n_coarse_dofs,
                            uint32_t n_fine_dofs, const uint32_t *coarse_dirichlet, uint32_t n_coarse_dirichlet,
                            const double *prolongation_1d ,
                            mfgpu_transfer **out);
int mfgpu_transfer_p_prolongation_1d(int degree_coarse, int degree_fine, double *p1);
int mfgpu_transfer_create_p_hn(int dim, int degree_coarse, int degree_fine, int number_type, uint32_t n_cells,
                               const uint32_t *coarse_cell_dofs ,
                               const uint32_t *fine_cell_dofs , uint32_t n_coarse_dofs,
                               uint32_t n_fine_dofs, const uint32_t *coarse_dirichlet, uint32_t n_coarse_dirichlet,
                               const double *prolongation_1d ,
                               const uint32_t *constraint_mask ,
                               const double *coarse_constraint_weights , mfgpu_transfer **out);
int mfgpu_transfer_p_owner_list(int dim, int degree_fine, uint32_t n_cells, const uint32_t *fine_cell_dofs,
                                const uint32_t *constraint_mask , uint32_t n_fine_dofs,
                                uint32_t *out );

typedef struct mfgpu_level mfgpu_level;
int mfgpu_level_create(const mfgpu_desc *desc, const uint32_t *edge_dofs, uint32_t n_edge, mfgpu_level **out);
mfgpu_handle *mfgpu_level_operator(mfgpu_level *level);
int mfgpu_level_vmult_interface_down(mfgpu_level *level, void *dst_dev, const void *src_dev, void *stream);
int mfgpu_level_vmult_interface_up(mfgpu_level *level, void *dst_dev, const void *src_dev, void *stream);
int mfgpu_level_update_coefficients(mfgpu_level *level, const void *coefficient_dev, const void *mass_coefficient_dev,
                                    void *stream);
void mfgpu_level_destroy(mfgpu_level *level);

// ... 151 lines not shown
```

Measured before the change: 80.49 billion DoFs/s.

## Pair adjacent plane batches in one workgroup and fuse shared-DoF reduction via LDS

```diff
diff --git a/dealii-cuda_amd/csrc/mfgpu_api.hip b/dealii-cuda_amd/csrc/mfgpu_api.hip
--- a/dealii-cuda_amd/csrc/mfgpu_api.hip
+++ b/dealii-cuda_amd/csrc/mfgpu_api.hip
@@ -64,6 +64,8 @@
   DeviceArray<uint32_t> d_bdofsp, d_idxp;
   DeviceArray<uint32_t> d_shtab;
   bool shared_records = false;
+  bool pair = false;
+  DeviceArray<uint32_t> d_pair;
   size_t record_bytes = 0;
   DeviceArray<uint32_t> d_hnrec;
   DeviceArray<uint32_t> d_hn_slot;
@@ -96,9 +98,9 @@
   size_t lds = 0, device_bytes = 0;
   PlaneKernel planes = PlaneKernel::none;
   BatchKernel batches = BatchKernel::none;
-  enum { kPlain, kMasked, kBatch };
-  CellKernel<double> kernels_f64[3];
-  CellKernel<float> kernels_f32[3];
+  enum { kPlain, kMasked, kBatch, kPair };
+  CellKernel<double> kernels_f64[4];
+  CellKernel<float> kernels_f32[4];
   template <typename T>
   CellKernel<T> &kernel(int which) {
     if constexpr (std::is_same<T, double>::value) return kernels_f64[which];
@@ -179,9 +181,10 @@
   const Plan &P = h->plan;
   const size_t ng = 1 + h->seg_end.size();
   const bool shared = P.sh_p2_use && !h->no_shared_records && n_priority == 0 && ng == 2;
+  if (n_priority || ng != 2) h->pair = false;
   std::vector<Pass2Group> groups;
   int rc;
-  if ((rc = pass2_groups(P, h->seg_end, priority, n_priority, shared, groups))) return rc;
+  if ((rc = pass2_groups(P, h->seg_end, priority, n_priority, shared, h->pair, groups))) return rc;
   std::vector<DeviceArray<uint32_t>> d_arr(ng), d_tiles(ng);
   std::vector<uint32_t> n_tiles(ng, 0u);
   const bool reverse = (size_t)P.halo_off.back() * esize(h->number_type) <= ((size_t)256 << 20);
@@ -279,6 +282,14 @@
     if ((rc = up(h->d_idxp, rx.data(), rx.size()))) return rc;
     if (h->shared_records && (rc = up(h->d_shtab, P.sh_batch.data(), P.sh_batch.size()))) return rc;
     h->record_bytes = h->d_bdofsp.bytes() + h->d_idxp.bytes() + h->d_shtab.bytes();
+    h->plan.pair_mode = P.pair_offer && pairs_wanted(d);
+    h->pair = P.pair_mode && kernel_exists(h->planes, P.n, d.number_type, false, h->shared_records, false, true) &&
+              !(h->shared_records ? P.sh_pair : P.pr_pair).empty();
+    if (h->pair) {
+      const std::vector<uint32_t> &rp = h->shared_records ? P.sh_pair : P.pr_pair;
+      if ((rc = up(h->d_pair, rp.data(), rp.size()))) return rc;
+      h->record_bytes += h->d_pair.bytes();
+    }
   }
   if ((rc = up(h->d_orphans, P.orphans.data(), P.orphans.size()))) return rc;
   if (h->twopass) {
@@ -357,6 +368,15 @@
     CellKernel<T> &plain = h->kernel<T>(mfgpu_handle::kPlain), &masked = h->kernel<T>(mfgpu_handle::kMasked);
     HIP_TRY(bind_kernel<T>(h, h->planes, BatchKernel::none, false, h->shared_records, &plain));
     h->lds = plain.lds;
+    if (h->pair) {
+      CellKernel<T> &pk = h->kernel<T>(mfgpu_handle::kPair);
+      HIP_TRY(p_bind_pair<T>(P.n, h->shared_records, &pk));
+      if (pk.lds > kMaxLdsBytes || pk.per_cu < 1) {
+        set_error("internal: the pair kernel does not fit a CU");
+        return MFGPU_EINVAL;
+      }
+      h->lds = std::max(h->lds, pk.lds);
+    }
     if (P.n_plain_plane_batches < P.n_plane_batches) {
       HIP_TRY(bind_kernel<T>(h, h->planes, BatchKernel::none, true, false, &masked));
       h->lds = std::max(h->lds, masked.lds);
@@ -427,7 +447,8 @@
   if (h->p2_shared && group == 1)
     HIP_TRY(reduce_owner_batches_launch<T>((T *)dst, (const T *)src, h->d_halo.as<const T>(), h->d_p2rec.get(),
                                            h->d_p2tab.get(), (uint32_t)(h->plan.batch_cell_off.size() - 1),
-                                           (uint32_t)p_hs(h->plan.n) * 64u, h->p2_reverse ? 1 : 0, add, st));
+                                           (uint32_t)p_hs(h->plan.n) * 64u, h->p2_reverse ? 1 : 0, add,
+                                           h->pair ? 1 : 0, st));
   HIP_TRY(reduce_classes_launch<T>((T *)dst, (const T *)src, h->d_halo.as<const T>(), h->d_p2arr[group].get(),
                                    h->d_p2tiles[group].get(), h->n_p2tiles[group], add, st));
   return 0;
@@ -449,6 +470,15 @@
 int launch_cells(mfgpu_handle *h, ApplyArgs<T> a, uint32_t b0, uint32_t b1, hipStream_t st) {
   const Plan &P = h->plan;
   const uint32_t npl = P.n_plane_batches, nplain = P.n_plain_plane_batches;
+  if (h->pair) {
+    if (b0 != 0 || b1 != nplain || a.hole_len) {
+      set_error("internal: a handle in pair mode runs its cell loop in one piece");
+      return MFGPU_EINVAL;
+    }
+    a.batch0 = 0;
+    a.batch_end = nplain;
+    return launch_bound(h, h->kernel<T>(mfgpu_handle::kPair), a, nplain / 2, st);
+  }
   if (b0 < nplain) {
     a.batch0 = b0;
     a.batch_end = b1 < nplain ? b1 : nplain;
@@ -481,6 +511,7 @@
   a.bdofsp = h->d_bdofsp.get();
   a.idxp = h->d_idxp.get();
   a.shtab = h->shared_records ? h->d_shtab.get() : nullptr;
+  a.pairp = h->pair ? h->d_pair.get() : nullptr;
   a.hnrec = h->d_hnrec.get();
   a.hn_slot = h->d_hn_slot.get();
   a.coefp = h->d_coefp.as<const T>();
@@ -688,7 +719,7 @@
   return h->twopass ? upload_pass2(h, ids, n) : 0;
 }
 int handle_n_batches(const mfgpu_handle *h) { return (int)h->plan.batch_cell_off.size() - 1; }
-bool handle_ranged_ok(const mfgpu_handle *h) { return h->twopass && h->seg_end.size() == 1; }
+bool handle_ranged_ok(const mfgpu_handle *h) { return h->twopass && h->seg_end.size() == 1 && !h->pair; }
 int handle_batches_touching(const mfgpu_handle *h, const uint32_t *ids, uint32_t n, std::vector<uint8_t> &flags) {
   const Plan &P = h->plan;
   std::vector<uint8_t> mark(P.n_dofs, 0);
@@ -921,6 +952,16 @@
   return 0;
 }
 
+int mfgpu_pair_stats(const mfgpu_handle *h, uint64_t s[4]) {
+  if (!h || !s) return MFGPU_EINVAL;
+  const Plan &P = h->plan;
+  s[0] = h->pair ? 1 : 0;
+  s[1] = h->pair ? P.n_pairs : 0;
+  s[2] = h->pair ? P.fused_dofs : 0;
+  s[3] = h->pair ? (h->shared_records ? P.sh_pair.size() : P.pr_pair.size()) / kPairWords : 0;
+  return 0;
+}
+
 int mfgpu_record_stats(const mfgpu_handle *h, uint64_t s[4]) {
   if (!h || !s) return MFGPU_EINVAL;
   const Plan &P = h->plan;
diff --git a/dealii-cuda_amd/csrc/mfgpu_internal.h b/dealii-cuda_amd/csrc/mfgpu_internal.h
--- a/dealii-cuda_amd/csrc/mfgpu_internal.h
+++ b/dealii-cuda_amd/csrc/mfgpu_internal.h
@@ -73,6 +73,9 @@
   bool sh_use = false;
   std::vector<uint32_t> sh_p2rec, sh_p2tab;
   bool sh_p2_use = false;
+  bool pair_offer = false, pair_mode = false;
+  uint32_t n_pairs = 0, fused_dofs = 0;
+  std::vector<uint32_t> pair_fused, pr_pair, sh_pair;
   uint64_t n_first = 0, n_add = 0;
 };
 
@@ -82,6 +85,7 @@
   bool segregate_masked = false;
   bool masked_planes = false;
   uint32_t private_max = 0;
+  bool pairs = false;
 };
 
 int build_plan(const mfgpu_desc &d, Plan &plan, uint32_t max_chunks = 3, const PlanLimits *limits = nullptr);
@@ -96,7 +100,8 @@
 int choose_kernel_and_plan(const mfgpu_desc &d, PlaneKernel &pk, BatchKernel &bk, Plan &plan);
 
 constexpr bool planes4_wide(int n) { return n >= 6; }
-constexpr bool kernel_exists(PlaneKernel k, int n, int number_type, bool hn, bool sh, bool mass) {
+constexpr bool kernel_exists(PlaneKernel k, int n, int number_type, bool hn, bool sh, bool mass, bool pair = false) {
+  if (pair && (k != PlaneKernel::planes3 || n != 5 || hn || mass)) return false;
   switch (k) {
     case PlaneKernel::planes3: return n >= 3 && n <= 5 && !(sh && hn);
     case PlaneKernel::planes4:
@@ -119,6 +124,11 @@
 constexpr double kShareMaxFraction = 0.5;
 void share_plane_records(Plan &plan);
 constexpr int kP2Header = 16, kP2MaxK = 12, kP2SlotBits = 12;
+constexpr int kP2Fused = 15;
+constexpr int kPairMaxFused = 64, kPairWords = 2 * 2 * 64;
+inline bool pairs_wanted(const mfgpu_desc &d) {
+  return !(d.flags & MFGPU_NO_BATCH_PAIRS) && !d.mass_coefficient && d.cell_loop_segments <= 1;
+}
 void share_pass2_records(Plan &plan);
 
 std::vector<uint16_t> x_lane_permutation(int n);
@@ -127,7 +137,7 @@
   std::vector<uint32_t> dofs, offsets = std::vector<uint32_t>(1, 0u), slots;
 };
 int pass2_groups(const Plan &plan, const std::vector<uint32_t> &seg_end, const uint32_t *priority, uint32_t n_priority,
-                 bool shared, std::vector<Pass2Group> &groups);
+                 bool shared, bool pair, std::vector<Pass2Group> &groups);
 
 int derive_tables(int n, const double *shape_values, const double *shape_gradients,
                   std::vector<double> &S, std::vector<double> &Dt);
diff --git a/dealii-cuda_amd/csrc/mfgpu_kernels.h b/dealii-cuda_amd/csrc/mfgpu_kernels.h
--- a/dealii-cuda_amd/csrc/mfgpu_kernels.h
+++ b/dealii-cuda_amd/csrc/mfgpu_kernels.h
@@ -43,6 +43,7 @@
   const uint32_t *shtab = nullptr;
   const T *mass = nullptr;
   const T *massp = nullptr;
+  const uint32_t *pairp = nullptr;
 };
 
 constexpr int kMaxFusedWidth = 3;
@@ -131,6 +132,8 @@
 MFGPU_CELL_LOOP_FAMILY(q)
 #undef MFGPU_CELL_LOOP_FAMILY
 template <typename T>
+hipError_t p_bind_pair(int n, bool sh, CellKernel<T> *k);
+template <typename T>
 using MultiKernel = CellKernel<T, MultiArgs<T>>;
 template <typename T, typename Args>
 hipError_t g_bind_width(int n, bool hn, bool sh, bool mass, int nv, uint32_t nb_max, CellKernel<T, Args> *k);
@@ -145,7 +148,8 @@
                                        const uint32_t *tiles, uint32_t n_tiles, int add, hipStream_t st);
 template <typename T>
 hipError_t reduce_owner_batches_launch(T *dst, const T *src, const T *halo, const uint32_t *rec, const uint32_t *tab,
-                                       uint32_t n_batches, uint32_t hstride, int reverse, int add, hipStream_t st);
+                                       uint32_t n_batches, uint32_t hstride, int reverse, int add, int pair,
+                                       hipStream_t st);
 template <typename T>
 hipError_t relayout_coef_launch(T *out, const T *in, const uint32_t *cell_batch, const uint32_t *cell_pos,
                                 size_t total, int n, hipStream_t st);
diff --git a/dealii-cuda_amd/csrc/mfgpu_kernels_p.hip b/dealii-cuda_amd/csrc/mfgpu_kernels_p.hip
--- a/dealii-cuda_amd/csrc/mfgpu_kernels_p.hip
+++ b/dealii-cuda_amd/csrc/mfgpu_kernels_p.hip
@@ -8,8 +8,23 @@
 
 #define MFGPU_PIN_VMEM() __builtin_amdgcn_sched_barrier(0x380)
 
-template <int n, typename T, bool ADD, bool HN, bool SH = false, bool MASS = false>
-__global__ void __launch_bounds__(64) __attribute__((amdgpu_waves_per_eu(1, 1)))
+template <int n, typename T>
+constexpr size_t p_pair_region_bytes() {
+  return (((size_t)p_kgu(n) * 64 * sizeof(double) + (size_t)2 * (p_cells_per_wave(n) + 1) * p_cell_stride(n) * sizeof(T)) +
+          15) / 16 * 16;
+}
+template <typename T>
+__device__ __forceinline__ T zero_if_flagged(T v, uint32_t g) {
+  if constexpr (sizeof(T) == 8) {
+    const unsigned long long keep = (unsigned long long)(long long)~((int)g >> 31);
+    return (T)__longlong_as_double((long long)((unsigned long long)__double_as_longlong((double)v) & keep));
+  } else {
+    return (T)__int_as_float(__float_as_int((float)v) & ~((int)g >> 31));
+  }
+}
+
+template <int n, typename T, bool ADD, bool HN, bool SH = false, bool MASS = false, bool PAIR = false>
+__global__ void __launch_bounds__(PAIR ? 128 : 64) __attribute__((amdgpu_waves_per_eu(1, 1)))
 apply_planes3(const ApplyArgs<T> A, const TablesEO<T, n> tab) {
   constexpr int n2 = n * n;
   constexpr int CW = p_cells_per_wave(n);
@@ -21,12 +36,18 @@
   constexpr int NIW = (n2 + 1) / 2;
   extern __shared__ __attribute__((aligned(16))) unsigned char smem_raw[];
   constexpr int PRIV = HN ? p_priv_max(n) : 0;
-  double *ua = reinterpret_cast<double *>(smem_raw);
+  constexpr size_t REGION = p_pair_region_bytes<n, T>();
+  static_assert(!PAIR || !HN, "pair regions");
+  const int wv = PAIR ? __builtin_amdgcn_readfirstlane((int)(threadIdx.x >> 6)) : 0;
+  unsigned char *const smem = smem_raw + (PAIR ? (size_t)wv * REGION : 0);
+  T *const xch_own = reinterpret_cast<T *>(smem_raw + 2 * REGION) + (PAIR ? wv * 128 : 0);
+  const T *const xch_other = reinterpret_cast<const T *>(smem_raw + 2 * REGION) + (PAIR ? (1 - wv) * 128 : 0);
+  double *ua = reinterpret_cast<double *>(smem);
   T *Aw = reinterpret_cast<T *>(ua + KGU * 64 + PRIV + (HN ? n2 : 0));
   T *Bw = Aw + (CW + 1) * SA;
   double *Wl = ua + KGU * 64 + PRIV;
 
-  const int lane = threadIdx.x;
+  const int lane = PAIR ? (int)(threadIdx.x & 63u) : (int)threadIdx.x;
   if (HN) {
     if (lane < n2) Wl[lane] = (double)A.hn_weights[lane];
   }
@@ -36,19 +57,25 @@
 
   uint32_t b, bstride, bend;
   {
-    const uint32_t nbt = A.batch_end - A.batch0 - A.hole_len, G = gridDim.x;
+    const uint32_t nbt = PAIR ? (A.batch_end - A.batch0) >> 1 : A.batch_end - A.batch0 - A.hole_len, G = gridDim.x;
+    const uint32_t first = PAIR ? 0u : A.batch0;
     if (G >= 8 && nbt >= G) {
       const uint32_t xcd = blockIdx.x & 7u, slot = blockIdx.x >> 3;
       const uint32_t q = G >> 3, rem = G & 7u;
       const uint32_t wlo = xcd * q + (xcd < rem ? xcd : rem);
       const uint32_t w = q + (xcd < rem ? 1u : 0u);
-      b = A.batch0 + (uint32_t)((uint64_t)nbt * wlo / G) + slot;
-      bend = A.batch0 + (uint32_t)((uint64_t)nbt * (wlo + w) / G);
+      b = first + (uint32_t)((uint64_t)nbt * wlo / G) + slot;
+      bend = first + (uint32_t)((uint64_t)nbt * (wlo + w) / G);
       bstride = w;
     } else {
-      b = A.batch0 + blockIdx.x;
-      bend = A.batch_end - A.hole_len;
+      b = first + blockIdx.x;
+      bend = first + nbt;
       bstride = G;
+    }
+    if (PAIR) {
+      b = A.batch0 + 2 * b + (uint32_t)wv;
+      bend = A.batch0 + 2 * bend;
+      bstride *= 2;
     }
   }
   if (b >= bend) return;
@@ -58,7 +85,7 @@
     return l < bend ? (l >= hole0 ? l + hole_len : l) : x;
   };
   if (b >= hole0) b += hole_len;
-  static_assert(kernel_exists(PlaneKernel::planes3, n, number_type_of<T>, HN, SH, MASS), "no such instantiation");
+  static_assert(kernel_exists(PlaneKernel::planes3, n, number_type_of<T>, HN, SH, MASS, PAIR), "no such instantiation");
   struct Meta {
     uint32_t base, drec, irec;
   };
@@ -111,6 +138,18 @@
     }
   };
 
+  auto load_pair = [&](uint32_t rec, uint32_t &px, uint32_t &gf) {
+    const uint32_t *p = A.pairp + (size_t)rec * kPairWords + wv * 128 + lane;
+    px = SH ? p[0] : nt_load(p);
+    gf = SH ? p[64] : nt_load(p + 64);
+  };
+  auto pair_barrier = [&]() {
+    __builtin_amdgcn_fence(__ATOMIC_RELEASE, "wavefront");
+    asm volatile("s_waitcnt lgkmcnt(0)" ::: "memory");
+    __builtin_amdgcn_s_barrier();
+    asm volatile("" ::: "memory");
+    __builtin_amdgcn_fence(__ATOMIC_ACQUIRE, "wavefront");
+  };
   uint32_t b1 = next_of(b), b2 = next_of(b1);
   uint32_t Gp[KGU], Gc[KGU], Gn[KGU], Gnn[KGU];
   uint32_t IXc[NIW], IXn[NIW];
@@ -130,6 +169,9 @@
   T Cc[n2];
   T Mm[MASS ? n2 : 1];
   T SVn[KGU], R[KGU], old[KGU];
+  uint32_t PXc = 0u, PXn = 0u, GFc = 0u, GFn = 0u, GFp = 0u;
+  T Fown = T(0), Fother = T(0), oldF = T(0);
+  int xbuf = 0;
   Meta Mp{0u, 0u, 0u}, Mc = Mp, M1 = Mp, M2 = Mp;
   uint32_t Mv = 0u;
   if (SH) {
@@ -142,6 +184,10 @@
   load_dofs(SH ? M1.drec : b1, Gn);
   load_ix(SH ? Mc.irec : b, IXc);
   if (HN) load_hn(b, Hc);
+  if (PAIR) {
+    load_pair(SH ? Mc.drec : b, PXc, GFc);
+    GFp = GFc;
+  }
   constexpr uint32_t kDummyIx = 8u * (uint32_t)(KGU * 64 - 1) * 0x10001u;
 #pragma unroll
   for (int w = 0; w < NIW; ++w) IXc[w] = lane_on ? IXc[w] : kDummyIx;
@@ -229,9 +275,11 @@
     load_ix(SH ? M1.irec : b1, IXn);
     if (SH) Mv = meta_request(next_of(b2));
     if (HN) load_hn(b1, Hn);
+    if (PAIR) load_pair(SH ? M1.drec : b1, PXn, GFn);
     if (ADD) {
 #pragma unroll
       for (int j = 0; j < JI; ++j) old[j] = *dst_at(Mp.base, Gp[j]);
+      if (PAIR) oldF = *dst_at(Mp.base, GFp);
     }
     STAMP(1);
     auto hookA = [&](int) {};
@@ -240,6 +288,10 @@
 #pragma unroll
       for (int j = (KGU * s) / (5 * n); j < (KGU * (s + 1)) / (5 * n); ++j)
         scatter_slot(j, bp, Mp.base, Gp[j], R[j], old[j]);
+      if (PAIR && s == 5 * n - 1) {
+        const T f = zero_if_flagged<T>(Fown + Fother, GFp);
+        *dst_at(Mp.base, GFp) = ADD ? oldF + f : f;
+      }
 #pragma unroll
       for (int j = (KGU * s) / (5 * n); j < (KGU * (s + 1)) / (5 * n); ++j)
         SVn[j] = src_at(M1.base, Gn[j]);
@@ -427,7 +479,16 @@
     }
 #pragma unroll
     for (int j = 0; j < KGU; ++j) R[j] = (T)ua[lane + j * 64];
+    if (PAIR) {
+      Fown = (T) * reinterpret_cast<const double *>(reinterpret_cast<const char *>(ua) + PXc);
+      xch_own[xbuf * 64 + lane] = Fown;
+    }
     WaveSync::sync();
+    if (PAIR) {
+      pair_barrier();
+      Fother = xch_other[xbuf * 64 + lane];
+      xbuf ^= 1;
+    }
     STAMP(5);
     stage_src(Gn, SVn);
     STAMP(6);
@@ -435,6 +496,7 @@
     if (SH) Mp = Mc;
 #pragma unroll
     for (int j = 0; j < KGU; ++j) Gp[j] = Gc[j];
+    if (PAIR) GFp = GFc;
     STAMP(7);
     RSTAMP(9);
     if (!has_next) break;
@@ -458,19 +520,32 @@
 #pragma unroll
       for (int w = 0; w < HROWS; ++w) Hc[w] = Hn[w];
     }
+    if (PAIR) {
+      PXc = PXn;
+      GFc = GFn;
+    }
   }
   if (ADD) {
 #pragma unroll
     for (int j = 0; j < JI; ++j) old[j] = *dst_at(Mp.base, Gp[j]);
+    if (PAIR) oldF = *dst_at(Mp.base, GFp);
   }
 #pragma unroll
   for (int j = 0; j < KGU; ++j) scatter_slot(j, bp, Mp.base, Gp[j], R[j], old[j]);
+  if (PAIR) {
+    const T f = zero_if_flagged<T>(Fown + Fother, GFp);
+    *dst_at(Mp.base, GFp) = ADD ? oldF + f : f;
+  }
 }
 
 template <int n, typename T>
 static size_t p_lds_bytes(bool hn) {
   return ((size_t)p_kgu(n) * 64 + (hn ? (size_t)p_priv_max(n) + n * n : 0)) * sizeof(double) +
          (size_t)2 * (p_cells_per_wave(n) + 1) * p_cell_stride(n) * sizeof(T);
+}
+template <int n, typename T>
+static size_t p_pair_lds_bytes() {
+  return 2 * p_pair_region_bytes<n, T>() + (size_t)2 * 2 * 64 * sizeof(T);
 }
 
 template <typename T>
@@ -484,6 +559,20 @@
       return hipErrorInvalidValue;
   }, hn, sh, mass);
 }
+template <typename T>
+hipError_t p_bind_pair(int n, bool sh, CellKernel<T> *k) {
+  return dispatch_instantiation(n, [&](auto N, auto SH) {
+    constexpr int n_ = N;
+    if constexpr (kernel_exists(PlaneKernel::planes3, n_, number_type_of<T>, false, SH, false, true))
+      return bind_cell_kernel<T, 128, apply_planes3<n_, T, false, false, SH, false, true>,
+                              apply_planes3<n_, T, true, false, SH, false, true>, make_tables_eo<T, n_>>(
+          p_pair_lds_bytes<n_, T>(), k);
+    else
+      return hipErrorInvalidValue;
+  }, sh);
+}
+template hipError_t p_bind_pair<double>(int, bool, CellKernel<double> *);
+template hipError_t p_bind_pair<float>(int, bool, CellKernel<float> *);
 template hipError_t p_bind<double>(int, int, bool, bool, bool, bool, uint32_t, CellKernel<double> *);
 template hipError_t p_bind<float>(int, int, bool, bool, bool, bool, uint32_t, CellKernel<float> *);
 
diff --git a/dealii-cuda_amd/csrc/mfgpu_pass2.hip b/dealii-cuda_amd/csrc/mfgpu_pass2.hip
--- a/dealii-cuda_amd/csrc/mfgpu_pass2.hip
+++ b/dealii-cuda_amd/csrc/mfgpu_pass2.hip
@@ -104,7 +104,7 @@
 __device__ __forceinline__ void reduce_owned(T *__restrict__ dst, const T *__restrict__ src,
                                              const T *__restrict__ halo, const uint32_t *__restrict__ r, uint32_t e,
                                              uint32_t d, uint32_t kk, uint32_t kw, uint32_t hslot0, uint32_t hstride,
-                                             int add) {
+                                             uint2 fused, int add) {
   const T *const hb = halo + hslot0;
   auto partial = [&](uint32_t w) -> T {
     return hb[(w >> kP2SlotBits) * hstride + (w & ((1u << kP2SlotBits) - 1u))];
@@ -114,6 +114,7 @@
 #pragma unroll
   for (int t = 0; t < KU; ++t) w[t] = (uint32_t)t < kk ? r[r[3 + t] + e] : 0u;
   if (d == 0xffffffffu) return;
+  if (fused.y && e - fused.x < fused.y && !(d >> 31)) return;
   T v;
   if (d >> 31) {
     v = src[d & 0x7fffffffu];
@@ -137,11 +138,13 @@
 __global__ void __launch_bounds__(256)
 reduce_owner_batches(T *__restrict__ dst, const T *__restrict__ src, const T *__restrict__ halo,
                      const uint32_t *__restrict__ rec, const uint2 *__restrict__ tab, uint32_t n_batches,
-                     uint32_t hstride, int reverse, int add) {
+                     uint32_t hstride, int reverse, int add, int pair) {
   const uint32_t ob = reverse ? n_batches - 1u - blockIdx.x : blockIdx.x;
   const uint2 t = tab[ob];
   const uint32_t *const r = rec + t.y;
   const uint32_t e0 = r[1];
+  const uint32_t fw = pair && !(ob & 1u) ? r[kP2Fused] : 0u;
+  const uint2 fused = make_uint2(fw & 0xffffu, fw >> 16);
   dst += t.x;
   src += t.x;
   for (uint32_t e = threadIdx.x; e < e0; e += 256u) {
@@ -150,13 +153,13 @@
     const uint32_t h0 = ob * hstride;
     switch (kw) {
       case 0: break;
-      case 1: reduce_owned<T, 1>(dst, src, halo, r, e, d, kk, kw, h0, hstride, add); break;
-      case 2: reduce_owned<T, 2>(dst, src, halo, r, e, d, kk, kw, h0, hstride, add); break;
-      case 3: reduce_owned<T, 3>(dst, src, halo, r, e, d, kk, kw, h0, hstride, add); break;
-      case 4: reduce_owned<T, 4>(dst, src, halo, r, e, d, kk, kw, h0, hstride, add); break;
+      case 1: reduce_owned<T, 1>(dst, src, halo, r, e, d, kk, kw, h0, hstride, fused, add); break;
+      case 2: reduce_owned<T, 2>(dst, src, halo, r, e, d, kk, kw, h0, hstride, fused, add); break;
+      case 3: reduce_owned<T, 3>(dst, src, halo, r, e, d, kk, kw, h0, hstride, fused, add); break;
+      case 4: reduce_owned<T, 4>(dst, src, halo, r, e, d, kk, kw, h0, hstride, fused, add); break;
       case 5: case 6: case 7:
-      case 8: reduce_owned<T, 8>(dst, src, halo, r, e, d, kk, kw, h0, hstride, add); break;
-      default: reduce_owned<T, 0>(dst, src, halo, r, e, d, kk, kw, h0, hstride, add); break;
+      case 8: reduce_owned<T, 8>(dst, src, halo, r, e, d, kk, kw, h0, hstride, fused, add); break;
+      default: reduce_owned<T, 0>(dst, src, halo, r, e, d, kk, kw, h0, hstride, fused, add); break;
     }
   }
 }
@@ -225,16 +228,19 @@
                                                        const uint32_t *, const uint32_t *, uint32_t, int, hipStream_t);
 template <typename T>
 hipError_t reduce_owner_batches_launch(T *dst, const T *src, const T *halo, const uint32_t *rec, const uint32_t *tab,
-                                       uint32_t n_batches, uint32_t hstride, int reverse, int add, hipStream_t st) {
+                                       uint32_t n_batches, uint32_t hstride, int reverse, int add, int pair,
+                                       hipStream_t st) {
   if (n_batches == 0) return hipSuccess;
   hipLaunchKernelGGL(reduce_owner_batches<T>, dim3(n_batches), dim3(256), 0, st, dst, src, halo, rec,
-                     reinterpret_cast<const uint2 *>(tab), n_batches, hstride, reverse, add);
+                     reinterpret_cast<const uint2 *>(tab), n_batches, hstride, reverse, add, pair);
   return hipGetLastError();
 }
 template hipError_t reduce_owner_batches_launch<double>(double *, const double *, const double *, const uint32_t *,
-                                                        const uint32_t *, uint32_t, uint32_t, int, int, hipStream_t);
+                                                        const uint32_t *, uint32_t, uint32_t, int, int, int,
+                                                        hipStream_t);
 template hipError_t reduce_owner_batches_launch<float>(float *, const float *, const float *, const uint32_t *,
-                                                       const uint32_t *, uint32_t, uint32_t, int, int, hipStream_t);
+                                                       const uint32_t *, uint32_t, uint32_t, int, int, int,
+                                                       hipStream_t);
 template hipError_t reduce_classes_launch<double>(double *, const double *, const double *, const uint32_t *,
                                                   const uint32_t *, uint32_t, int, hipStream_t);
 template hipError_t reduce_classes_launch<float>(float *, const float *, const float *, const uint32_t *,
diff --git a/dealii-cuda_amd/csrc/mfgpu_plan.cpp b/dealii-cuda_amd/csrc/mfgpu_plan.cpp
--- a/dealii-cuda_amd/csrc/mfgpu_plan.cpp
+++ b/dealii-cuda_amd/csrc/mfgpu_plan.cpp
@@ -716,6 +716,56 @@
     i = j;
   }
 }
+std::vector<std::vector<uint32_t>> fusable_dofs(const Plan &P) {
+  const size_t nb = P.batch_cell_off.size() - 1;
+  const uint32_t hs = (uint32_t)p_hs(P.n) * 64u;
+  std::vector<std::vector<uint32_t>> f(nb);
+  for (size_t i = 0; i < P.sdofs.size(); ++i) {
+    if (P.s_off[i + 1] - P.s_off[i] != 2 || (P.sdofs[i] >> 31)) continue;
+    const uint32_t t0 = P.s_idx[P.s_off[i]] / hs, t1 = P.s_idx[P.s_off[i] + 1] / hs;
+    if (t1 == t0 + 1 && t0 < nb && f[t0].size() < (size_t)kPairMaxFused) f[t0].push_back((uint32_t)i);
+  }
+  return f;
+}
+
+void find_batch_pairs(Plan &P, const Description &m, const Incidence &inc) {
+  P.pair_offer = P.pair_mode = false;
+  P.n_pairs = P.fused_dofs = 0;
+  P.pair_fused.clear();
+  const size_t nb = P.batch_cell_off.size() - 1;
+  if (nb < 2 || (nb & 1) || P.n_plane_batches != nb || P.n_plain_plane_batches != nb || m.dim != 3) return;
+  const uint32_t full = (uint32_t)p_cells_per_wave(m.n);
+  std::vector<uint32_t> batch_of(m.nc, NONE);
+  for (size_t b = 0; b < nb; ++b) {
+    if (P.batch_cell_off[b + 1] - P.batch_cell_off[b] != full) return;
+    for (uint32_t c = P.batch_cell_off[b]; c < P.batch_cell_off[b + 1]; ++c) batch_of[P.cell_order[c]] = (uint32_t)b;
+  }
+  const std::vector<uint32_t> nbr = face_neighbours(m, inc);
+  auto across = [&](uint32_t c, int side) {
+    const uint32_t c2 = nbr[(size_t)c * 6 + side];
+    return c2 == NONE ? NONE : batch_of[c2];
+  };
+  const std::vector<std::vector<uint32_t>> f = fusable_dofs(P);
+  for (uint32_t L = 0; L < nb; L += 2) {
+    const uint32_t R = L + 1;
+    uint32_t faces = 0;
+    for (uint32_t c = P.batch_cell_off[L]; c < P.batch_cell_off[L + 1]; ++c) {
+      const uint32_t hi = across(P.cell_order[c], 1), lo = across(P.cell_order[c], 0);
+      if ((hi != L && hi != R) || lo == R) return;
+      faces += hi == R;
+    }
+    for (uint32_t c = P.batch_cell_off[R]; c < P.batch_cell_off[R + 1]; ++c) {
+      const uint32_t hi = across(P.cell_order[c], 1), lo = across(P.cell_order[c], 0);
+      if ((lo != L && lo != R) || hi == L) return;
+    }
+    if (faces == 0 || f[L].empty()) return;
+  }
+  for (uint32_t L = 0; L < nb; L += 2) P.pair_fused.insert(P.pair_fused.end(), f[L].begin(), f[L].end());
+  std::sort(P.pair_fused.begin(), P.pair_fused.end());
+  P.pair_offer = true;
+  P.n_pairs = (uint32_t)(nb / 2);
+  P.fused_dofs = (uint32_t)P.pair_fused.size();
+}
 }
 
 int build_plan(const mfgpu_desc &d, Plan &P, uint32_t max_chunks, const PlanLimits *limits) {
@@ -743,6 +793,8 @@
   count_plane_batches(P, R, B.masked);
   emit_pass2_csr(P, m, C.ntouch, G);
   emit_pass2_groups(P, G);
+  P.pair_offer = P.pair_mode = false;
+  if (limits && limits->pairs) find_batch_pairs(P, m, inc);
   return 0;
 }
 
@@ -762,6 +814,14 @@
   std::vector<HnLine> lines[3];
   std::vector<uint16_t> pnodes;
   std::vector<uint32_t> priv_pos((size_t)P.nd);
+  std::vector<std::vector<uint32_t>> fus;
+  std::vector<uint32_t> local_slot, avoid;
+  if (P.pair_offer) {
+    fus = fusable_dofs(P);
+    local_slot.assign(P.n_dofs, 0u);
+  }
+  P.pr_pair.assign(P.pair_offer ? nbat * (size_t)kPairWords : 0, 0u);
+  bool pairs_fit = true;
   for (size_t b = 0; b < nbat; ++b) {
     const uint32_t c0 = P.batch_cell_off[b], nc = P.batch_cell_off[b + 1] - c0;
     const uint32_t d0 = P.batch_dof_off[b], nbd = P.batch_dof_off[b + 1] - d0, ni = P.batch_nint[b];
@@ -771,9 +831,32 @@
     }
     slot_of.assign(nbd, 0u);
     for (uint32_t t = 0; t < nbd; ++t) slot_of[t] = t < ni ? t : (uint32_t)JI + (t - ni);
+    uint32_t pad_t = ni;
+    if (P.pair_offer) {
+      avoid.clear();
+      for (size_t nbb = b ? b - 1 : b; nbb <= b; ++nbb)
+        for (uint32_t i : fus[nbb]) avoid.push_back(P.sdofs[i] & 0x7fffffffu);
+      std::sort(avoid.begin(), avoid.end());
+      while (pad_t < nbd && std::binary_search(avoid.begin(), avoid.end(), P.bdofs[d0 + pad_t] & 0x7fffffffu)) ++pad_t;
+      if (pad_t == nbd) {
+        pairs_fit = false;
+        pad_t = ni;
+      }
+      for (uint32_t t = 0; t < nbd; ++t) local_slot[P.bdofs[d0 + t] & 0x7fffffffu] = slot_of[t];
+      uint32_t *rec = P.pr_pair.data() + b * (size_t)kPairWords;
+      const uint32_t padg = (P.bdofs[d0 + pad_t] & 0x7fffffffu) | 0x80000000u;
+      for (int w = 0; w < 2; ++w)
+        for (uint32_t i = 0; i < 64; ++i) {
+          const std::vector<uint32_t> *f = w == 0 ? &fus[b] : b ? &fus[b - 1] : nullptr;
+          const bool on = f && i < f->size();
+          const uint32_t g = on ? P.sdofs[(*f)[i]] & 0x7fffffffu : 0u;
+          rec[(w * 2 + 0) * 64 + i] = on ? 8u * local_slot[g] : dummy;
+          rec[(w * 2 + 1) * 64 + i] = on && w == 0 ? g : padg;
+        }
+    }
     for (int t = 0; t < NB; ++t) {
       uint32_t src_t;
-      if (t < JI) src_t = (uint32_t)t < ni ? (uint32_t)t : ni;
+      if (t < JI) src_t = (uint32_t)t < ni ? (uint32_t)t : pad_t;
       else src_t = std::min<uint32_t>(ni + (uint32_t)(t - JI), nbd - 1);
       bd[b * NB + t] = P.bdofs[d0 + src_t];
     }
@@ -835,6 +918,12 @@
       }
     }
   }
+  if (!pairs_fit) {
+    P.pair_offer = P.pair_mode = false;
+    P.n_pairs = P.fused_dofs = 0;
+    P.pair_fused.clear();
+    return build_plane_records(P, constraint_mask);
+  }
   share_plane_records(P);
   share_pass2_records(P);
   return 0;
@@ -867,6 +956,8 @@
   P.sh_dofs.clear();
   P.sh_idx.clear();
   P.sh_batch.assign(nbat * kShBatchWords, 0u);
+  P.sh_pair.clear();
+  bool pair_records_shared = true;
   SeenRecords seen_d, seen_x;
   std::vector<uint32_t> rel(NB);
   for (size_t b = 0; b < nbat; ++b) {
@@ -878,10 +969,29 @@
     e[0] = base;
     e[1] = (uint32_t)(intern_record(P.sh_dofs, seen_d, rel.data(), NB) / NB);
     e[2] = (uint32_t)(intern_record(P.sh_idx, seen_x, P.pr_idx.data() + b * NX, NX) / NX);
+    if (P.pair_offer) {
+      uint32_t prel[kPairWords];
+      for (int t = 0; t < kPairWords; ++t) {
+        const uint32_t w = P.pr_pair[b * (size_t)kPairWords + t];
+        prel[t] = ((t >> 6) & 1) ? (w & 0x80000000u) | ((w & 0x7fffffffu) - base) : w;
+      }
+      const size_t at = (size_t)e[1] * kPairWords;
+      if (at == P.sh_pair.size()) P.sh_pair.insert(P.sh_pair.end(), prel, prel + kPairWords);
+      else if (std::memcmp(P.sh_pair.data() + at, prel, sizeof(prel))) pair_records_shared = false;
+    }
   }
   const size_t shared = P.sh_dofs.size() + P.sh_idx.size() + P.sh_batch.size();
   const size_t expanded = P.pr_dofs.size() + P.pr_idx.size();
   P.sh_use = nbat > 0 && P.pr_hn.empty() && (double)shared <= kShareMaxFraction * (double)expanded;
+  if (P.pair_offer && !pair_records_shared) {
+    P.sh_pair.clear();
+    if (P.sh_use) {
+      P.pair_offer = P.pair_mode = false;
+      P.n_pairs = P.fused_dofs = 0;
+      P.pair_fused.clear();
+      P.pr_pair.clear();
+    }
+  }
 }
 
 void share_pass2_records(Plan &P) {
@@ -910,6 +1020,8 @@
   P.sh_p2tab.assign(2 * nb, 0u);
   SeenRecords seen;
   std::vector<uint32_t> rec;
+  std::vector<std::vector<uint32_t>> fus;
+  if (P.pair_offer) fus = fusable_dofs(P);
   for (size_t b = 0; b < nb; ++b) {
     std::vector<uint32_t> &m = owned[b];
     auto k_of = [&](uint32_t i) { return P.s_off[i + 1] - P.s_off[i]; };
@@ -921,6 +1033,15 @@
     rec[0] = ne;
     rec[1] = e0;
     rec[2] = kmax;
+    if (P.pair_offer && !fus[b].empty()) {
+      uint32_t lo = ne, hi = 0;
+      for (uint32_t e = 0; e < ne; ++e)
+        if (std::binary_search(fus[b].begin(), fus[b].end(), m[e])) {
+          lo = std::min(lo, e);
+          hi = e + 1;
+        }
+      if (lo < hi) rec[kP2Fused] = lo | ((hi - lo) << 16);
+    }
     rec.resize(kP2Header + 2 * (size_t)e0, 0u);
     for (uint32_t e = 0; e < e0; ++e) rec[kP2Header + e] = e < ne ? P.sdofs[m[e]] - base : 0xffffffffu;
     for (uint32_t e = 0; e < ne; ++e) rec[kP2Header + e0 + e] = k_of(m[e]);
@@ -983,6 +1104,7 @@
     lim.segregate_masked = hn;
     lim.masked_planes = hn && plane_kernel_exists(true);
     lim.private_max = (uint32_t)p_priv_max(d.degree + 1);
+    lim.pairs = !hn && kernel_exists(plane_kind, d.degree + 1, d.number_type, false, false, false, true);
   }
   int rc = build_plan(d, plan, (pencils_x && d.degree == 3) ? 4u : 3u, planes ? &lim : nullptr);
   if (rc == MFGPU_EUNSUPPORTED && planes && d.kernel == MFGPU_KERNEL_AUTO && xk_ok) {
@@ -1046,7 +1168,8 @@
 }
 
 int pass2_groups(const Plan &P, const std::vector<uint32_t> &seg_end, const uint32_t *priority, uint32_t n_priority,
-                 bool shared, std::vector<Pass2Group> &groups) {
+                 bool shared, bool pair, std::vector<Pass2Group> &groups) {
+  size_t next_fused = 0;
   std::vector<uint8_t> prio(P.n_dofs, 0);
   for (uint32_t i = 0; i < n_priority; ++i) {
     if (priority[i] >= P.n_dofs) {
@@ -1064,6 +1187,10 @@
   };
   for (size_t i = 0; i < P.sdofs.size(); ++i) {
     size_t seg = 0;
+    if (pair && next_fused < P.pair_fused.size() && P.pair_fused[next_fused] == i) {
+      ++next_fused;
+      continue;
+    }
     if (shared && P.s_off[i + 1] > P.s_off[i]) continue;
     if (P.s_off[i + 1] > P.s_off[i]) {
       const uint32_t slot = P.s_idx[P.s_off[i + 1] - 1];
@@ -1095,6 +1222,7 @@
   d.mass_coefficient = nullptr;
   int rc = mfgpu::choose_kernel_and_plan(d, pk, bk, p->plan);
   if (!rc && pk != mfgpu::PlaneKernel::none) rc = mfgpu::build_plane_records(p->plan, desc->constraint_mask);
+  p->plan.pair_mode = !rc && p->plan.pair_offer && mfgpu::pairs_wanted(*desc);
   if (rc) {
     delete p;
     return rc;
@@ -1170,6 +1298,9 @@
     case 19: v = &p->plan.sh_batch; break;
     case 20: v = &p->plan.sh_p2rec; break;
     case 21: v = &p->plan.sh_p2tab; break;
+    case 22: v = &p->plan.pair_fused; break;
+    case 23: v = &p->plan.pr_pair; break;
+    case 24: v = &p->plan.sh_pair; break;
     default: mfgpu::set_error("bad array id"); return MFGPU_EINVAL;
   }
   *ptr = v->data();
@@ -1188,6 +1319,16 @@
   return p ? (p->plan.sh_use ? 1 : 0) | (p->plan.sh_p2_use ? 2 : 0) : 0;
 }
 
+int mfgpu_plan_pair_stats(const mfgpu_plan *p, uint64_t s[4]) {
+  if (!p || !s) return MFGPU_EINVAL;
+  const mfgpu::Plan &P = p->plan;
+  s[0] = P.pair_mode ? 1 : 0;
+  s[1] = P.pair_mode ? P.n_pairs : 0;
+  s[2] = P.pair_mode ? P.fused_dofs : 0;
+  s[3] = P.pair_mode ? (P.sh_pair.empty() ? P.n_pairs * 2 : P.sh_pair.size() / mfgpu::kPairWords) : 0;
+  return 0;
+}
+
 int64_t mfgpu_plan_lmap(const mfgpu_plan *p, const uint16_t **ptr) {
   if (!p || !ptr) return MFGPU_EINVAL;
   *ptr = p->plan.lmap.data();
diff --git a/dealii-cuda_amd/pymfgpu/__init__.py b/dealii-cuda_amd/pymfgpu/__init__.py
--- a/dealii-cuda_amd/pymfgpu/__init__.py
+++ b/dealii-cuda_amd/pymfgpu/__init__.py
@@ -13,6 +13,7 @@
 EUNSUPPORTED = -4
 MULTI_ADD, MULTI_LOOP, MULTI_FUSED = 1, 2, 4
 UNIFORM_J0, HANGING_NODES, COLORED_SCATTER, NO_SHARED_RECORDS = 1, 2, 1 << 8, 1 << 9
+NO_BATCH_PAIRS = 1 << 11
 UPDATABLE_COEFFICIENTS = 1 << 10
 KERNEL_AUTO, KERNEL_PENCILS, KERNEL_PENCILS_X, KERNEL_PLANES, KERNEL_PLANES_2W = 0, 1, 2, 3, 4
 
@@ -84,7 +85,7 @@
     "mfgpu_vec_sadd", "mfgpu_vec_equ", "mfgpu_vec_scale", "mfgpu_vec_divide", "mfgpu_vec_invert", "mfgpu_vec_mul",
     "mfgpu_vec_dot", "mfgpu_vec_l2_norm", "mfgpu_vec_add_and_dot", "mfgpu_vec_all_zero", "mfgpu_profile_enable", "mfgpu_profile_read", "mfgpu_profile_read_pass2",
     "mfgpu_plan_create", "mfgpu_plan_destroy", "mfgpu_plan_array_u32", "mfgpu_plan_lmap", "mfgpu_plan_bflags",
-    "mfgpu_plan_shares_records", "mfgpu_record_stats",
+    "mfgpu_plan_shares_records", "mfgpu_record_stats", "mfgpu_pair_stats", "mfgpu_plan_pair_stats",
     "mfgpu_vec_alloc", "mfgpu_vec_free", "mfgpu_vec_fill", "mfgpu_vec_from_host", "mfgpu_vec_to_host",
     "mfgpu_device_synchronize", "mfgpu_device_memory_info", "mfgpu_mesh_create_uniform", "mfgpu_mesh_create_adaptive", "mfgpu_mesh_create_ball", "mfgpu_mesh_create_from_leaves",
     "mfgpu_mesh_cell_levels", "mfgpu_mesh_destroy",
@@ -169,6 +170,8 @@
         L.mfgpu_plan_bflags.restype = C.c_int64
         L.mfgpu_plan_shares_records.argtypes = [C.c_void_p]
         L.mfgpu_record_stats.argtypes = [C.c_void_p, C.POINTER(C.c_uint64)]
+        L.mfgpu_pair_stats.argtypes = [C.c_void_p, C.POINTER(C.c_uint64)]
+        L.mfgpu_plan_pair_stats.argtypes = [C.c_void_p, C.POINTER(C.c_uint64)]
         L.mfgpu_vec_alloc.argtypes = [C.POINTER(C.c_void_p), C.c_size_t, C.c_int]
         L.mfgpu_vec_free.argtypes = [C.c_void_p]
         L.mfgpu_vec_fill.argtypes = [C.c_void_p, C.c_size_t, C.c_int, C.c_double, C.c_void_p]
@@ -520,6 +523,14 @@
     sh_p2rec = property(lambda s: s._u32(20))
     sh_p2tab = property(lambda s: s._u32(21).reshape(-1, 2))
     shares_pass2_records = property(lambda s: bool(lib().mfgpu_plan_shares_records(s._h) & 2))
+    pair_fused = property(lambda s: s._u32(22))
+    pr_pair = property(lambda s: s._u32(23).reshape(-1, 2, 2, 64))
+    sh_pair = property(lambda s: s._u32(24).reshape(-1, 2, 2, 64))
+
+    def pair_stats(self):
+        r = (C.c_uint64 * 4)()
+        _check(lib().mfgpu_plan_pair_stats(self._h, r))
+        return dict(pair_mode=bool(r[0]), n_pairs=int(r[1]), fused_dofs=int(r[2]), pair_records=int(r[3]))
 
     @property
     def lmap(self):
@@ -668,6 +679,9 @@
         out.update(index_records="shared" if r[0] & 1 else "expanded",
                    pass2_records="shared" if r[0] & 2 else "expanded", distinct_dof_records=int(r[1]),
                    distinct_index_records=int(r[2]), index_record_bytes=int(r[3]))
+        q = (C.c_uint64 * 4)()
+        _check(lib().mfgpu_pair_stats(self._h, q))
+        out.update(pair_mode=bool(q[0]), n_pairs=int(q[1]), fused_dofs=int(q[2]), pair_records=int(q[3]))
         return out
 
     def kernel_name(self):
diff --git a/include/mfgpu.h b/include/mfgpu.h
--- a/include/mfgpu.h
+++ b/include/mfgpu.h
@@ -25,6 +25,8 @@
 #define MFGPU_NO_SHARED_RECORDS (1u << 9)
 
 #define MFGPU_UPDATABLE_COEFFICIENTS (1u << 10)
+
+#define MFGPU_NO_BATCH_PAIRS (1u << 11)
 
 typedef struct mfgpu_handle mfgpu_handle;
 
@@ -92,6 +94,8 @@
 
 int mfgpu_record_stats(const mfgpu_handle *h, uint64_t stats[4]);
 
+int mfgpu_pair_stats(const mfgpu_handle *h, uint64_t stats[4]);
+
 const char *mfgpu_kernel_name(const mfgpu_handle *h);
 
 int mfgpu_profile_enable(mfgpu_handle *h, int on);
@@ -103,6 +107,7 @@
 void mfgpu_plan_destroy(mfgpu_plan *p);
 int64_t mfgpu_plan_array_u32(const mfgpu_plan *p, int what, const uint32_t **ptr);
 int mfgpu_plan_shares_records(const mfgpu_plan *p);
+int mfgpu_plan_pair_stats(const mfgpu_plan *p, uint64_t stats[4]);
 int mfgpu_plan_multi_groups(uint32_t n_vectors, const uint32_t *widths, uint32_t n_widths, uint32_t *groups,
                             uint32_t capacity);
 int64_t mfgpu_plan_lmap(const mfgpu_plan *p, const uint16_t **ptr);
```

Measured after the change: 82.94 billion DoFs/s, median of 6. +3.0%, better.
